# zakuro-ai/asr

Measured on AMD Instinct MI355X. Metric: utterances/sec (10 s, 161-bin) DS2 5x1024 BiGRU CTC train step, higher is better.
Workload: dtype bf16

## Files before the change

### asr_amd/_lib.py

```python
from __future__ import annotations

import ctypes as C
import os
from typing import Optional

_HERE = os.path.dirname(os.path.abspath(__file__))
LIB_PATH = os.environ.get("DS2_LIB_PATH") or os.path.join(_HERE, "lib", "libds2hip.so")

_lib: Optional[C.CDLL] = None

vp, i32, i64, f32, f64, sz = C.c_void_p, C.c_int, C.c_longlong, C.c_float, C.c_double, C.c_size_t

SIGNATURES = {
    "ds2_version": (C.c_char_p, []),
    "ds2_last_error": (C.c_char_p, []),
    "ds2_device_info": (i32, [C.POINTER(i32), C.POINTER(i32), C.c_char_p, i32]),
    "ds2_debug_flags": (i32, [vp, i32]),
    "ds2_rnn_ctx_init": (i32, [vp, vp, vp, vp]),
    "ds2_memset_async": (i32, [vp, i32, sz, vp]),
    "ds2_ablation_build": (i32, []),
    "ds2_rnn_persistent_status": (i32, [vp, vp]),
    "ds2_rnn_persistent_counters": (i32, [vp, vp]),
    "ds2_rnn_poison_if_starved": (i32, [vp, vp, sz, vp]),
    "ds2_rnn_poison_seen": (i32, [vp]),
    "ds2_rnn_step_gate": (i32, [vp, vp, vp, vp]),
    "ds2_rnn_persistent_enable": (i32, [vp, i32, i32]),
    "ds2_rnn_last_path": (i32, [vp]),
    "ds2_rnn_bwd_ksplit_footprint": (i32, [i32, i32, C.POINTER(i32)]),
    "ds2_gemm_f32_workspace_bytes": (sz, [i32, i32, i32, i32]),
    "ds2_gemm_f32": (i32, [i32, i32, i32, i32, i32, vp, i32, i64, vp, i32, i64, vp, i32, i64, vp, i32, i32, i32, vp, sz, vp]),
    "ds2_gemm_bf16_workspace_bytes": (sz, [i32, i32, i32, i32]),
    "ds2_conv1_fwd_bf16_stat_blocks": (i32, [i32, i32, i32]),
    "ds2_conv1_fwd_bf16_stats": (i32, [vp, vp, vp, vp, vp, i32, i32, i32, vp, vp]),
    "ds2_conv2_fwd_bf16_stat_blocks": (i32, [i32, i32, i32]),
    "ds2_conv2_fwd_bf16_stats": (i32, [vp, vp, vp, vp, vp, i32, i32, i32, vp, vp]),
    "ds2_chanstats_from_partials_workspace_bytes": (sz, []),
    "ds2_chanstats_from_partials": (i32, [vp, i32, i32, f64, vp, vp, vp, vp, f32, vp, sz, vp]),
    "ds2_gemm_bf16_tn": (i32, [i32, i32, i32, vp, i32, i64, vp, i32, i64, vp, i32, i64, i32, i32, i32, vp, sz, vp]),
    "ds2_gemm_bf16_tn_group": (i32, [i32, vp, i32, vp]),
    "ds2_gemm_bf16_tn_splitk_group_workspace_bytes": (sz, [i32, vp, i32]),
    "ds2_gemm_bf16_tn_splitk_group": (i32, [i32, vp, i32, vp, sz, vp]),
    "ds2_gemm_bf16_tn_splitk_group_ep": (i32, [i32, vp, i32, i32, vp, vp, vp, vp, sz, vp]),
    "ds2_gemm_bf16_nt": (i32, [i32, i32, i32, vp, i32, i64, vp, i32, i64, vp, i32, i64, vp, i32, i32, i32, vp, sz, vp]),
    "ds2_cast_bf16": (i32, [vp, i32, vp, i32, i32, i32, vp]),
    "ds2_gemm_bf16_nt_obf16": (i32, [i32, i32, i32, vp, i32, vp, i32, vp, i32, vp, vp]),
    "ds2_cast_f32_from_bf16": (i32, [vp, vp, i64, vp]),
    "ds2_rnn_fwd_x": (i32, [vp, i32, vp, vp, vp, vp, vp, vp, vp, i32, i32, i32, vp, vp, vp, vp, sz, vp]),
    "ds2_split_bf16": (i32, [vp, i32, vp, i32, i32, i32, i32, vp]),
    "ds2_cast_transpose_bf16": (i32, [vp, i32, vp, i32, i32, i32, vp]),
    "ds2_cast_bf16_both_workspace_bytes": (sz, [i32, i32]),
    "ds2_cast_bf16_both": (i32, [vp, i32, vp, i32, vp, i32, i32, i32, vp, vp, sz, vp]),
    "ds2_transpose_bf16": (i32, [vp, i32, vp, i32, i32, i32, vp, vp, sz, vp]),
    "ds2_colreduce_workspace_bytes": (sz, [i32, i32]),
    "ds2_colstats_f32": (i32, [vp, i32, i32, i32, vp, vp, vp, vp, f32, vp, sz, vp]),
    "ds2_add_colstats_f32": (i32, [vp, i32, vp, i32, vp, i32, i32, i32, vp, vp, vp, vp, f32, vp, sz, vp]),
    "ds2_colsum_f32": (i32, [vp, i32, i32, i32, vp, vp, vp, sz, vp]),
    "ds2_bn1d_apply_f32": (i32, [vp, i32, vp, i32, i32, i32, vp, vp, vp, vp, f32, vp]),
    "ds2_bn1d_apply_bf16": (i32, [vp, i32, vp, i32, i32, i32, vp, vp, vp, vp, f32, vp]),
    "ds2_bn1d_bwd_f32": (i32, [vp, i32, vp, i32, vp, i32, i32, i32, vp, vp, vp, f32, vp, vp, vp, sz, vp]),
    "ds2_bn1d_bwd_xbf16": (i32, [vp, i32, vp, i32, vp, i32, i32, i32, vp, vp, vp, f32, vp, vp, vp, sz, vp]),
    "ds2_center_colstats": (i32, [vp, i32, vp, i32, vp, i32, vp, i32, i32, i32, vp, vp, vp, vp, vp, f32, vp, sz, vp]),
    "ds2_wih_fold_bf16": (i32, [vp, i32, vp, i32, i32, vp, vp, vp, vp, f32, vp, i32, vp, vp, vp, vp]),
    "ds2_scale_rank1_f32": (i32, [vp, i32, i32, i32, vp, vp, vp, vp]),
    "ds2_chanreduce_workspace_bytes": (sz, [i32]),
    "ds2_bn2d_stats_f32": (i32, [vp, i32, i32, i32, i32, vp, vp, vp, vp, f32, vp, sz, vp]),
    "ds2_bn2d_act_fwd_f32": (i32, [vp, vp, i32, i32, i32, i32, vp, vp, vp, vp, vp, f32, vp]),
    "ds2_bn2d_act_bwd_f32": (i32, [vp, vp, vp, i32, i32, i32, i32, vp, vp, vp, vp, vp, f32, vp, vp, vp, sz, vp]),
    "ds2_bn2d_act_fwd_fused": (i32, [vp, i32, i32, i32, vp, vp, vp, vp, vp, f32, vp, vp, vp, vp]),
    "ds2_bn2d_act_collapse": (i32, [vp, i32, i32, i32, vp, vp, vp, vp, vp, f32, vp, vp, i32, vp]),
    "ds2_bn2d_act_bwd_fused_workspace_bytes": (sz, [i32, i32, i32]),
    "ds2_bn2d_act_bwd_fused": (i32, [vp, vp, i32, i32, i32, vp, vp, vp, vp, vp, f32, vp, vp, vp, vp, vp, vp, vp, sz, vp]),
    "ds2_transpose_bft_f32": (i32, [vp, vp, i32, i32, i32, i32, vp]),
    "ds2_transpose2d_f32": (i32, [vp, i32, i64, vp, i32, i64, i32, i32, i32, vp]),
    "ds2_conv_dims": (None, [i32, i32, C.POINTER(i32), C.POINTER(i32), C.POINTER(i32)]),
    "ds2_conv_packed_floats": (sz, [i32]),
    "ds2_conv_pack_f32": (i32, [vp, vp, vp, vp, vp, vp]),
    "ds2_conv1_fwd_f32": (i32, [vp, vp, vp, vp, vp, i32, i32, i32, vp]),
    "ds2_conv2_fwd_f32": (i32, [vp, vp, vp, vp, vp, i32, i32, i32, vp]),
    "ds2_conv2_dgrad_f32": (i32, [vp, vp, vp, i32, i32, i32, vp]),
    "ds2_conv_wgrad_workspace_bytes": (sz, [i32, i32, i32]),
    "ds2_conv1_wgrad_f32": (i32, [vp, vp, vp, vp, i32, i32, i32, i32, vp, sz, vp]),
    "ds2_conv2_wgrad_f32": (i32, [vp, vp, vp, vp, i32, i32, i32, i32, vp, sz, vp]),
    "ds2_conv2_bf16_packed_bytes": (sz, [i32]),
    "ds2_conv2_pack_bf16": (i32, [vp, vp, vp, vp, vp]),
    "ds2_nhwc_bf16_f32": (i32, [vp, vp, i32, i32, i32, vp]),
    "ds2_conv2_fwd_bf16": (i32, [vp, vp, vp, vp, vp, i32, i32, i32, vp]),
    "ds2_conv2_dgrad_bf16": (i32, [vp, vp, vp, vp, i32, i32, i32, vp]),
    "ds2_conv_padded_pitch": (i32, [i32]),
    "ds2_padcast_bf16": (i32, [vp, vp, i64, i32, vp]),
    "ds2_conv2_wgrad_bf16_workspace_bytes": (sz, [i32, i32]),
    "ds2_conv2_wgrad_bf16": (i32, [vp, vp, vp, vp, i32, i32, i32, vp, sz, vp]),
    "ds2_conv2_wgrad_nhwc_bf16": (i32, [vp, vp, vp, vp, i32, i32, i32, vp, sz, vp]),
    "ds2_rnn_packed_bytes": (sz, [i32, i32, i32, i32]),
    "ds2_rnn_pack_whh": (i32, [i32, vp, vp, vp, i32, i32, vp]),
    "ds2_weight_prep_bf16": (i32, [vp, i32, vp]),
    "ds2_rnn_fwd_workspace_bytes": (sz, [i32, i32, i32]),
    "ds2_rnn_fwd_ex": (i32, [vp, i32, vp, vp, vp, vp, vp, vp, i32, i32, i32, i32, vp, vp, vp, sz, vp]),
    "ds2_rnn_fwd": (i32, [vp, i32, vp, vp, vp, vp, vp, vp, i32, i32, i32, i32, vp, vp, sz, vp]),
    "ds2_rnn_bwd_workspace_bytes": (sz, [i32, i32, i32, i32]),
    "ds2_rnn_bwd_ex": (i32, [vp, i32, vp, i32, vp, vp, vp, vp, vp, i32, i32, i32, i32, vp, vp, vp, vp, vp, sz, vp]),
    "ds2_rnn_bwd_bn": (i32, [vp, i32, vp, i32, vp, i32, vp, vp, vp, vp, vp, f32, vp, vp, vp, vp, vp, vp, i32, i32, i32, i32, vp, vp, vp, vp, vp, sz, vp]),
    "ds2_rnn_bwd_bn_xbf16": (i32, [vp, i32, vp, i32, vp, i32, vp, vp, vp, vp, vp, f32, vp, vp, vp, vp, vp, vp, i32, i32, i32, i32, vp, vp, vp, vp, vp, sz, vp]),
    "ds2_rnn_bias_grads": (i32, [i32, vp, i32, i32, vp, vp, vp]),
    "ds2_rnn_bwd": (i32, [vp, i32, vp, i32, vp, vp, vp, vp, vp, i32, i32, i32, i32, vp, vp, vp, sz, vp]),
    "ds2_ctc_workspace_bytes": (sz, [i32, i32, i32]),
    "ds2_ctc_loss_f32": (i32, [vp, i32, i32, i32, i32, vp, vp, vp, vp, i32, vp, vp, i32, f32, vp, sz, vp]),
    "ds2_ctc_loss_ex_f32": (i32, [vp, i32, i32, i32, i32, vp, vp, vp, vp, i32, vp, vp, i32, f32, i32, vp, sz, vp]),
    "ds2_ctc_star_workspace_bytes": (sz, [i32, i32, i32]),
    "ds2_ctc_star_loss_f32": (i32, [vp, i32, i32, i32, i32, vp, vp, vp, vp, i32, f32, vp, vp, vp, i32, f32, i32, vp, sz, vp]),
    "ds2_ctc_mwer_workspace_bytes": (sz, [i32, i32, i32, i32]),
    "ds2_ctc_mwer_f32": (i32, [vp, i32, i32, i32, i32, i32, vp, vp, vp, vp, vp, i32, vp, vp, vp, vp, vp, i32, f32, i32, i32, vp, sz, vp]),
    "ds2_ctc_conf_max_unit_labels": (i32, []),
    "ds2_ctc_conf_workspace_bytes": (sz, [i32, i32, i32]),
    "ds2_ctc_conf_f32": (i32, [vp, i32, i32, i32, i32, vp, vp, vp, vp, i32, vp, vp, vp, vp, vp, i32, vp, vp, i32, vp, sz, vp]),
    "ds2_ctc_batch_mean_f32": (i32, [vp, i32, vp, vp]),
    "ds2_ctc_align_workspace_bytes": (sz, [i32, i32, i32]),
    "ds2_ctc_align_f32": (i32, [vp, i64, i64, i32, i32, i32, i32, vp, vp, vp, vp, i32, i32, vp, vp, vp, vp, vp, vp, sz, vp]),
    "ds2_ctc_align_tiled_workspace_bytes": (sz, [i32, i32, i32, i32, i32]),
    "ds2_ctc_align_tiled_f32": (i32, [vp, i64, i64, i32, i32, i32, i32, vp, vp, vp, vp, i32, i32, i32, vp, vp, vp, vp, vp, vp, sz, vp]),
    "ds2_ctc_align_star_row_f32": (i32, [vp, i64, i64, i32, i32, i32, i32, vp, f32, vp, vp]),
    "ds2_ctc_align_star_workspace_bytes": (sz, [i32, i32, i32]),
    "ds2_ctc_align_star_f32": (i32, [vp, i64, i64, i32, i32, i32, i32, vp, vp, vp, vp, i32, i32, f32, vp, vp, vp, vp, vp, vp, vp, sz, vp]),
    "ds2_ctc_align_star_tiled_workspace_bytes": (sz, [i32, i32, i32, i32, i32]),
    "ds2_ctc_align_star_tiled_f32": (i32, [vp, i64, i64, i32, i32, i32, i32, vp, vp, vp, vp, i32, i32, i32, f32, vp, vp, vp, vp, vp, vp, vp,
                                           sz, vp]),
    "ds2_ctc_kws_workspace_bytes": (sz, [i32, i32, i32, i32]),
    "ds2_ctc_kws_f32": (i32, [vp, i64, i64, i32, i32, i32, i32, vp, vp, vp, vp, i32, i32, vp, i32, vp, vp, vp, vp, vp, vp, vp, sz, vp]),
    "ds2_add_i64": (i32, [vp, i32, i64, vp]),
    "ds2_softmax_rows_f32": (i32, [vp, i32, vp, i32, i32, i32, vp]),
    "ds2_greedy_decode_workspace_bytes": (sz, [i32, i32]),
    "ds2_greedy_decode_f32": (i32, [vp, i64, i64, i32, i32, i32, vp, i32, vp, vp, vp, vp, sz, vp]),
    "ds2_ctc_segment_workspace_bytes": (sz, [i32, i32]),
    "ds2_ctc_segment_f32": (i32, [vp, i64, i64, i32, i32, i32, vp, i32, f32, i32, i32, i32, i32, vp, vp, vp, vp, vp, sz, vp]),
    "ds2_ctc_segment_gather_f32": (i32, [vp, i64, i64, i32, i32, i32, vp, vp, vp, i32, i32, vp, vp, vp]),
    "ds2_ctc_beam_max_width": (i32, []),
    "ds2_ctc_beam_workspace_bytes": (sz, [i32, i32, i32]),
    "ds2_ctc_beam_decode_f32": (i32, [vp, i64, i64, i32, i32, i32, vp, i32, i32, i32, f32, vp, vp, vp, vp, vp, sz, vp]),
    "ds2_ctc_beam_lm_max_candidates": (i32, []),
    "ds2_ctc_lm_packed_bytes": (sz, [i32, i32, i32, i32, i32]),
    "ds2_ctc_lm_pack": (i32, [i32, i32, vp, vp, vp, vp, i32, vp, vp, vp, i32, vp, i32, vp, i32, i32, vp, sz]),
    "ds2_ctc_lm_score": (i32, [vp, vp, i32, i32, C.POINTER(f32)]),
    "ds2_ctc_beam_decode_lm_f32": (i32, [vp, i64, i64, i32, i32, i32, vp, i32, i32, i32, f32, vp, sz, i32, i32, i32, f32, f32, vp, vp, vp, vp,
                                         vp, sz, vp]),
    "ds2_ctc_hot_packed_bytes": (sz, [i32, i32]),
    "ds2_ctc_hot_pack": (i32, [i32, i32, vp, vp, vp, vp, vp, vp, i32, vp, sz]),
    "ds2_ctc_hot_step": (i32, [vp, i32, i32, C.POINTER(i32), C.POINTER(f32)]),
    "ds2_ctc_beam_decode_hot_f32": (i32, [vp, i64, i64, i32, i32, i32, vp, i32, i32, i32, f32, vp, sz, i32, i32, i32, f32, f32, vp, vp, sz,
                                          vp, vp, vp, vp, vp, sz, vp]),
    "ds2_edit_distance_workspace_bytes": (sz, [i32, i64]),
    "ds2_edit_distance_i32": (i32, [vp, i64, vp, vp, vp, vp, i32, i64, vp, vp, sz, vp]),
    "ds2_edit_align_workspace_bytes": (sz, [i32, i64]),
    "ds2_edit_align_i32": (i32, [vp, i64, vp, vp, vp, vp, i32, i64, vp, vp, vp, vp, sz, vp]),
    "ds2_conv1_bf16_row_pitch": (i32, [i32]),
    "ds2_conv1_bf16_bytes": (sz, [i32, i32, i32, i32]),
    "ds2_conv1_pack_bf16": (i32, [vp, vp, vp]),
    "ds2_conv1_gather_bf16": (i32, [vp, vp, vp, i32, i32, i32, vp]),
    "ds2_conv1_fwd_bf16": (i32, [vp, vp, vp, vp, vp, i32, i32, i32, vp]),
    "ds2_conv1_wgrad_bf16_workspace_bytes": (sz, [i32, i32]),
    "ds2_conv1_wgrad_bf16": (i32, [vp, vp, vp, vp, i32, i32, i32, vp, sz, vp]),
    "ds2_spectrogram_frames": (i32, [i32, i32]),
    "ds2_spectrogram_workspace_bytes": (sz, [i32, i32, i32, i32]),
    "ds2_spectrogram_f32": (i32, [vp, i64, vp, i32, i32, i32, i32, vp, i32, i32, vp, vp, sz, vp]),
    "ds2_spectrogram_aug_workspace_bytes": (sz, [i32, i32, i32, i32]),
    "ds2_spectrogram_aug_f32": (i32, [vp, i64, vp, i32, i32, i32, i32, vp, i32, i32, vp, i64, vp, vp, vp, vp, vp, i32, vp, i32, vp, vp, sz,
                                      vp]),
    "ds2_tempo_sizes": (i32, [i32, f64, f64, f64, C.POINTER(i32), C.POINTER(i32), C.POINTER(i32)]),
    "ds2_tempo_out_samples": (i32, [i32, f64]),
    "ds2_tempo_workspace_bytes": (sz, [i32]),
    "ds2_tempo_gain_f32": (i32, [vp, i64, vp, vp, vp, i32, i32, f64, f64, f64, vp, i64, vp, vp, i32, vp, sz, vp]),
    "ds2_wave_unpack_f32": (i32, [vp, i64, i32, vp, vp, vp, i32, i32, vp, i64, vp]),
    "ds2_resample_out_samples": (i64, [i64, i32, i32]),
    "ds2_resample_tile_samples": (i32, []),
    "ds2_wave_resample_f32": (i32, [vp, i64, i32, vp, vp, vp, vp, vp, vp, vp, vp, i64, i32, i32, vp, i64, vp]),
    "ds2_reverb_max_taps": (i32, []),
    "ds2_reverb_tile_samples": (i32, []),
    "ds2_reverb_tap_chunk": (i32, []),
    "ds2_reverb_f32": (i32, [vp, i64, vp, vp, i64, vp, vp, i32, i32, vp, i64, vp]),
    "ds2_adamw_f32": (i32, [vp, vp, vp, vp, i64, f32, f32, f32, f32, f32, i32, f32, vp]),
    "ds2_adamw_gated_f32": (i32, [vp, vp, vp, vp, i64, f32, f32, f32, f32, f32, i32, f32, vp, vp]),
    "ds2_scale_f32": (i32, [vp, i64, f32, vp]),
    "ds2_bf16_residual_f32": (i32, [vp, vp, i64, vp]),
    "ds2_sum3_f32": (i32, [vp, vp, vp, vp, i64, vp]),
}


class TnProblem(C.Structure):
    _fields_ = [("A", vp), ("B", vp), ("C", vp), ("M", i32), ("N", i32), ("K", i32), ("lda", i32), ("ldb", i32), ("ldc", i32)]


class PrepLayer(C.Structure):
    _fields_ = [("whh", vp), ("wp_fwd", vp), ("wp_bwd", vp), ("wih", vp), ("wih_t", vp), ("wih_r", vp),
                ("gates", i32), ("H", i32), ("R", i32), ("Cc", i32), ("ld_wih", i32), ("ld_t", i32), ("ld_r", i32), ("reserved", i32)]


class DS2LibraryError(RuntimeError):
    pass


def load() -> C.CDLL:
    global _lib
    if _lib is not None:
        return _lib
    if not os.path.exists(LIB_PATH):
        raise DS2LibraryError(
            f"{LIB_PATH} not found: build the HIP extension first "
            "(python -c 'import __graft_entry__ as g; g.build()'  or  make -C asr_amd/csrc). "
            "asr_amd has no CPU fallback.")
    lib = C.CDLL(LIB_PATH)
    for name, (res, args) in SIGNATURES.items():
        fn = getattr(lib, name)
        fn.restype = res
        fn.argtypes = args
    _lib = lib
    return lib


def check(rc: int, what: str = ""):
    if rc != 0:
        msg = load().ds2_last_error().decode(errors="replace")
        raise DS2LibraryError(f"libds2hip call failed{(' in ' + what) if what else ''}: {msg}")


def version() -> str:
    return load().ds2_version().decode()


def conv_dims(F: int, Tin: int):
    d1, d2, t = i32(), i32(), i32()
    load().ds2_conv_dims(F, Tin, C.byref(d1), C.byref(d2), C.byref(t))
    return d1.value, d2.value, t.value
```

### asr_amd/csrc/conv_bf16.hip

```cpp
#include "common.h"
#include <stdlib.h>

namespace {

typedef __bf16 bf16x8 __attribute__((ext_vector_type(8)));

constexpr int TT = 128, KT = 11, PT = 5, CH = 32;
constexpr int NPIX = TT + KT - 1;
constexpr int IPITCH = 80;
constexpr int WROW = KT * 2 * 2 * 32 * 16;

__device__ __attribute__((aligned(16))) float g_zero_cb[4] = {0.f, 0.f, 0.f, 0.f};

struct CArgs {
  const __bf16* in;
  const __bf16* wpk;
  const float* bias;
  float* out;
  const int* lens;
  int B, Din, T, Dtot, KD, SD, PD, OS, OO;
  int gx, gy, gz;
};

constexpr int IN_CHUNKS = NPIX * 4;
constexpr int IN_IT = (IN_CHUNKS + 255) / 256;
constexpr int W_CHUNKS = WROW / 16;
constexpr int W_IT = (W_CHUNKS + 255) / 256;

template <int SD, int R>
__global__ __launch_bounds__(256) void conv2_bf16_rows_kernel(CArgs a, int n_out, float* __restrict__ stat_part) {
  constexpr int RING = (R - 1) * SD + 1;
  constexpr int SLOT = NPIX * IPITCH;
  __shared__ __attribute__((aligned(16))) char in_lds[RING * SLOT];
  __shared__ __attribute__((aligned(16))) char w_lds[WROW];
  const int tid = threadIdx.x, lane = tid & 63, wave = tid >> 6;
  const int half = lane >> 5, l31 = lane & 31;
  int bx, by, bz;
  {
    const int total = a.gx * a.gy * a.gz, id = blockIdx.x;
    const int lin = (total & 7) == 0 ? (id & 7) * (total >> 3) + (id >> 3) : id;
    by = lin % a.gy;
    const int pair = lin / a.gy;
    bx = pair % a.gx; bz = pair / a.gx;
  }
  const int t0 = bx * TT, o0 = R * by, b = bz;
  const int len = a.lens ? min(a.lens[b], a.T) : a.T;
  const int t = t0 + wave * 32 + l31;
  auto out_ptr = [&](int o, int co) { return a.out + (((long long)b * CH + co) * a.Dtot + (a.OS * o + a.OO)) * a.T + t; };
  if (t0 >= len) {
    if (t < a.T) {
#pragma unroll
      for (int q = 0; q < R; ++q)
        if (o0 + q < n_out) {
#pragma unroll
          for (int r = 0; r < 16; ++r) *out_ptr(o0 + q, (r & 3) + 8 * (r >> 2) + 4 * half) = 0.f;
        }
    }
    return;
  }
  f32x16 acc[R];
#pragma unroll
  for (int q = 0; q < R; ++q)
#pragma unroll
    for (int r = 0; r < 16; ++r) acc[q][r] = 0.f;

  const int f0 = SD * o0 - a.PD;
  f32x4 ri[IN_IT], rw[W_IT];
  auto load_in = [&](int f) {
    const bool rowok = f >= 0 && f < a.Din;
    const char* rowp = reinterpret_cast<const char*>(a.in + (((long long)b * a.Din + (rowok ? f : 0)) * a.T) * CH);
#pragma unroll
    for (int u = 0; u < IN_IT; ++u) {
      const int c = tid + 256 * u;
      const int pix = c >> 2, q = c & 3;
      const int tt = t0 - PT + pix;
      const bool ok = rowok && c < IN_CHUNKS && tt >= 0 && tt < a.T;
      const void* p = ok ? (const void*)(rowp + ((long long)tt * CH) * 2 + q * 16) : (const void*)g_zero_cb;
      ri[u] = *reinterpret_cast<const f32x4*>(p);
    }
  };
  auto store_in = [&](int slot) {
#pragma unroll
    for (int u = 0; u < IN_IT; ++u) {
      const int c = tid + 256 * u;
      if (c < IN_CHUNKS) *reinterpret_cast<f32x4*>(in_lds + slot * SLOT + (c >> 2) * IPITCH + (c & 3) * 16) = ri[u];
    }
  };
  auto load_w = [&](int kd) {
    const char* wp = reinterpret_cast<const char*>(a.wpk) + (long long)kd * WROW;
#pragma unroll
    for (int u = 0; u < W_IT; ++u) {
      const int c = tid + 256 * u;
      rw[u] = *reinterpret_cast<const f32x4*>(wp + (c < W_CHUNKS ? c : 0) * 16);
    }
  };
  auto store_w = [&]() {
#pragma unroll
    for (int u = 0; u < W_IT; ++u) {
      const int c = tid + 256 * u;
      if (c < W_CHUNKS) *reinterpret_cast<f32x4*>(w_lds + c * 16) = rw[u];
    }
  };
#pragma unroll
  for (int j = 0; j < RING - 1; ++j) {
    load_in(f0 + j);
    store_in(j);
  }
  load_in(f0 + RING - 1);
  load_w(0);
  const int pix_off = (wave * 32 + l31) * IPITCH + half * 16;
  const char* abase = w_lds + half * (32 * 16) + l31 * 16;
  int slot0 = 0;
  for (int kd = 0; kd < a.KD; ++kd) {
    __syncthreads();
    {
      int snew = slot0 + RING - 1;
      if (snew >= RING) snew -= RING;
      store_in(snew);
    }
    store_w();
    __syncthreads();
    if (kd + 1 < a.KD) {
      load_in(f0 + kd + RING);
      load_w(kd + 1);
    }
    const char* bq[R];
#pragma unroll
    for (int q = 0; q < R; ++q) {
      int sl = slot0 + q * SD;
      if (sl >= RING) sl -= RING;
      bq[q] = in_lds + sl * SLOT + pix_off;
    }
#pragma unroll
    for (int kt = 0; kt < KT; ++kt) {
#pragma unroll
      for (int kk = 0; kk < 2; ++kk) {
        const bf16x8 af = *reinterpret_cast<const bf16x8*>(abase + (kt * 2 + kk) * (2 * 32 * 16));
#pragma unroll
        for (int q = 0; q < R; ++q) {
          const bf16x8 x = *reinterpret_cast<const bf16x8*>(bq[q] + kt * IPITCH + kk * 32);
          acc[q] = __builtin_amdgcn_mfma_f32_32x32x16_bf16(af, x, acc[q], 0, 0, 0);
        }
      }
    }
    slot0 = slot0 + 1 == RING ? 0 : slot0 + 1;
  }
  float bv[16];
#pragma unroll
  for (int r = 0; r < 16; ++r) bv[r] = a.bias ? a.bias[(r & 3) + 8 * (r >> 2) + 4 * half] : 0.f;
  float s1[16], s2[16];
#pragma unroll
  for (int r = 0; r < 16; ++r) { s1[r] = 0.f; s2[r] = 0.f; }
#pragma unroll
  for (int q = 0; q < R; ++q)
    if (o0 + q < n_out) {
#pragma unroll
      for (int r = 0; r < 16; ++r) {
        const float v = (t >= len || t >= a.T) ? 0.f : acc[q][r] + bv[r];
        if (t < a.T) *out_ptr(o0 + q, (r & 3) + 8 * (r >> 2) + 4 * half) = v;
        s1[r] += v;
        s2[r] += v * v;
      }
    }
  if (stat_part) {
    __shared__ float red[4][32][2];
#pragma unroll
    for (int r = 0; r < 16; ++r) {
#pragma unroll
      for (int m = 1; m < 32; m <<= 1) { s1[r] += __shfl_xor(s1[r], m); s2[r] += __shfl_xor(s2[r], m); }
      if (l31 == 0) { const int co = (r & 3) + 8 * (r >> 2) + 4 * half; red[wave][co][0] = s1[r]; red[wave][co][1] = s2[r]; }
    }
    __syncthreads();
    if (tid < 64) {
      const int co = tid >> 1, w = tid & 1;
      const float sum = ((red[0][co][w] + red[1][co][w]) + red[2][co][w]) + red[3][co][w];
      const long long blk = ((long long)bz * a.gy + by) * a.gx + bx;
      stat_part[(blk * 32 + co) * 2 + w] = sum;
    }
  }
}

__global__ __launch_bounds__(256) void nhwc_cast_kernel(const float* __restrict__ src, __bf16* __restrict__ dst, int Bn, int D, int T) {
  __shared__ float tile[CH][65];
  const int t0 = blockIdx.x * 64, d = blockIdx.y, b = blockIdx.z;
  const int tx = threadIdx.x & 63, ty = threadIdx.x >> 6;
#pragma unroll
  for (int i = 0; i < 8; ++i) {
    const int c = ty + 4 * i, t = t0 + tx;
    tile[c][tx] = (t < T) ? src[(((long long)b * CH + c) * D + d) * T + t] : 0.f;
  }
  __syncthreads();
  const int c = threadIdx.x & 31, tq = threadIdx.x >> 5;
#pragma unroll
  for (int i = 0; i < 8; ++i) {
    const int tl = tq + 8 * i, t = t0 + tl;
    if (t < T) dst[(((long long)b * D + d) * T + t) * CH + c] = (__bf16)tile[c][tl];
  }
}

__global__ void pack_conv2_bf16_kernel(const float* __restrict__ W, __bf16* __restrict__ wf, __bf16* __restrict__ wd0, __bf16* __restrict__ wd1) {
  const int per_row = WROW / 2;
  const int nf = 21 * per_row, n0 = 11 * per_row, n1 = 10 * per_row;
  const int idx = blockIdx.x * blockDim.x + threadIdx.x;
  if (idx >= nf + n0 + n1) return;
  int which, i;
  if (idx < nf) { which = 0; i = idx; } else if (idx < nf + n0) { which = 1; i = idx - nf; } else { which = 2; i = idx - nf - n0; }
  const int j = i & 7, m = (i >> 3) & 31, kg = (i >> 8) & 1, kk = (i >> 9) & 1;
  const int rest = i >> 10;
  const int kt = rest % KT, kdr = rest / KT;
  const int kch = kk * 16 + kg * 8 + j;
  float v;
  if (which == 0) {
    v = W[((m * 32 + kch) * 21 + kdr) * 11 + kt];
    wf[i] = (__bf16)v;
  } else {
    const int p = which - 1, KDe = (21 - p + 1) / 2;
    v = W[((kch * 32 + m) * 21 + (2 * (KDe - 1 - kdr) + p)) * 11 + (10 - kt)];
    (which == 1 ? wd0 : wd1)[i] = (__bf16)v;
  }
}

}

extern "C" size_t ds2_conv2_bf16_packed_bytes(int which) { return (size_t)(which == 0 ? 21 : which == 1 ? 11 : 10) * WROW; }

extern "C" int ds2_conv2_pack_bf16(const float* w2, void* wf, void* wd0, void* wd1, void* stream) {
  DS2_REQUIRE(w2 && wf && wd0 && wd1, "ds2_conv2_pack_bf16: null pointer");
  const int total = (21 + 11 + 10) * (WROW / 2);
  hipLaunchKernelGGL(pack_conv2_bf16_kernel, dim3(ceil_div(total, 256)), dim3(256), 0, (hipStream_t)stream, w2, (__bf16*)wf, (__bf16*)wd0,
                     (__bf16*)wd1);
  DS2_LAUNCH_CHECK("pack_conv2_bf16_kernel");
  return 0;
}

extern "C" int ds2_nhwc_bf16_f32(const float* src, void* dst, int B, int D, int T, void* stream) {
  DS2_REQUIRE(src && dst && B > 0 && D > 0 && T > 0, "ds2_nhwc_bf16_f32: bad args");
  hipLaunchKernelGGL(nhwc_cast_kernel, dim3(ceil_div(T, 64), D, B), dim3(256), 0, (hipStream_t)stream, src, (__bf16*)dst, B, D, T);
  DS2_LAUNCH_CHECK("nhwc_cast_kernel");
  return 0;
}

extern "C" int ds2_conv2_fwd_bf16_stat_blocks(int B, int D1, int T) {
  const int D2 = (D1 + 2 * 10 - 21) / 2 + 1;
  return ceil_div(T, TT) * ceil_div(D2, 3) * B;
}

extern "C" int ds2_conv2_fwd_bf16_stats(const void* a1_nhwc, const void* wf, const float* bias, const int* lens_dev, float* y2, int B, int D1,
                                        int T, float* stat_part, void* stream) {
  DS2_REQUIRE(a1_nhwc && wf && y2, "ds2_conv2_fwd_bf16: null pointer");
  const int D2 = (D1 + 2 * 10 - 21) / 2 + 1;
  CArgs a{};
  a.in = (const __bf16*)a1_nhwc; a.wpk = (const __bf16*)wf; a.bias = bias; a.out = y2; a.lens = lens_dev;
  a.B = B; a.Din = D1; a.T = T; a.Dtot = D2; a.KD = 21; a.SD = 2; a.PD = 10; a.OS = 1; a.OO = 0;
  if (stat_part) DS2_HIP(hipMemsetAsync(stat_part, 0, (size_t)ds2_conv2_fwd_bf16_stat_blocks(B, D1, T) * 64 * sizeof(float), (hipStream_t)stream));
  a.gx = ceil_div(T, TT); a.gy = ceil_div(D2, 3); a.gz = B;
  hipLaunchKernelGGL((conv2_bf16_rows_kernel<2, 3>), dim3(a.gx * a.gy * a.gz), dim3(256), 0, (hipStream_t)stream, a, D2, stat_part);
  DS2_LAUNCH_CHECK("conv2_bf16_rows_kernel fwd");
  return 0;
}

extern "C" int ds2_conv2_fwd_bf16(const void* a1_nhwc, const void* wf, const float* bias, const int* lens_dev, float* y2, int B, int D1,
                                  int T, void* stream) {
  return ds2_conv2_fwd_bf16_stats(a1_nhwc, wf, bias, lens_dev, y2, B, D1, T, nullptr, stream);
}

extern "C" int ds2_conv2_dgrad_bf16(const void* dy2_nhwc, const void* wd0, const void* wd1, float* da1, int B, int D1, int T, void* stream) {
  DS2_REQUIRE(dy2_nhwc && wd0 && wd1 && da1, "ds2_conv2_dgrad_bf16: null pointer");
  const int D2 = (D1 + 2 * 10 - 21) / 2 + 1;
  for (int p = 0; p < 2; ++p) {
    const int KDe = (21 - p + 1) / 2;
    const int n_o = (D1 - p + 1) / 2;
    CArgs a{};
    a.in = (const __bf16*)dy2_nhwc; a.wpk = (const __bf16*)(p == 0 ? wd0 : wd1); a.bias = nullptr; a.out = da1; a.lens = nullptr;
    a.B = B; a.Din = D2; a.T = T; a.Dtot = D1; a.KD = KDe; a.SD = 1; a.PD = KDe - 6; a.OS = 2; a.OO = p;
    a.gx = ceil_div(T, TT); a.gy = ceil_div(n_o, 4); a.gz = B;
    hipLaunchKernelGGL((conv2_bf16_rows_kernel<1, 4>), dim3(a.gx * a.gy * a.gz), dim3(256), 0, (hipStream_t)stream, a, n_o, (float*)nullptr);
  }
  DS2_LAUNCH_CHECK("conv2_bf16_rows_kernel dgrad");
  return 0;
}

namespace {

constexpr int WT = 64;
constexpr int WK = WT + 16;
constexpr int WPITCH = 176;
constexpr int KDG = 3;
constexpr int TAPS = KDG * KT;
constexpr int TPW = (TAPS + 3) / 4;

struct WArgs {
  const __bf16* a1p;
  const __bf16* dyp;
  float* part;
  const int* lens;
  int B, D1, D2, T, Tp, pairs_per_chunk;
};

typedef unsigned int u32x4 __attribute__((ext_vector_type(4)));

__device__ __forceinline__ void store_shifted_copies(const u32x4 lo, const u32x4 hi, char* dst ) {
  const unsigned W[8] = {lo.x, lo.y, lo.z, lo.w, hi.x, hi.y, hi.z, hi.w};
#pragma unroll
  for (int r = 0; r < 8; ++r) {
    const int w0 = (8 - r) >> 1;
    u32x4 o;
    if ((r & 1) == 0) {
      o = u32x4{W[w0], W[w0 + 1], W[w0 + 2], W[w0 + 3]};
    } else {
      o = u32x4{__builtin_amdgcn_alignbit(W[w0 + 1], W[w0], 16), __builtin_amdgcn_alignbit(W[w0 + 2], W[w0 + 1], 16),
                __builtin_amdgcn_alignbit(W[w0 + 3], W[w0 + 2], 16), __builtin_amdgcn_alignbit(W[w0 + 4], W[w0 + 3], 16)};
    }
    *reinterpret_cast<u32x4*>(dst + r * 32 * WPITCH) = o;
  }
}

__global__ __launch_bounds__(256) __attribute__((amdgpu_waves_per_eu(2, 2))) void conv2_wgrad_bf16_kernel(WArgs a) {
  __shared__ __attribute__((aligned(16))) char dy_lds[8 * 32 * WPITCH];
  __shared__ __attribute__((aligned(16))) char a1_lds[KDG * 32 * WPITCH];
  const int tid = threadIdx.x, lane = tid & 63;
  const int wave = __builtin_amdgcn_readfirstlane(tid >> 6);
  const int l31 = lane & 31, half = lane >> 5;
  const int grp = blockIdx.x, chunk = blockIdx.y;
  const int kd0 = grp * KDG;

  f32x16 acc[TPW];
#pragma unroll
  for (int i = 0; i < TPW; ++i)
#pragma unroll
    for (int r = 0; r < 16; ++r) acc[i][r] = 0.f;

  constexpr int NDY = 2, NA1 = (KDG * 32 * 10 + 255) / 256;
  u32x4 dlo[NDY], dhi[NDY], av[NA1];

  const int npairs = a.B * a.D2;
  const int pend = min(npairs, (chunk + 1) * a.pairs_per_chunk);
  int p = chunk * a.pairs_per_chunk, t0 = 0, len = 0;
  auto settle = [&]() {
    while (p < pend) {
      len = a.lens ? min(a.lens[p / a.D2], a.T) : a.T;
      if (t0 < len) return true;
      ++p;
      t0 = 0;
    }
    return false;
  };
  auto load_tile = [&]() {
    const int b = p / a.D2, o = p % a.D2;
#pragma unroll
    for (int k = 0; k < NDY; ++k) {
      const int idx = tid + 256 * k;
      const int co = idx / 11, m = idx % 11;
      const __bf16* row = a.dyp + (((long long)b * 32 + min(co, 31)) * a.D2 + o) * a.Tp;
      const int xl = t0 - 8 + m * 8, xh = xl + 8;
      const bool okl = idx < 352 && m >= 2 && m < 2 + WT / 8 && xl + 8 <= a.Tp;
      const bool okh = idx < 352 && m + 1 >= 2 && m + 1 < 2 + WT / 8 && xh + 8 <= a.Tp;
      dlo[k] = *reinterpret_cast<const u32x4*>(okl ? (const void*)(row + xl) : (const void*)g_zero_cb);
      dhi[k] = *reinterpret_cast<const u32x4*>(okh ? (const void*)(row + xh) : (const void*)g_zero_cb);
    }
#pragma unroll
    for (int k = 0; k < NA1; ++k) {
      const int c = tid + 256 * k;
      const int ch = c % 10, ci = (c / 10) % 32, kdl = c / 320;
      const int f = 2 * o + (kd0 + kdl) - 10;
      const int x0 = t0 + ch * 8;
      const bool ok = c < KDG * 320 && (kd0 + kdl) < 21 && f >= 0 && f < a.D1 && x0 + 8 <= a.Tp;
      av[k] = *reinterpret_cast<const u32x4*>(ok ? (const void*)(a.a1p + (((long long)b * 32 + ci) * a.D1 + f) * a.Tp + x0)
                                                 : (const void*)g_zero_cb);
    }
  };

  bool have = settle();
  if (have) load_tile();
  while (have) {
    __syncthreads();
#pragma unroll
    for (int k = 0; k < NDY; ++k) {
      const int idx = tid + 256 * k;
      if (idx < 352) store_shifted_copies(dlo[k], dhi[k], dy_lds + (idx / 11) * WPITCH + (idx % 11) * 16);
    }
#pragma unroll
    for (int k = 0; k < NA1; ++k) {
      const int c = tid + 256 * k;
      if (c < KDG * 320) *reinterpret_cast<u32x4*>(a1_lds + ((c / 320) * 32 + (c / 10) % 32) * WPITCH + (c % 10) * 16) = av[k];
    }
    __syncthreads();
    t0 += WT;
    have = settle();
    if (have) load_tile();
    const char* ap[3];
#pragma unroll
    for (int q = 0; q < 3; ++q) {
      const int kt = min(wave + 4 * q, KT - 1);
      const int s = kt - PT;
      const int r = s & 7;
      const int joff = (s < 0) ? 8 : 0;
      ap[q] = dy_lds + (r * 32 + l31) * WPITCH + (8 * half + joff) * 2;
    }
    const char* bp = a1_lds + l31 * WPITCH + (8 * half) * 2;
#pragma unroll
    for (int ks = 0; ks < WK / 16; ++ks) {
      bf16x8 af[3], bfr[KDG];
#pragma unroll
      for (int q = 0; q < 3; ++q) af[q] = *reinterpret_cast<const bf16x8*>(ap[q] + ks * 32);
#pragma unroll
      for (int kdl = 0; kdl < KDG; ++kdl) bfr[kdl] = *reinterpret_cast<const bf16x8*>(bp + kdl * 32 * WPITCH + ks * 32);
#pragma unroll
      for (int q = 0; q < 3; ++q)
#pragma unroll
        for (int kdl = 0; kdl < KDG; ++kdl) acc[q * KDG + kdl] = __builtin_amdgcn_mfma_f32_32x32x16_bf16(af[q], bfr[kdl], acc[q * KDG + kdl], 0, 0, 0);
    }
  }
#pragma unroll
  for (int i = 0; i < TPW; ++i) {
    const int kt = wave + 4 * (i / KDG), kdl = i % KDG;
    if (kt < KT) {
      const int tap = kdl * KT + kt;
      float* out = a.part + ((((long long)chunk * gridDim.x + grp) * TAPS + tap) * 32) * 32;
#pragma unroll
      for (int r = 0; r < 16; ++r) {
        const int co = (r & 3) + 8 * (r >> 2) + 4 * half;
        out[co * 32 + l31] = acc[i][r];
      }
    }
  }
}

__global__ void conv2_wgrad_bf16_reduce_kernel(const float* __restrict__ part, float* __restrict__ dW, int chunks, int ngroups) {
  const int j = blockIdx.x * blockDim.x + threadIdx.x;
  const int per_chunk = ngroups * TAPS * 32 * 32;
  if (j >= per_chunk) return;
  const int ci = j & 31, co = (j >> 5) & 31, tap = (j >> 10) % TAPS, grp = (j >> 10) / TAPS;
// ... 259 lines not shown
```

### asr_amd/csrc/norm.hip

```cpp
#include "common.h"
#include <algorithm>

namespace {

typedef float f32x4_dw __attribute__((ext_vector_type(4), aligned(4)));
typedef __bf16 nbf16x4 __attribute__((ext_vector_type(4)));
constexpr int BN_ROWS_PER_BLOCK = 32;
__device__ __forceinline__ f32x4 ld4(const float* __restrict__ p, int valid, bool vec) {
  f32x4 v = {0.f, 0.f, 0.f, 0.f};
  if (valid >= 4 && vec) {
    v = *reinterpret_cast<const f32x4*>(p);
  } else if (valid >= 4) {
    const f32x4_dw q = *reinterpret_cast<const f32x4_dw*>(p);
    v.x = q.x; v.y = q.y; v.z = q.z; v.w = q.w;
  } else {
    if (valid > 0) v.x = p[0];
    if (valid > 1) v.y = p[1];
    if (valid > 2) v.z = p[2];
    if (valid > 3) v.w = p[3];
  }
  return v;
}
__device__ __forceinline__ void st4(float* __restrict__ p, f32x4 v, int valid, bool vec) {
  if (valid >= 4 && vec) {
// ... 347 lines not shown
#pragma unroll
        for (int j = 0; j < 4; ++j) if (tq0 + j < T) out_f32[row * T + tq0 + j] = r[j];
      }
    }
    if (out_pad) {
#pragma unroll
      for (int j = 0; j < 4; ++j) if (tq0 + j < T) out_pad[row * Tp + 8 + tq0 + j] = (nbf16)r[j];
      if (blockIdx.x == 0 && l16 < 8) out_pad[row * Tp + l16] = (nbf16)0.f;
      if (blockIdx.x == gridDim.x - 1) for (int q = l16; T + 8 + q < Tp; q += 16) out_pad[row * Tp + T + 8 + q] = (nbf16)0.f;
    }
    if (BWD && chan_part) {
      float sum = ((r[0] + r[1]) + r[2]) + r[3];
#pragma unroll
      for (int m = 1; m < 16; m <<= 1) sum += __shfl_xor(sum, m);
      const long long blk = ((long long)blockIdx.z * gridDim.y + blockIdx.y) * gridDim.x + blockIdx.x;
      if (l16 == 0) chan_part[blk * CH + c] = sum;
    }
  }
  if (out_nhwc) {
    __syncthreads();
    typedef nbf16 nbf16x8 __attribute__((ext_vector_type(8)));
    const int c8 = (threadIdx.x & 3) * 8, tl = threadIdx.x >> 2, tt = t0 + tl;
    if (tt < T) {
      nbf16x8 o;
#pragma unroll
      for (int j = 0; j < 8; ++j) o[j] = (nbf16)tile[c8 + j][tl];
      *reinterpret_cast<nbf16x8*>(out_nhwc + (((long long)b * D + d) * T + tt) * CH + c8) = o;
    }
  }
}

__global__ __launch_bounds__(256) void bn2d_act_collapse_kernel(const float* __restrict__ Yraw, int Bn, int D, int T, const int* __restrict__ lens,
                                                                const float* __restrict__ mean, const float* __restrict__ var,
                                                                const float* __restrict__ gamma, const float* __restrict__ beta, float eps,
                                                                float* __restrict__ out_f32, nbf16* __restrict__ out_bf, int ldb) {
  typedef float f32x4u __attribute__((ext_vector_type(4), aligned(4)));
  typedef nbf16 nbf16x8 __attribute__((ext_vector_type(8)));
  __shared__ float tile[64][33];
  const int F = 32 * D;
  const int b = blockIdx.z;
  const int f0 = blockIdx.y * 64, t0 = blockIdx.x * 32;
  const int len = min(lens[b], T);
  {
    const int q4 = (threadIdx.x & 7) * 4, t = t0 + q4;
#pragma unroll
    for (int i = 0; i < 2; ++i) {
      const int fl = (threadIdx.x >> 3) + 32 * i, f = f0 + fl;
      float a[4] = {0.f, 0.f, 0.f, 0.f};
      if (f < F && t < len) {
        const int c = f / D;
        const float sc = rsqrtf(var[c] + eps) * gamma[c], mu = mean[c], be = beta[c];
        const float* p = Yraw + ((long long)b * F + f) * T + t;
        float y[4] = {0.f, 0.f, 0.f, 0.f};
        if (t + 3 < T) { const f32x4u q = *reinterpret_cast<const f32x4u*>(p); y[0] = q.x; y[1] = q.y; y[2] = q.z; y[3] = q.w; }
        else for (int j = 0; j < 4; ++j) if (t + j < T) y[j] = p[j];
#pragma unroll
        for (int j = 0; j < 4; ++j) a[j] = (t + j < len) ? fminf(fmaxf((y[j] - mu) * sc + be, 0.f), 20.f) : 0.f;
      }
#pragma unroll
      for (int j = 0; j < 4; ++j) tile[fl][q4 + j] = a[j];
    }
  }
  __syncthreads();
  const int tl = threadIdx.x >> 3, t = t0 + tl, f8 = (threadIdx.x & 7) * 8, f = f0 + f8;
  if (t < T) {
    const long long row = (long long)t * Bn + b;
    if (out_f32) {
#pragma unroll
      for (int j = 0; j < 8; ++j) if (f + j < F) out_f32[row * F + f + j] = tile[f8 + j][tl];
    }
    if (out_bf && f < ldb) {
      nbf16x8 o;
#pragma unroll
      for (int j = 0; j < 8; ++j) o[j] = (f + j < F) ? (nbf16)tile[f8 + j][tl] : (nbf16)0.f;
      *reinterpret_cast<nbf16x8*>(out_bf + row * ldb + f) = o;
    }
  }
}

__global__ __launch_bounds__(256) void chan_part_finalize_kernel(const float* __restrict__ part, long long n, long long rpb, double* __restrict__ tmp,
                                                                 int nblk, float* __restrict__ out, int stage) {
  __shared__ double red[8][32];
  const int c = threadIdx.x & 31, r = threadIdx.x >> 5;
  double s = 0.0;
  if (stage == 0) {
    const long long k0 = (long long)blockIdx.x * rpb, k1 = k0 + rpb < n ? k0 + rpb : n;
    long long k = k0 + r;
    for (; k + 24 < k1; k += 32) {
      const float v0 = part[k * 32 + c], v1 = part[(k + 8) * 32 + c], v2 = part[(k + 16) * 32 + c], v3 = part[(k + 24) * 32 + c];
      s += (double)v0; s += (double)v1; s += (double)v2; s += (double)v3;
    }
    for (; k < k1; k += 8) s += (double)part[k * 32 + c];
  } else {
    for (int k = r; k < nblk; k += 8) s += tmp[(long long)k * 32 + c];
  }
  red[r][c] = s;
  __syncthreads();
  if (r == 0) {
    double t = 0.0;
#pragma unroll
    for (int i = 0; i < 8; ++i) t += red[i][c];
    if (stage == 0) tmp[(long long)blockIdx.x * 32 + c] = t;
    else out[c] = (float)t;
  }
}

__global__ __launch_bounds__(256) void transpose_bft_kernel(const float* __restrict__ src, float* __restrict__ dst, int Bn, int F, int T,
                                                            int dir) {
  typedef float f32x4u __attribute__((ext_vector_type(4), aligned(4)));
  __shared__ float tile[64][65];
  const int b = blockIdx.z;
  const int f0 = blockIdx.y * 64, t0 = blockIdx.x * 64;
  const int q4 = (threadIdx.x & 15) * 4, r16 = threadIdx.x >> 4;
  auto bft = [&](int f, int t) { return ((long long)b * F + f) * T + t; };
  auto tbf = [&](int t, int f) { return ((long long)t * Bn + b) * F + f; };
#pragma unroll
  for (int i = 0; i < 4; ++i) {
    const int r = r16 + 16 * i;
    float v[4] = {0.f, 0.f, 0.f, 0.f};
    if (dir == 0) {
      const int f = f0 + r, t = t0 + q4;
      if (f < F) {
        if (t + 3 < T) { const f32x4u q = *reinterpret_cast<const f32x4u*>(src + bft(f, t)); v[0] = q.x; v[1] = q.y; v[2] = q.z; v[3] = q.w; }
        else for (int j = 0; j < 4; ++j) if (t + j < T) v[j] = src[bft(f, t + j)];
      }
    } else {
      const int t = t0 + r, f = f0 + q4;
      if (t < T) {
        if (f + 3 < F) { const f32x4u q = *reinterpret_cast<const f32x4u*>(src + tbf(t, f)); v[0] = q.x; v[1] = q.y; v[2] = q.z; v[3] = q.w; }
        else for (int j = 0; j < 4; ++j) if (f + j < F) v[j] = src[tbf(t, f + j)];
      }
    }
#pragma unroll
    for (int j = 0; j < 4; ++j) tile[r][q4 + j] = v[j];
  }
  __syncthreads();
#pragma unroll
  for (int i = 0; i < 4; ++i) {
    const int r = r16 + 16 * i;
    const f32x4u o = {tile[q4][r], tile[q4 + 1][r], tile[q4 + 2][r], tile[q4 + 3][r]};
    if (dir == 0) {
      const int t = t0 + r, f = f0 + q4;
      if (t < T) {
        if (f + 3 < F) *reinterpret_cast<f32x4u*>(dst + tbf(t, f)) = o;
        else for (int j = 0; j < 4; ++j) if (f + j < F) dst[tbf(t, f + j)] = o[j];
      }
    } else {
      const int f = f0 + r, t = t0 + q4;
      if (f < F) {
        if (t + 3 < T) *reinterpret_cast<f32x4u*>(dst + bft(f, t)) = o;
        else for (int j = 0; j < 4; ++j) if (t + j < T) dst[bft(f, t + j)] = o[j];
      }
    }
  }
}

__global__ __launch_bounds__(256) void transpose2d_kernel(const float* __restrict__ src, int lds_, long long ss, float* __restrict__ dst,
                                                          int ldd, long long sd, int R, int Cc) {
  __shared__ float tile[32][33];
  src += (long long)blockIdx.z * ss;
  dst += (long long)blockIdx.z * sd;
  const int r0 = blockIdx.y * 32, c0 = blockIdx.x * 32;
  const int tx = threadIdx.x & 31, ty = threadIdx.x >> 5;
#pragma unroll
  for (int i = 0; i < 4; ++i) {
    const int r = r0 + ty + 8 * i, c = c0 + tx;
    tile[ty + 8 * i][tx] = (r < R && c < Cc) ? src[(long long)r * lds_ + c] : 0.f;
  }
  __syncthreads();
#pragma unroll
  for (int i = 0; i < 4; ++i) {
    const int c = c0 + ty + 8 * i, r = r0 + tx;
    if (r < R && c < Cc) dst[(long long)c * ldd + r] = tile[tx][ty + 8 * i];
  }
}


__global__ __launch_bounds__(256) void center_colstats_kernel(const float* __restrict__ Xa, int lda, const float* __restrict__ Xb, int ldb,
                                                              const float* __restrict__ hsum, int ntiles, __bf16* __restrict__ Yc, int ldy,
                                                              int M, int H, int rows_per_chunk, float inv_m, float* __restrict__ m0_out,
                                                              float* __restrict__ part, int vec) {
  __shared__ float red[16][64][2];
  const int cq = threadIdx.x & 15, rg = threadIdx.x >> 4;
  const int c0 = blockIdx.x * 64 + cq * 4;
  const int valid = H - c0;
  const int rbeg = blockIdx.y * rows_per_chunk;
  const int rend = min(M, rbeg + rows_per_chunk);
  f32x4 s0 = {0, 0, 0, 0}, s1 = {0, 0, 0, 0}, m0 = {0, 0, 0, 0};
  if (valid > 0) {
    for (int d = 0; d < 2; ++d)
      for (int t = 0; t < ntiles; ++t) m0 += ld4(hsum + ((long long)d * ntiles + t) * H + c0, valid, false);
    m0 *= inv_m;
    if (blockIdx.y == 0 && rg == 0) st4(m0_out + c0, m0, valid, false);
    for (int r = rbeg + rg; r < rend; r += 16) {
      const f32x4 x = ld4(Xa + (long long)r * lda + c0, valid, vec) + ld4(Xb + (long long)r * ldb + c0, valid, vec);
      const f32x4 xc = x - m0;
      s0 += xc;
      s1 += xc * xc;
      if (valid >= 4) {
        *reinterpret_cast<nbf16x4*>(Yc + (long long)r * ldy + c0) = nbf16x4{(__bf16)xc.x, (__bf16)xc.y, (__bf16)xc.z, (__bf16)xc.w};
      } else {
        const float v[4] = {xc.x, xc.y, xc.z, xc.w};
        for (int e = 0; e < 4; ++e) Yc[(long long)r * ldy + c0 + e] = (__bf16)(e < valid ? v[e] : 0.f);
      }
    }
  } else if (c0 < ldy) {
    for (int r = rbeg + rg; r < rend; r += 16)
      for (int e = 0; e < 4 && c0 + e < ldy; ++e) Yc[(long long)r * ldy + c0 + e] = (__bf16)0.f;
  }
  red[rg][cq * 4 + 0][0] = s0.x; red[rg][cq * 4 + 0][1] = s1.x;
  red[rg][cq * 4 + 1][0] = s0.y; red[rg][cq * 4 + 1][1] = s1.y;
  red[rg][cq * 4 + 2][0] = s0.z; red[rg][cq * 4 + 2][1] = s1.z;
  red[rg][cq * 4 + 3][0] = s0.w; red[rg][cq * 4 + 3][1] = s1.w;
  __syncthreads();
  if (threadIdx.x < 128) {
    const int c = threadIdx.x >> 1, w = threadIdx.x & 1;
    float sacc = 0.f;
#pragma unroll
    for (int g = 0; g < 16; ++g) sacc += red[g][c][w];
    const int col = blockIdx.x * 64 + c;
    if (col < H) part[((long long)blockIdx.y * H + col) * 2 + w] = sacc;
  }
}

__global__ __launch_bounds__(256) void center_finalize_kernel(const float* __restrict__ part, int chunks, int H, double count,
                                                              const float* __restrict__ m0, float* __restrict__ mean, float* __restrict__ var,
                                                              float* __restrict__ delta, float* __restrict__ run_mean,
                                                              float* __restrict__ run_var, float momentum) {
  __shared__ double red[8][32][2];
  const int cl = threadIdx.x & 31, grp = threadIdx.x >> 5;
  const int c = blockIdx.x * 32 + cl;
  double a = 0.0, b = 0.0;
  if (c < H)
    for (int k = grp; k < chunks; k += 8) {
      a += (double)part[((long long)k * H + c) * 2 + 0];
      b += (double)part[((long long)k * H + c) * 2 + 1];
    }
  red[grp][cl][0] = a;
  red[grp][cl][1] = b;
  __syncthreads();
  if (grp != 0 || c >= H) return;
  a = 0.0; b = 0.0;
#pragma unroll
  for (int g = 0; g < 8; ++g) { a += red[g][cl][0]; b += red[g][cl][1]; }
  const double d = a / count;
  double v = b / count - d * d;
  if (v < 0.0) v = 0.0;
  const double m = (double)m0[c] + d;
  delta[c] = (float)d;
  mean[c] = (float)m;
  var[c] = (float)v;
  if (run_mean) {
    const double unb = count > 1.0 ? v * count / (count - 1.0) : v;
    run_mean[c] = (float)((1.0 - momentum) * (double)run_mean[c] + momentum * m);
    run_var[c] = (float)((1.0 - momentum) * (double)run_var[c] + momentum * unb);
  }
}

__global__ __launch_bounds__(256) void col_reduce_bwd_xbf_kernel(const __bf16* __restrict__ X, int ldx, const float* __restrict__ dY, int lddy, int M, int H,
                                                                 int rows_per_chunk, const float* __restrict__ mean, const float* __restrict__ var,
                                                                 float eps, float* __restrict__ part, int vec) {
  __shared__ float red[16][64][2];
  const int cq = threadIdx.x & 15, rg = threadIdx.x >> 4;
  const int c0 = blockIdx.x * 64 + cq * 4;
  const int valid = H - c0;
  const int rbeg = blockIdx.y * rows_per_chunk;
  const int rend = min(M, rbeg + rows_per_chunk);
  f32x4 s0 = {0, 0, 0, 0}, s1 = {0, 0, 0, 0};
  if (valid > 0) {
    const f32x4 mu = ld4(mean + c0, valid, false), vv = ld4(var + c0, valid, false);
    f32x4 rs;
    rs.x = rsqrtf(vv.x + eps); rs.y = rsqrtf(vv.y + eps); rs.z = rsqrtf(vv.z + eps); rs.w = rsqrtf(vv.w + eps);
    for (int r = rbeg + rg; r < rend; r += 16) {
      f32x4 x = {0.f, 0.f, 0.f, 0.f};
      if (valid >= 4) {
        const nbf16x4 q = *reinterpret_cast<const nbf16x4*>(X + (long long)r * ldx + c0);
        x = f32x4{(float)q[0], (float)q[1], (float)q[2], (float)q[3]};
      } else {
        float v[4] = {0.f, 0.f, 0.f, 0.f};
        for (int e = 0; e < valid; ++e) v[e] = (float)X[(long long)r * ldx + c0 + e];
        x = f32x4{v[0], v[1], v[2], v[3]};
      }
      const f32x4 dy = ld4(dY + (long long)r * lddy + c0, valid, vec);
      s0 += dy;
      s1 += dy * ((x - mu) * rs);
    }
  }
  red[rg][cq * 4 + 0][0] = s0.x; red[rg][cq * 4 + 0][1] = s1.x;
  red[rg][cq * 4 + 1][0] = s0.y; red[rg][cq * 4 + 1][1] = s1.y;
  red[rg][cq * 4 + 2][0] = s0.z; red[rg][cq * 4 + 2][1] = s1.z;
  red[rg][cq * 4 + 3][0] = s0.w; red[rg][cq * 4 + 3][1] = s1.w;
  __syncthreads();
  if (threadIdx.x < 128) {
    const int c = threadIdx.x >> 1, w = threadIdx.x & 1;
    float sacc = 0.f;
#pragma unroll
    for (int g = 0; g < 16; ++g) sacc += red[g][c][w];
    const int col = blockIdx.x * 64 + c;
    if (col < H) part[((long long)blockIdx.y * H + col) * 2 + w] = sacc;
  }
}

__global__ __launch_bounds__(256) void bn1d_bwd_apply_xbf_kernel(const float* __restrict__ dY, int lddy, const __bf16* __restrict__ X, int ldx,
                                                                 float* __restrict__ dX, int lddx, int M, int H, const float* __restrict__ mean,
                                                                 const float* __restrict__ var, const float* __restrict__ gamma,
                                                                 const float* __restrict__ s0, const float* __restrict__ s1, float eps,
// ... 78 lines not shown
  return col_reduce_launch(0, X, ldx, nullptr, 0, nullptr, 0, M, H, nullptr, nullptr, 0.f, 0, mean, var, run_mean, run_var,
                           momentum, ws, ws_bytes, (hipStream_t)stream);
}

extern "C" int ds2_add_colstats_f32(const float* Xa, int lda, const float* Xb, int ldb, float* Y, int ldy, int M, int H,
                                    float* mean, float* var, float* run_mean, float* run_var, float momentum, void* ws,
                                    size_t ws_bytes, void* stream) {
  DS2_REQUIRE(Xa && Xb && Y && mean && var && M > 0 && H > 0, "ds2_add_colstats_f32: bad args");
  return col_reduce_launch(1, Xa, lda, Xb, ldb, Y, ldy, M, H, nullptr, nullptr, 0.f, 0, mean, var, run_mean, run_var, momentum,
                           ws, ws_bytes, (hipStream_t)stream);
}

extern "C" int ds2_colsum_f32(const float* X, int ldx, int M, int H, float* sum, float* sumsq, void* ws, size_t ws_bytes,
                              void* stream) {
  DS2_REQUIRE(X && sum && sumsq && M > 0 && H > 0, "ds2_colsum_f32: bad args");
  return col_reduce_launch(0, X, ldx, nullptr, 0, nullptr, 0, M, H, nullptr, nullptr, 0.f, 1, sum, sumsq, nullptr, nullptr, 0.f,
                           ws, ws_bytes, (hipStream_t)stream);
}

extern "C" int ds2_bn1d_apply_f32(const float* X, int ldx, float* Y, int ldy, int M, int H, const float* mean, const float* var,
                                  const float* gamma, const float* beta, float eps, void* stream) {
  DS2_REQUIRE(X && Y && mean && var && gamma && beta, "ds2_bn1d_apply_f32: null pointer");
  const int vec = (ldx % 4 == 0) && (ldy % 4 == 0) && ((uintptr_t)X % 16 == 0) && ((uintptr_t)Y % 16 == 0);
  dim3 grid(ceil_div(ceil_div(H, 4), 256), ceil_div(M, BN_ROWS_PER_BLOCK));
  hipLaunchKernelGGL((bn1d_apply_kernel<false>), grid, dim3(256), 0, (hipStream_t)stream, X, ldx, (void*)Y, ldy, M, H, mean, var, gamma, beta,
                     eps, vec);
  DS2_LAUNCH_CHECK("bn1d_apply_kernel");
  return 0;
}

extern "C" int ds2_bn1d_apply_bf16(const float* X, int ldx, void* Y, int ldy, int M, int H, const float* mean, const float* var,
                                   const float* gamma, const float* beta, float eps, void* stream) {
  DS2_REQUIRE(X && Y && mean && var && gamma && beta, "ds2_bn1d_apply_bf16: null pointer");
  DS2_REQUIRE(ldy >= H && (ldy % 8) == 0, "ds2_bn1d_apply_bf16: bad output pitch %d", ldy);
  const int vec = (ldx % 4 == 0) && ((uintptr_t)X % 16 == 0);
  dim3 grid(ceil_div(ldy / 4, 256), ceil_div(M, BN_ROWS_PER_BLOCK));
  hipLaunchKernelGGL((bn1d_apply_kernel<true>), grid, dim3(256), 0, (hipStream_t)stream, X, ldx, Y, ldy, M, H, mean, var, gamma, beta, eps, vec);
  DS2_LAUNCH_CHECK("bn1d_apply_kernel<bf16>");
  return 0;
}

int ds2i_bn1d_bwd_apply(const float* dY, int lddy, const float* X, int ldx, float* dX, int lddx, int M, int H, const float* mean, const float* var,
                        const float* gamma, const float* s0, const float* s1, float eps, hipStream_t stream) {
  const int vec = (ldx % 4 == 0) && (lddy % 4 == 0) && (lddx % 4 == 0) && ((uintptr_t)X % 16 == 0) &&
                  ((uintptr_t)dY % 16 == 0) && ((uintptr_t)dX % 16 == 0);
  dim3 grid(ceil_div(ceil_div(H, 4), 256), ceil_div(M, BN_ROWS_PER_BLOCK));
  hipLaunchKernelGGL(bn1d_bwd_apply_kernel, grid, dim3(256), 0, stream, dY, lddy, X, ldx, dX, lddx, M, H, mean, var, gamma, s0, s1, eps,
                     1.0f / (float)M, vec);
  DS2_LAUNCH_CHECK("bn1d_bwd_apply_kernel");
  return 0;
}

extern "C" int ds2_bn1d_bwd_f32(const float* dY, int lddy, const float* X, int ldx, float* dX, int lddx, int M, int H,
                                const float* mean, const float* var, const float* gamma, float eps, float* dgamma, float* dbeta,
                                void* ws, size_t ws_bytes, void* stream) {
  DS2_REQUIRE(dY && X && mean && var && gamma && dgamma && dbeta, "ds2_bn1d_bwd_f32: null pointer");
  int rc = col_reduce_launch(2, X, ldx, dY, lddy, nullptr, 0, M, H, mean, var, eps, 1, dbeta, dgamma, nullptr, nullptr, 0.f, ws,
                             ws_bytes, (hipStream_t)stream);
  if (rc || !dX) return rc;
  return ds2i_bn1d_bwd_apply(dY, lddy, X, ldx, dX, lddx, M, H, mean, var, gamma, dbeta, dgamma, eps, (hipStream_t)stream);
}


int ds2i_bn1d_bwd_apply_xbf(const float* dY, int lddy, const void* X, int ldx, float* dX, int lddx, int M, int H, const float* mean, const float* var,
                            const float* gamma, const float* s0, const float* s1, float eps, hipStream_t stream) {
  DS2_REQUIRE((H % 4) == 0 && (ldx % 4) == 0, "bn1d_bwd_apply (bf16 input): H and its pitch must be multiples of 4");
  const int vec = (lddy % 4 == 0) && (lddx % 4 == 0) && ((uintptr_t)dY % 16 == 0) && ((uintptr_t)dX % 16 == 0);
  dim3 grid(ceil_div(ceil_div(H, 4), 256), ceil_div(M, BN_ROWS_PER_BLOCK));
  hipLaunchKernelGGL(bn1d_bwd_apply_xbf_kernel, grid, dim3(256), 0, stream, dY, lddy, (const __bf16*)X, ldx, dX, lddx, M, H, mean, var, gamma, s0, s1, eps,
                     1.0f / (float)M, vec);
  DS2_LAUNCH_CHECK("bn1d_bwd_apply_xbf_kernel");
  return 0;
}

extern "C" int ds2_center_colstats(const float* Xa, int lda, const float* Xb, int ldb, const float* hsum, int ntiles, void* Yc_bf16, int ldyc, int M,
                                   int H, float* mean, float* var, float* delta, float* run_mean, float* run_var, float momentum, void* ws,
                                   size_t ws_bytes, void* stream) {
  DS2_REQUIRE(Xa && Xb && hsum && Yc_bf16 && mean && var && delta && M > 0 && H > 0 && ntiles > 0, "ds2_center_colstats: bad args");
  DS2_REQUIRE(ldyc >= H && (ldyc % 8) == 0 && ((uintptr_t)Yc_bf16 % 16) == 0, "ds2_center_colstats: bad operand pitch %d", ldyc);
  const int colblocks = ceil_div(ldyc, 64);
  const int chunks = pick_chunks(M, colblocks, 64);
  const int rpc = ceil_div(M, chunks);
  const int nch = ceil_div(M, rpc);
  DS2_REQUIRE(ws && ws_bytes >= ((size_t)nch * H * 2 + H) * sizeof(float), "ds2_center_colstats: workspace too small");
  const int vec = (lda % 4 == 0) && (ldb % 4 == 0) && ((uintptr_t)Xa % 16 == 0) && ((uintptr_t)Xb % 16 == 0);
  float* part = (float*)ws;
  float* m0 = part + (size_t)nch * H * 2;
  hipStream_t s = (hipStream_t)stream;
  hipLaunchKernelGGL(center_colstats_kernel, dim3(colblocks, nch), dim3(256), 0, s, Xa, lda, Xb, ldb, hsum, ntiles, (__bf16*)Yc_bf16, ldyc, M, H, rpc,
                     1.0f / (float)M, m0, part, vec);
  DS2_LAUNCH_CHECK("center_colstats_kernel");
  hipLaunchKernelGGL(center_finalize_kernel, dim3(ceil_div(H, 32)), dim3(256), 0, s, (const float*)part, nch, H, (double)M, (const float*)m0, mean, var,
                     delta, run_mean, run_var, momentum);
  DS2_LAUNCH_CHECK("center_finalize_kernel");
  return 0;
}

extern "C" int ds2_bn1d_bwd_xbf16(const float* dY, int lddy, const void* X_bf16, int ldx, float* dX, int lddx, int M, int H, const float* mean,
                                  const float* var, const float* gamma, float eps, float* dgamma, float* dbeta, void* ws, size_t ws_bytes, void* stream) {
  DS2_REQUIRE(dY && X_bf16 && mean && var && gamma && dgamma && dbeta && M > 0 && H > 0 && (ldx % 4) == 0, "ds2_bn1d_bwd_xbf16: bad args");
  const int colblocks = ceil_div(H, 64);
  const int chunks = pick_chunks(M, colblocks, 64);
  const int rpc = ceil_div(M, chunks);
  const int nch = ceil_div(M, rpc);
  DS2_REQUIRE(ws && ws_bytes >= (size_t)nch * H * 2 * sizeof(float), "ds2_bn1d_bwd_xbf16: workspace too small");
  const int vec = (lddy % 4 == 0) && ((uintptr_t)dY % 16 == 0);
  hipStream_t s = (hipStream_t)stream;
  hipLaunchKernelGGL(col_reduce_bwd_xbf_kernel, dim3(colblocks, nch), dim3(256), 0, s, (const __bf16*)X_bf16, ldx, dY, lddy, M, H, rpc, mean, var, eps,
                     (float*)ws, vec);
  DS2_LAUNCH_CHECK("col_reduce_bwd_xbf_kernel");
  hipLaunchKernelGGL(col_finalize_kernel, dim3(ceil_div(H, 32)), dim3(256), 0, s, (const float*)ws, nch, H, (double)M, 1, dbeta, dgamma, (float*)nullptr,
                     (float*)nullptr, 0.f);
  DS2_LAUNCH_CHECK("col_finalize_kernel");
  if (!dX) return 0;
  return ds2i_bn1d_bwd_apply_xbf(dY, lddy, X_bf16, ldx, dX, lddx, M, H, mean, var, gamma, dbeta, dgamma, eps, s);
}

extern "C" int ds2_scale_rank1_f32(float* C, int ldc, int R, int N, const float* scale, const float* rowv, const float* shift, void* stream) {
  DS2_REQUIRE(C && scale && rowv && shift && R > 0 && N > 0 && (N % 4) == 0 && (ldc % 4) == 0 && ((uintptr_t)C % 16) == 0 &&
              ((uintptr_t)scale % 16) == 0 && ((uintptr_t)shift % 16) == 0, "ds2_scale_rank1_f32: bad args");
  const long long total = (long long)R * (N / 4);
  const int blocks = (int)std::min<long long>((total + 255) / 256, 8192);
  hipLaunchKernelGGL(scale_rank1_kernel, dim3(blocks), dim3(256), 0, (hipStream_t)stream, C, ldc, R, N, scale, rowv, shift);
  DS2_LAUNCH_CHECK("scale_rank1_kernel");
  return 0;
}

extern "C" size_t ds2_chanreduce_workspace_bytes(int C) { return (size_t)2048 * 2 * sizeof(float) * (size_t)(C > 1 ? C : 1); }

static int chan_reduce_launch(int mode, const float* Y, const float* dA, int Bn, int C, int D, int T, const int* lens,
                              const float* mean, const float* var, const float* gamma, const float* beta, float eps, int kind,
                              float* out0, float* out1, float* run_mean, float* run_var, float momentum, void* ws,
                              size_t ws_bytes, hipStream_t s) {
  const int nrows = Bn * D;
  int chunks = 2048 / C;
  if (chunks < 1) chunks = 1;
  if (chunks > nrows) chunks = nrows;
  const int rpc = ceil_div(nrows, chunks);
  const int nch = ceil_div(nrows, rpc);
  DS2_REQUIRE(ws && ws_bytes >= (size_t)nch * C * 2 * sizeof(float), "chan_reduce: workspace too small");
  float* part = (float*)ws;
  dim3 grid(C, nch), block(256);
  if (mode == 0) hipLaunchKernelGGL((chan_reduce_kernel<0>), grid, block, 0, s, Y, dA, Bn, C, D, T, rpc, lens, mean, var, gamma, beta, eps, part);
  else hipLaunchKernelGGL((chan_reduce_kernel<1>), grid, block, 0, s, Y, dA, Bn, C, D, T, rpc, lens, mean, var, gamma, beta, eps, part);
  DS2_LAUNCH_CHECK("chan_reduce_kernel");
  hipLaunchKernelGGL(col_finalize_kernel, dim3(ceil_div(C, 32)), dim3(256), 0, s, (const float*)part, nch, C,
                     (double)Bn * D * T, kind, out0, out1, run_mean, run_var, momentum);
  DS2_LAUNCH_CHECK("col_finalize_kernel");
  return 0;
}

__global__ __launch_bounds__(256) void chanstats_partials_kernel(const float* __restrict__ part, int n, int rpb, double* __restrict__ tmp, int nblk,
                                                                 double count, float* __restrict__ mean, float* __restrict__ var,
                                                                 float* __restrict__ run_mean, float* __restrict__ run_var, float momentum, int stage) {
  __shared__ double red[4][64];
  const int c = threadIdx.x & 63, r = threadIdx.x >> 6;
  double s = 0.0;
  if (stage == 0) {
    const int k0 = blockIdx.x * rpb, k1 = min(n, k0 + rpb);
    int k = k0 + r;
    for (; k + 12 < k1; k += 16) {
      const float v0 = part[(long long)k * 64 + c], v1 = part[(long long)(k + 4) * 64 + c], v2 = part[(long long)(k + 8) * 64 + c],
                  v3 = part[(long long)(k + 12) * 64 + c];
      s += (double)v0; s += (double)v1; s += (double)v2; s += (double)v3;
    }
    for (; k < k1; k += 4) s += (double)part[(long long)k * 64 + c];
  } else {
    for (int k = r; k < nblk; k += 4) s += tmp[(long long)k * 64 + c];
  }
  red[r][c] = s;
  __syncthreads();
  if (r != 0) return;
  const double t = ((red[0][c] + red[1][c]) + red[2][c]) + red[3][c];
  if (stage == 0) {
    tmp[(long long)blockIdx.x * 64 + c] = t;
    return;
  }
  red[0][c] = t;
  __syncthreads();
  if (c < 32) {
    const double m = red[0][2 * c] / count;
    double v = red[0][2 * c + 1] / count - m * m;
    if (v < 0.0) v = 0.0;
    mean[c] = (float)m;
    var[c] = (float)v;
    if (run_mean) {
      const double unb = count > 1.0 ? v * count / (count - 1.0) : v;
      run_mean[c] = (float)((1.0 - momentum) * (double)run_mean[c] + momentum * m);
      run_var[c] = (float)((1.0 - momentum) * (double)run_var[c] + momentum * unb);
    }
  }
}

extern "C" size_t ds2_chanstats_from_partials_workspace_bytes(void) { return (size_t)128 * 64 * sizeof(double); }

extern "C" int ds2_chanstats_from_partials(const float* part, int nblk, int C, double count, float* mean, float* var, float* run_mean,
                                           float* run_var, float momentum, void* ws, size_t ws_bytes, void* stream) {
  DS2_REQUIRE(part && mean && var && nblk > 0 && C > 0 && count > 0, "ds2_chanstats_from_partials: bad args");
  if (C == 32 && nblk >= 512 && ws && ws_bytes >= ds2_chanstats_from_partials_workspace_bytes()) {
    constexpr int SB = 128;
    const int rpb = ceil_div(nblk, SB), nb = ceil_div(nblk, rpb);
    hipLaunchKernelGGL(chanstats_partials_kernel, dim3(nb), dim3(256), 0, (hipStream_t)stream, part, nblk, rpb, (double*)ws, nb, count, mean, var,
                       run_mean, run_var, momentum, 0);
    hipLaunchKernelGGL(chanstats_partials_kernel, dim3(1), dim3(256), 0, (hipStream_t)stream, part, nblk, rpb, (double*)ws, nb, count, mean, var,
                       run_mean, run_var, momentum, 1);
    DS2_LAUNCH_CHECK("chanstats_partials_kernel");
    return 0;
  }
  hipLaunchKernelGGL(col_finalize_kernel, dim3(ceil_div(C, 32)), dim3(256), 0, (hipStream_t)stream, part, nblk, C, count, 0, mean, var, run_mean,
                     run_var, momentum);
  DS2_LAUNCH_CHECK("col_finalize_kernel");
  return 0;
}

extern "C" int ds2_bn2d_stats_f32(const float* Y, int B, int C, int D, int T, float* mean, float* var, float* run_mean,
                                  float* run_var, float momentum, void* ws, size_t ws_bytes, void* stream) {
  DS2_REQUIRE(Y && mean && var, "ds2_bn2d_stats_f32: null pointer");
  return chan_reduce_launch(0, Y, nullptr, B, C, D, T, nullptr, nullptr, nullptr, nullptr, nullptr, 0.f, 0, mean, var, run_mean,
                            run_var, momentum, ws, ws_bytes, (hipStream_t)stream);
}

extern "C" int ds2_bn2d_act_fwd_f32(const float* Y, float* A, int B, int C, int D, int T, const int* lens_dev, const float* mean,
                                    const float* var, const float* gamma, const float* beta, float eps, void* stream) {
  DS2_REQUIRE(Y && A && lens_dev && mean && var && gamma && beta, "ds2_bn2d_act_fwd_f32: null pointer");
  const long long total = (long long)B * C * D * ((T + 3) / 4);
  int blocks = (int)((total + 255) / 256);
  if (blocks > 8192) blocks = 8192;
  hipLaunchKernelGGL(bn2d_act_fwd_kernel, dim3(blocks), dim3(256), 0, (hipStream_t)stream, Y, A, B, C, D, T, lens_dev, mean, var,
                     gamma, beta, eps);
  DS2_LAUNCH_CHECK("bn2d_act_fwd_kernel");
  return 0;
}

extern "C" int ds2_bn2d_act_bwd_f32(const float* Y, const float* dA, float* dY, int B, int C, int D, int T, const int* lens_dev,
                                    const float* mean, const float* var, const float* gamma, const float* beta, float eps,
                                    float* dgamma, float* dbeta, void* ws, size_t ws_bytes, void* stream) {
  DS2_REQUIRE(Y && dA && dY && lens_dev && mean && var && gamma && beta && dgamma && dbeta, "ds2_bn2d_act_bwd_f32: null pointer");
  int rc = chan_reduce_launch(1, Y, dA, B, C, D, T, lens_dev, mean, var, gamma, beta, eps, 1, dbeta, dgamma, nullptr, nullptr,
                              0.f, ws, ws_bytes, (hipStream_t)stream);
  if (rc) return rc;
  const long long total = (long long)B * C * D * ((T + 3) / 4);
  int blocks = (int)((total + 255) / 256);
  if (blocks > 8192) blocks = 8192;
  hipLaunchKernelGGL(bn2d_act_bwd_apply_kernel, dim3(blocks), dim3(256), 0, (hipStream_t)stream, Y, dA, dY, B, C, D, T, lens_dev,
                     mean, var, gamma, beta, (const float*)dbeta, (const float*)dgamma, eps, 1.0f / ((float)B * D * T));
  DS2_LAUNCH_CHECK("bn2d_act_bwd_apply_kernel");
  return 0;
}

extern "C" int ds2_bn2d_act_fwd_fused(const float* Y, int B, int D, int T, const int* lens_dev, const float* mean, const float* var,
                                      const float* gamma, const float* beta, float eps, float* a_f32, void* a_pad, void* a_nhwc, void* stream) {
  DS2_REQUIRE(Y && lens_dev && mean && var && gamma && beta && (a_f32 || a_pad || a_nhwc), "ds2_bn2d_act_fwd_fused: null pointer");
  const int Tp = (T + 16 + 7) / 8 * 8;
  hipLaunchKernelGGL((bn2d_tile_kernel<false>), dim3(ceil_div(T, 64), D, B), dim3(256), 0, (hipStream_t)stream, Y, (const float*)nullptr, B, D, T, Tp,
                     lens_dev, mean, var, gamma, beta, (const float*)nullptr, (const float*)nullptr, eps, 0.f, a_f32, (nbf16*)a_pad, (nbf16*)a_nhwc,
                     (float*)nullptr);
  DS2_LAUNCH_CHECK("bn2d_tile_kernel<fwd>");
  return 0;
}

extern "C" int ds2_bn2d_act_collapse(const float* Y, int B, int D, int T, const int* lens_dev, const float* mean, const float* var,
                                     const float* gamma, const float* beta, float eps, float* x_f32, void* x_bf16, int ld_bf, void* stream) {
  DS2_REQUIRE(Y && lens_dev && mean && var && gamma && beta && (x_f32 || x_bf16), "ds2_bn2d_act_collapse: null pointer");
  DS2_REQUIRE(!x_bf16 || (ld_bf >= 32 * D && (ld_bf % 8) == 0), "ds2_bn2d_act_collapse: bad bf16 pitch %d", ld_bf);
  hipLaunchKernelGGL(bn2d_act_collapse_kernel, dim3(ceil_div(T, 32), ceil_div(ld_bf > 32 * D ? ld_bf : 32 * D, 64), B), dim3(256), 0, (hipStream_t)stream, Y, B, D, T, lens_dev, mean, var,
                     gamma, beta, eps, x_f32, (nbf16*)x_bf16, ld_bf);
  DS2_LAUNCH_CHECK("bn2d_act_collapse_kernel");
  return 0;
}

constexpr int CPF_BLOCKS = 128;
extern "C" size_t ds2_bn2d_act_bwd_fused_workspace_bytes(int B, int D, int T) {
  return ds2_chanreduce_workspace_bytes(32) + align_up((size_t)B * D * ceil_div(T, 64) * 32 * sizeof(float), 16) + (size_t)CPF_BLOCKS * 32 * sizeof(double);
}

extern "C" int ds2_bn2d_act_bwd_fused(const float* Y, const float* dA, int B, int D, int T, const int* lens_dev, const float* mean,
                                      const float* var, const float* gamma, const float* beta, float eps, float* dgamma, float* dbeta,
                                      float* dbias, float* dy_f32, void* dy_pad, void* dy_nhwc, void* ws, size_t ws_bytes, void* stream) {
  DS2_REQUIRE(Y && dA && lens_dev && mean && var && gamma && beta && dgamma && dbeta && dbias, "ds2_bn2d_act_bwd_fused: null pointer");
  DS2_REQUIRE(ws && ws_bytes >= ds2_bn2d_act_bwd_fused_workspace_bytes(B, D, T), "ds2_bn2d_act_bwd_fused: workspace too small");
  const size_t red_bytes = ds2_chanreduce_workspace_bytes(32);
  int rc = chan_reduce_launch(1, Y, dA, B, 32, D, T, lens_dev, mean, var, gamma, beta, eps, 1, dbeta, dgamma, nullptr, nullptr, 0.f, ws,
                              red_bytes, (hipStream_t)stream);
  if (rc) return rc;
  float* part = reinterpret_cast<float*>(static_cast<char*>(ws) + red_bytes);
  const int Tp = (T + 16 + 7) / 8 * 8;
  const dim3 grid(ceil_div(T, 64), D, B);
  hipLaunchKernelGGL((bn2d_tile_kernel<true>), grid, dim3(256), 0, (hipStream_t)stream, Y, dA, B, D, T, Tp, lens_dev, mean, var, gamma, beta,
                     (const float*)dbeta, (const float*)dgamma, eps, 1.0f / ((float)B * D * T), dy_f32, (nbf16*)dy_pad, (nbf16*)dy_nhwc, part);
  DS2_LAUNCH_CHECK("bn2d_tile_kernel<bwd>");
  const long long nparts = (long long)grid.x * grid.y * grid.z;
  double* tmp = reinterpret_cast<double*>(reinterpret_cast<char*>(part) + align_up((size_t)nparts * 32 * sizeof(float), 16));
  const long long rpb = (nparts + CPF_BLOCKS - 1) / CPF_BLOCKS;
  const int nblk = (int)((nparts + rpb - 1) / rpb);
  hipLaunchKernelGGL(chan_part_finalize_kernel, dim3(nblk), dim3(256), 0, (hipStream_t)stream, (const float*)part, nparts, rpb, tmp, nblk, dbias, 0);
  hipLaunchKernelGGL(chan_part_finalize_kernel, dim3(1), dim3(256), 0, (hipStream_t)stream, (const float*)part, nparts, rpb, tmp, nblk, dbias, 1);
  DS2_LAUNCH_CHECK("chan_part_finalize_kernel");
  return 0;
}

extern "C" int ds2_transpose_bft_f32(const float* src, float* dst, int B, int F, int T, int dir, void* stream) {
  DS2_REQUIRE(src && dst && B > 0 && F > 0 && T > 0, "ds2_transpose_bft_f32: bad args");
  dim3 grid(ceil_div(T, 64), ceil_div(F, 64), B);
  hipLaunchKernelGGL(transpose_bft_kernel, grid, dim3(256), 0, (hipStream_t)stream, src, dst, B, F, T, dir);
  DS2_LAUNCH_CHECK("transpose_bft_kernel");
  return 0;
}

extern "C" int ds2_transpose2d_f32(const float* src, int ld_src, long long stride_src, float* dst, int ld_dst, long long stride_dst,
                                   int R, int Cc, int batch, void* stream) {
  DS2_REQUIRE(src && dst && R > 0 && Cc > 0 && batch > 0, "ds2_transpose2d_f32: bad args");
  dim3 grid(ceil_div(Cc, 32), ceil_div(R, 32), batch);
  hipLaunchKernelGGL(transpose2d_kernel, grid, dim3(256), 0, (hipStream_t)stream, src, ld_src, stride_src, dst, ld_dst, stride_dst, R, Cc);
  DS2_LAUNCH_CHECK("transpose2d_kernel");
  return 0;
}
```

### asr_amd/engine.py

```python
from __future__ import annotations

from dataclasses import dataclass, field
from typing import Dict, List, Optional

import torch

from . import _lib, ops

Tensor = torch.Tensor
import os as _os
def _tune(name: str, default: str) -> str:
    return _os.environ.get(name, default) if _os.environ.get("DS2_EXPERIMENTAL") == "1" else default


OVERLAP_MODE = _tune("DS2_OVERLAP", "2")
OVERLAP_WGRAD = OVERLAP_MODE == "1"
WGRAD_TN = _tune("DS2_WGRAD_TN", "1") != "0"
CONV_STATS = _tune("DS2_CONV_STATS", "1") != "0"
FUSE_BN_BWD = _tune("DS2_FUSE_BN_BWD", "1") != "0"
WGRAD_SIDE = _tune("DS2_WGRAD_SIDE", "sk")
WGRAD_IDLE = _tune("DS2_WGRAD_IDLE", "1") != "0"
WGRAD_IDLE_MIN_CUS = int(_tune("DS2_WGRAD_IDLE_MIN_CUS", "64"))
F32_GEMM = _os.environ.get("DS2_F32_GEMM", "split")

# ... 522 lines not shown
    done("fc")
    if deferred:
        serial = getattr(getattr(on_bucket, "__self__", None), "mode", None) == "serial"
        dy = _backward_rnn_deferred(W, Gr, cfg, ctx, dy, done, on_bucket is not None, serial)
        first_layer = -1
    else:
        first_layer = L - 1
    defer = idle_f32 and not OVERLAP_WGRAD
    pending_off = None
    for l in range(first_layer, -1, -1):
        lc = ctx.layers[l]
        bf = cfg.precision == "bf16"
        split = (not bf) and lc.xs is not None
        bfd = bf and B % 8 == 0
        gshape = lc.gx.shape if lc.gx is not None else lc.gshape
        dgx_bf = torch.empty(gshape, dtype=torch.bfloat16, device=dy.device) if bfd else None
        rmode = 1 if bf else (2 if (F32_RNN == "split" and H % 32 == 0) else 0)
        ops.rnn_bwd(G, dy, lc.gx, lc.aux, lc.hbuf, lc.wpb, lens_dev, T, B, H, bf16=rmode, dgx_bf16=dgx_bf, gates_bf16=lc.rec)
        if not bf:
            _BWD_PERSISTENT[f32_key] = bool(ops.rnn_last_path(dy.device) & 2)
        if pending_off is not None:
            fn, ev, pl = pending_off
            pending_off = None
            fn(after=ev)
            with torch.cuda.stream(side):
                done(f"rnns.{pl}")
        lc.rec = None
        dgx = dgx_bf if bfd else lc.gx
        dgxT = dgs = dbih_sum = None
        if bfd:
            dxn = ops.gemm_bf16_nt(dgx_bf, (lc.wihT if lc.wihT is not None else ops.cast_transpose_bf16(W[f"rnns.{l}.wih_cat"])))
            dgxT, dbih_sum = ops.transpose_bf16(dgx_bf, colsum=Gr[f"rnns.{l}.bih_cat"].view(-1))
        elif bf:
            dgx_r, dgxT, dbih_sum = ops.cast_bf16_both(dgx, colsum=True)
            dxn = ops.gemm_bf16_nt(dgx_r, (lc.wihT if lc.wihT is not None else ops.cast_transpose_bf16(W[f"rnns.{l}.wih_cat"])))
            del dgx_r
        elif split:
            dgs = ops.split_bf16(dgx, 0, pad_rows=64)
            wT = ops.transpose_batched(W[f"rnns.{l}.wih_cat"].unsqueeze(0))[0]
            dxn = ops.gemm_bf16_nt(dgs[:M], ops.split_bf16(wT, 1))
            del wT
        else:
            dxn = ops.gemm(dgx, W[f"rnns.{l}.wih_cat"])
        def off_path(l=l, lc=lc, dgx=dgx, dgs=dgs, dgxT=dgxT, dbih_sum=dbih_sum, bf=bf, bfd=bfd, split=split, after=None):
            if after is not None:
                side.wait_event(after)
            else:
                side.wait_stream(main)
            keep.append((dgx, lc.aux, lc.hbuf, lc.xn))
            with torch.cuda.stream(side):
                dbih = Gr[f"rnns.{l}.bih_cat"]
                if not bfd:
                    dbih.copy_(dbih_sum if bf else ops.colsum(dgx))
                dbhh = Gr[f"rnns.{l}.bhh_cat"]
                dbhh.copy_(dbih.view(2, G * H))
                auxT = None
                if G == 3 and T > 1 and bfd:
                    dbn = torch.empty(2 * H, dtype=torch.float32, device=dgx.device)
                    auxT = ops.cast_transpose_bf16(lc.aux, colsum=dbn)
                    dbhh[:, 2 * H:] = dbn.view(2, H)
                elif G == 3:
                    dbhh[:, 2 * H:] = ops.colsum(lc.aux).view(2, H)
                dwhh = Gr[f"rnns.{l}.whh_cat"]
                if T > 1 and bfd:
                    hT = ops.cast_transpose_bf16(lc.hbuf)
                    rows = 2 * H if G == 3 else G * H
                    ka = (slice(B, M), slice(0, M - B))
                    kb = (slice(0, M - B), slice(B, M))
                    ops.gemm_bf16_nt_pair(dgxT[0:rows, ka[0]], dgxT[G * H:G * H + rows, ka[1]], hT[0:H, kb[0]], hT[H:2 * H, kb[1]], dwhh[:, :rows])
                    if G == 3:
                        ops.gemm_bf16_nt_pair(auxT[0:H, ka[0]], auxT[H:2 * H, ka[1]], hT[0:H, kb[0]], hT[H:2 * H, kb[1]], dwhh[:, 2 * H:])
                    keep.append((dgxT, hT, auxT))
                elif T > 1 and split:
                    C2, Iw = 2 * G * H, W[f"rnns.{l}.wih_cat"].shape[1]
                    Ip = lc.xs.shape[1] // 3
                    hs = ops.split_bf16(lc.hbuf, 2)
                    d_hi, d_lo, h_hi, h_lo = dgs[:, :C2], dgs[:, 2 * C2:], hs[:, :2 * H], hs[:, 2 * H:]
                    rows = 2 * H if G == 3 else G * H
                    ra, rb = (slice(B, M), slice(0, M - B)), (slice(0, M - B), slice(B, M))
                    probs = []
                    for d in (0, 1):
                        for a, b in ((d_hi, h_hi), (d_hi, h_lo), (d_lo, h_hi)):
                            probs.append((a[ra[d], d * G * H:d * G * H + rows], b[rb[d], d * H:(d + 1) * H], dwhh[d, :rows]))
                    if G == 3:
                        axs = ops.split_bf16(lc.aux, 2)
                        a_hi, a_lo = axs[:, :2 * H], axs[:, 2 * H:]
                        for d in (0, 1):
                            for a, b in ((a_hi, h_hi), (a_hi, h_lo), (a_lo, h_hi)):
                                probs.append((a[ra[d], d * H:(d + 1) * H], b[rb[d], d * H:(d + 1) * H], dwhh[d, 2 * H:]))
                        keep.append((axs,))
                    x_hi, x_lo = lc.xs[:, :Iw], lc.xs[:, 2 * Ip:2 * Ip + Iw]
                    for a, b in ((d_hi, x_hi), (d_hi, x_lo), (d_lo, x_hi)):
                        probs.append((a, b, Gr[f"rnns.{l}.wih_cat"]))
                    if len(probs) <= 16 and Iw % 8 == 0:
                        ops.gemm_bf16_tn_splitk_group(probs)
                    else:
                        seen = set()
                        for a, b, o in probs:
                            ops.gemm_bf16_tn(a, b, out=o, accumulate=o.data_ptr() in seen)
                            seen.add(o.data_ptr())
                    keep.append((hs, dgs, lc.xs))
                elif T > 1:
                    K = (T - 1) * B
                    ldg, ldh = 2 * G * H, 2 * H
                    a0 = dgx.data_ptr() + 4 * (B * ldg)
                    b0 = lc.hbuf.data_ptr()
                    a1 = dgx.data_ptr() + 4 * (G * H)
                    b1 = lc.hbuf.data_ptr() + 4 * (H + B * ldh)
                    sA, sB = (a1 - a0) // 4, (b1 - b0) // 4
                    rows = 2 * H if G == 3 else G * H
                    ops.gemm_raw(True, False, rows, H, K, a0, ldg, sA, b0, ldh, sB, dwhh.data_ptr(), H, G * H * H, dgx.device, batch=2)
                    if G == 3:
                        x0 = lc.aux.data_ptr() + 4 * (B * ldh)
                        x1 = lc.aux.data_ptr() + 4 * H
                        ops.gemm_raw(True, False, H, H, K, x0, ldh, (x1 - x0) // 4, b0, ldh, sB, dwhh.data_ptr() + 4 * (2 * H * H), H,
                                     G * H * H, dgx.device, batch=2)
                else:
                    dwhh.zero_()
                if bf:
                    xnT = ops.transpose_bf16(lc.xn[:, :W[f"rnns.{l}.wih_cat"].shape[1]])
                    ops.gemm_bf16_nt(dgxT, xnT, out=Gr[f"rnns.{l}.wih_cat"])
                    keep.append((dgxT, xnT))
                elif split and T > 1:
                    pass
                elif split:
                    C2, I = 2 * G * H, W[f"rnns.{l}.wih_cat"].shape[1]
                    Ip = lc.xs.shape[1] // 3
                    for k, (a, b) in enumerate(((dgs[:, :C2], lc.xs[:, :I]), (dgs[:, :C2], lc.xs[:, 2 * Ip:2 * Ip + I]), (dgs[:, 2 * C2:], lc.xs[:, :I]))):
                        ops.gemm_bf16_tn(a, b, out=Gr[f"rnns.{l}.wih_cat"], accumulate=k > 0)
                    keep.append((dgs, lc.xs))
                else:
                    ops.gemm(dgx, lc.xn, transA=True, out=Gr[f"rnns.{l}.wih_cat"])
            lc.gx = lc.aux = lc.hbuf = lc.xn = lc.wpb = lc.xs = lc.wihT = None
        if not defer:
            off_path()
        if l > 0:
            bp = f"rnns.{l}.batch_norm.module."
            dy = ops.bn1d_bwd(dxn, lc.xin, lc.mean, lc.var, W[bp + "weight"], Gr[bp + "weight"], Gr[bp + "bias"])
        else:
            dy = dxn
        del dxn
        if defer and l > 0:
            ev = torch.cuda.Event()
            ev.record(main)
            pending_off = (off_path, ev, l)
            continue
        if defer:
            off_path()
        if side is not main:
            side.wait_stream(main)
        with torch.cuda.stream(side):
            done(f"rnns.{l}")
    cp = "conv.seq_module."
    da2 = ops.transpose_bft(dy, B, 32 * D2, T, to_tbf=False).view(B, 32, D2, T)
    m2, v2 = ctx.st2
    bf = cfg.precision == "bf16"
    if bf:
        _, dy2p, dy2n = ops.bn2d_act_bwd_fused(ctx.y2, da2, lens_dev, m2, v2, W[cp + "4.weight"], W[cp + "4.bias"], Gr[cp + "4.weight"],
                                               Gr[cp + "4.bias"], Gr[cp + "3.bias"], want_pad=CONV2_WGRAD != "nhwc", want_nhwc=True)
        del da2
        if CONV2_WGRAD == "nhwc":
            ops.conv2_wgrad_nhwc_bf16(ctx.a1p, dy2n, lens_dev, Gr[cp + "3.weight"])
        else:
            ops.conv2_wgrad_bf16(ctx.a1p, dy2p, lens_dev, Gr[cp + "3.weight"], T)
        da1 = ops.conv2_dgrad_bf16(dy2n, ctx.packs[1], ctx.packs[2], D1)
        del dy2p, dy2n
        m1, v1 = ctx.st1
        dy1, _, _ = ops.bn2d_act_bwd_fused(ctx.y1, da1, lens_dev, m1, v1, W[cp + "1.weight"], W[cp + "1.bias"], Gr[cp + "1.weight"],
                                           Gr[cp + "1.bias"], Gr[cp + "0.bias"], want_f32=True)
        del da1
        ops.conv1_wgrad_bf16(ctx.x16t, dy1, lens_dev, Gr[cp + "0.weight"], ctx.x.shape[3])
        ctx.x16t = None
    elif F32_CONV == "split":
        dy2, dy2p, dy2n = ops.bn2d_act_bwd_fused(ctx.y2, da2, lens_dev, m2, v2, W[cp + "4.weight"], W[cp + "4.bias"], Gr[cp + "4.weight"],
                                                 Gr[cp + "4.bias"], Gr[cp + "3.bias"], want_f32=True, want_pad=True, want_nhwc=True)
        del da2
        r2 = ops.bf16_residual(dy2)
        del dy2
        dy2p_lo, dy2n_lo = ops.padcast_bf16(r2), ops.nhwc_bf16(r2)
        r2 = ops.bf16_residual(ctx.a1)
        a1p = (ops.padcast_bf16(ctx.a1), ops.padcast_bf16(r2))
        del r2
        ph = ops.conv2_pack_bf16(W[cp + "3.weight"])
        pl = ops.conv2_pack_bf16(ops.bf16_residual(W[cp + "3.weight"]))
        g2 = Gr[cp + "3.weight"]
        gb, gc = torch.empty_like(g2), torch.empty_like(g2)
        ops.conv2_wgrad_bf16(a1p[0], dy2p, lens_dev, g2, T)
        ops.conv2_wgrad_bf16(a1p[1], dy2p, lens_dev, gb, T)
        ops.conv2_wgrad_bf16(a1p[0], dy2p_lo, lens_dev, gc, T)
        ops.sum3_(g2, gb, gc)
        del a1p
        wd0, wd1, wl0, wl1 = ph[1], ph[2], pl[1], pl[2]
        da1 = ops.conv2_dgrad_bf16(dy2n, wd0, wd1, D1)
        ops.sum3_(da1, ops.conv2_dgrad_bf16(dy2n_lo, wd0, wd1, D1), ops.conv2_dgrad_bf16(dy2n, wl0, wl1, D1))
        del dy2p, dy2n, dy2p_lo, dy2n_lo
        m1, v1 = ctx.st1
        dy1 = ops.bn2d_act_bwd(ctx.y1, da1, lens_dev, m1, v1, W[cp + "1.weight"], W[cp + "1.bias"], Gr[cp + "1.weight"], Gr[cp + "1.bias"])
        del da1
        Gr[cp + "0.bias"].copy_(ops.chan_sum(dy1))
        ops.conv1_wgrad(ctx.x, dy1, lens_dev, Gr[cp + "0.weight"])
    else:
        dy2 = ops.bn2d_act_bwd(ctx.y2, da2, lens_dev, m2, v2, W[cp + "4.weight"], W[cp + "4.bias"], Gr[cp + "4.weight"], Gr[cp + "4.bias"])
        del da2
        Gr[cp + "3.bias"].copy_(ops.chan_sum(dy2))
        ops.conv2_wgrad(ctx.a1, dy2, lens_dev, Gr[cp + "3.weight"])
        da1 = ops.conv2_dgrad(dy2, ctx.packs[0], D1)
        del dy2
        m1, v1 = ctx.st1
        dy1 = ops.bn2d_act_bwd(ctx.y1, da1, lens_dev, m1, v1, W[cp + "1.weight"], W[cp + "1.bias"], Gr[cp + "1.weight"], Gr[cp + "1.bias"])
        del da1
        Gr[cp + "0.bias"].copy_(ops.chan_sum(dy1))
        ops.conv1_wgrad(ctx.x, dy1, lens_dev, Gr[cp + "0.weight"])
    done("conv")
    if side is not main:
        main.wait_stream(side)
    if getattr(ctx, "side_used", False):
        main.wait_stream(_side_stream(dlogits.device))
    keep.clear()
```

### asr_amd/ops.py

```python
from __future__ import annotations

import ctypes as C
import math
import threading
from typing import Optional, Tuple

import numpy as np
import torch

from . import _lib

Tensor = torch.Tensor
BN_EPS = 1e-5
BN_MOMENTUM = 0.1


def _ptr(t: Optional[Tensor]):
    return None if t is None else t.data_ptr()


def _stream():
    return torch.cuda.current_stream().cuda_stream


# ... 467 lines not shown
    if out is None:
        both = torch.empty(2, H, dtype=torch.float32, device=dY.device)
        out = (both[0], both[1])
    s0, s1 = out
    _chk_f32(s0, s1)
    assert s0.is_contiguous() and s1.is_contiguous() and s0.numel() == H == s1.numel()
    wsb = lib.ds2_colreduce_workspace_bytes(M, H)
    ws = _ws(wsb, dY.device)
    _lib.check(lib.ds2_bn1d_bwd_xbf16(dY.data_ptr(), _row_pitch(dY), X.data_ptr(), X.stride(0), None, 0, M, H, mean.data_ptr(), var.data_ptr(),
                                      gamma.data_ptr(), BN_EPS, s1.data_ptr(), s0.data_ptr(), ws.data_ptr(), wsb, _stream()), "ds2_bn1d_bwd_xbf16")
    return s0, s1


def bn1d_bwd_xbf(dY: Tensor, X: Tensor, mean: Tensor, var: Tensor, gamma: Tensor, dgamma: Tensor, dbeta: Tensor) -> Tensor:
    _chk_f32(dY, mean, var, gamma, dgamma, dbeta)
    assert X.dtype == torch.bfloat16 and X.is_cuda and X.stride(1) == 1
    lib = _lib.load()
    M, H = dY.shape
    dX = torch.empty(M, H, dtype=torch.float32, device=dY.device)
    wsb = lib.ds2_colreduce_workspace_bytes(M, H)
    ws = _ws(wsb, dY.device)
    _lib.check(lib.ds2_bn1d_bwd_xbf16(dY.data_ptr(), _row_pitch(dY), X.data_ptr(), X.stride(0), dX.data_ptr(), H, M, H, mean.data_ptr(), var.data_ptr(),
                                      gamma.data_ptr(), BN_EPS, dgamma.data_ptr(), dbeta.data_ptr(), ws.data_ptr(), wsb, _stream()), "ds2_bn1d_bwd_xbf16")
    return dX


def colsum(X: Tensor) -> Tensor:
    _chk_f32(X)
    lib = _lib.load()
    M, H = X.shape
    s = torch.empty(H, dtype=torch.float32, device=X.device)
    s2 = torch.empty_like(s)
    wsb = lib.ds2_colreduce_workspace_bytes(M, H)
    ws = _ws(wsb, X.device)
    _lib.check(lib.ds2_colsum_f32(X.data_ptr(), _row_pitch(X), M, H, s.data_ptr(), s2.data_ptr(), ws.data_ptr(), wsb, _stream()),
               "ds2_colsum_f32")
    return s


def bn1d_apply(X: Tensor, mean: Tensor, var: Tensor, gamma: Tensor, beta: Tensor) -> Tensor:
    _chk_f32(X, mean, var, gamma, beta)
    M, H = X.shape
    Y = torch.empty(M, H, dtype=torch.float32, device=X.device)
    _lib.check(_lib.load().ds2_bn1d_apply_f32(X.data_ptr(), _row_pitch(X), Y.data_ptr(), H, M, H, mean.data_ptr(), var.data_ptr(),
                                              gamma.data_ptr(), beta.data_ptr(), BN_EPS, _stream()), "ds2_bn1d_apply_f32")
    return Y


def bn1d_apply_bf16(X: Tensor, mean: Tensor, var: Tensor, gamma: Tensor, beta: Tensor) -> Tensor:
    _chk_f32(X, mean, var, gamma, beta)
    M, H = X.shape
    Y = torch.empty(M, _pad8(H), dtype=torch.bfloat16, device=X.device)
    _lib.check(_lib.load().ds2_bn1d_apply_bf16(X.data_ptr(), _row_pitch(X), Y.data_ptr(), Y.size(1), M, H, mean.data_ptr(), var.data_ptr(),
                                               gamma.data_ptr(), beta.data_ptr(), BN_EPS, _stream()), "ds2_bn1d_apply_bf16")
    return Y


def bn1d_bwd(dY: Tensor, X: Tensor, mean: Tensor, var: Tensor, gamma: Tensor, dgamma: Tensor, dbeta: Tensor,
             dX: Optional[Tensor] = None) -> Tensor:
    _chk_f32(dY, X, mean, var, gamma, dgamma, dbeta, dX)
    lib = _lib.load()
    M, H = X.shape
    if dX is None:
        dX = torch.empty(M, H, dtype=torch.float32, device=X.device)
    wsb = lib.ds2_colreduce_workspace_bytes(M, H)
    ws = _ws(wsb, X.device)
    _lib.check(lib.ds2_bn1d_bwd_f32(dY.data_ptr(), _row_pitch(dY), X.data_ptr(), _row_pitch(X), dX.data_ptr(), _row_pitch(dX), M, H,
                                    mean.data_ptr(), var.data_ptr(), gamma.data_ptr(), BN_EPS, dgamma.data_ptr(), dbeta.data_ptr(),
                                    ws.data_ptr(), wsb, _stream()), "ds2_bn1d_bwd_f32")
    return dX


def bn2d_stats(Y: Tensor, run_mean: Optional[Tensor] = None, run_var: Optional[Tensor] = None):
    _chk_f32(Y, run_mean, run_var)
    lib = _lib.load()
    B, Cc, D, T = Y.shape
    mean = torch.empty(Cc, dtype=torch.float32, device=Y.device)
    var = torch.empty_like(mean)
    wsb = lib.ds2_chanreduce_workspace_bytes(Cc)
    ws = _ws(wsb, Y.device)
    _lib.check(lib.ds2_bn2d_stats_f32(Y.data_ptr(), B, Cc, D, T, mean.data_ptr(), var.data_ptr(), _ptr(run_mean), _ptr(run_var),
                                      BN_MOMENTUM, ws.data_ptr(), wsb, _stream()), "ds2_bn2d_stats_f32")
    return mean, var


def bn2d_act_fwd(Y: Tensor, lens_dev: Tensor, mean, var, gamma, beta) -> Tensor:
    _chk_f32(Y, mean, var, gamma, beta)
    B, Cc, D, T = Y.shape
    A = torch.empty_like(Y)
    _lib.check(_lib.load().ds2_bn2d_act_fwd_f32(Y.data_ptr(), A.data_ptr(), B, Cc, D, T, lens_dev.data_ptr(), mean.data_ptr(),
                                                var.data_ptr(), gamma.data_ptr(), beta.data_ptr(), BN_EPS, _stream()),
               "ds2_bn2d_act_fwd_f32")
    return A


def bn2d_act_bwd(Y: Tensor, dA: Tensor, lens_dev: Tensor, mean, var, gamma, beta, dgamma: Tensor, dbeta: Tensor) -> Tensor:
    _chk_f32(Y, dA, mean, var, gamma, beta, dgamma, dbeta)
    lib = _lib.load()
    B, Cc, D, T = Y.shape
    dY = torch.empty_like(Y)
    wsb = lib.ds2_chanreduce_workspace_bytes(Cc)
    ws = _ws(wsb, Y.device)
    _lib.check(lib.ds2_bn2d_act_bwd_f32(Y.data_ptr(), dA.data_ptr(), dY.data_ptr(), B, Cc, D, T, lens_dev.data_ptr(), mean.data_ptr(),
                                        var.data_ptr(), gamma.data_ptr(), beta.data_ptr(), BN_EPS, dgamma.data_ptr(), dbeta.data_ptr(),
                                        ws.data_ptr(), wsb, _stream()), "ds2_bn2d_act_bwd_f32")
    return dY


def bn2d_act_fwd_fused(Y: Tensor, lens_dev: Tensor, mean, var, gamma, beta, want_f32=False, want_pad=False, want_nhwc=False):
    _chk_f32(Y, mean, var, gamma, beta)
    lib = _lib.load()
    B, Cc, D, T = Y.shape
    assert Cc == 32 and Y.is_contiguous() and (want_f32 or want_pad or want_nhwc)
    a32 = torch.empty_like(Y) if want_f32 else None
    apad = torch.empty(B, 32, D, lib.ds2_conv_padded_pitch(T), dtype=torch.bfloat16, device=Y.device) if want_pad else None
    anh = torch.empty(B, D, T, 32, dtype=torch.bfloat16, device=Y.device) if want_nhwc else None
    _lib.check(lib.ds2_bn2d_act_fwd_fused(Y.data_ptr(), B, D, T, lens_dev.data_ptr(), mean.data_ptr(), var.data_ptr(), gamma.data_ptr(),
                                          beta.data_ptr(), BN_EPS, _ptr(a32), _ptr(apad), _ptr(anh), _stream()), "ds2_bn2d_act_fwd_fused")
    return a32, apad, anh


def bn2d_act_collapse(Y: Tensor, lens_dev: Tensor, mean, var, gamma, beta, want_f32=False, want_bf16=True, pad_to: int = 8):
    _chk_f32(Y, mean, var, gamma, beta)
    B, Cc, D, T = Y.shape
    assert Cc == 32 and Y.is_contiguous() and (want_f32 or want_bf16)
    F = 32 * D
    x32 = torch.empty(T * B, F, dtype=torch.float32, device=Y.device) if want_f32 else None
    xbf = None
    if want_bf16:
        xbf = torch.empty(T * B, -(-F // pad_to) * pad_to, dtype=torch.bfloat16, device=Y.device)
    _lib.check(_lib.load().ds2_bn2d_act_collapse(Y.data_ptr(), B, D, T, lens_dev.data_ptr(), mean.data_ptr(), var.data_ptr(), gamma.data_ptr(),
                                                 beta.data_ptr(), BN_EPS, _ptr(x32), _ptr(xbf), xbf.size(1) if xbf is not None else 0, _stream()),
               "ds2_bn2d_act_collapse")
    return x32, xbf


def bn2d_act_bwd_fused(Y: Tensor, dA: Tensor, lens_dev: Tensor, mean, var, gamma, beta, dgamma: Tensor, dbeta: Tensor, dbias: Tensor,
                       want_f32=False, want_pad=False, want_nhwc=False):
    _chk_f32(Y, dA, mean, var, gamma, beta, dgamma, dbeta, dbias)
    lib = _lib.load()
    B, Cc, D, T = Y.shape
    assert Cc == 32 and Y.is_contiguous() and dA.is_contiguous() and dA.shape == Y.shape
    d32 = torch.empty_like(Y) if want_f32 else None
    dpad = torch.empty(B, 32, D, lib.ds2_conv_padded_pitch(T), dtype=torch.bfloat16, device=Y.device) if want_pad else None
    dnh = torch.empty(B, D, T, 32, dtype=torch.bfloat16, device=Y.device) if want_nhwc else None
    wsb = lib.ds2_bn2d_act_bwd_fused_workspace_bytes(B, D, T)
    ws = _ws(wsb, Y.device)
    _lib.check(lib.ds2_bn2d_act_bwd_fused(Y.data_ptr(), dA.data_ptr(), B, D, T, lens_dev.data_ptr(), mean.data_ptr(), var.data_ptr(),
                                          gamma.data_ptr(), beta.data_ptr(), BN_EPS, dgamma.data_ptr(), dbeta.data_ptr(), dbias.data_ptr(),
                                          _ptr(d32), _ptr(dpad), _ptr(dnh), ws.data_ptr(), wsb, _stream()), "ds2_bn2d_act_bwd_fused")
    return d32, dpad, dnh


def chan_sum(Y: Tensor) -> Tensor:
    mean, _ = bn2d_stats(Y)
    B, Cc, D, T = Y.shape
    return mean * float(B * D * T)


def transpose_bft(src: Tensor, B: int, F: int, T: int, to_tbf: bool) -> Tensor:
    _chk_f32(src)
    dst = torch.empty((T, B, F) if to_tbf else (B, F, T), dtype=torch.float32, device=src.device)
    _lib.check(_lib.load().ds2_transpose_bft_f32(src.data_ptr(), dst.data_ptr(), B, F, T, 0 if to_tbf else 1, _stream()),
               "ds2_transpose_bft_f32")
    return dst


def transpose_batched(src: Tensor) -> Tensor:
    _chk_f32(src)
    nb, R, Cc = src.shape
    dst = torch.empty(nb, Cc, R, dtype=torch.float32, device=src.device)
    _lib.check(_lib.load().ds2_transpose2d_f32(src.data_ptr(), Cc, R * Cc, dst.data_ptr(), R, R * Cc, R, Cc, nb, _stream()),
               "ds2_transpose2d_f32")
    return dst


def conv_pack(w1: Tensor, w2: Tensor):
    _chk_f32(w1, w2)
    lib = _lib.load()
    dev = w1.device
    wpk1 = torch.empty(lib.ds2_conv_packed_floats(0), dtype=torch.float32, device=dev)
    wpk2 = torch.empty(lib.ds2_conv_packed_floats(1), dtype=torch.float32, device=dev)
    wpk2d = torch.empty(lib.ds2_conv_packed_floats(2), dtype=torch.float32, device=dev)
    _lib.check(lib.ds2_conv_pack_f32(w1.data_ptr(), w2.data_ptr(), wpk1.data_ptr(), wpk2.data_ptr(), wpk2d.data_ptr(), _stream()),
               "ds2_conv_pack_f32")
    return wpk1, wpk2, wpk2d


def conv1_fwd(x: Tensor, wpk1: Tensor, bias: Tensor, lens_dev: Tensor) -> Tensor:
    _chk_f32(x, wpk1, bias)
    B, _, F, Tin = x.shape
    D1, D2, T = _lib.conv_dims(F, Tin)
    y1 = torch.empty(B, 32, D1, T, dtype=torch.float32, device=x.device)
    _lib.check(_lib.load().ds2_conv1_fwd_f32(x.data_ptr(), wpk1.data_ptr(), bias.data_ptr(), lens_dev.data_ptr(), y1.data_ptr(), B, F,
                                             Tin, _stream()), "ds2_conv1_fwd_f32")
    return y1


def conv2_fwd(a1: Tensor, wpk2: Tensor, bias: Tensor, lens_dev: Tensor) -> Tensor:
    _chk_f32(a1, wpk2, bias)
    B, _, D1, T = a1.shape
    D2 = (D1 + 20 - 21) // 2 + 1
    y2 = torch.empty(B, 32, D2, T, dtype=torch.float32, device=a1.device)
    _lib.check(_lib.load().ds2_conv2_fwd_f32(a1.data_ptr(), wpk2.data_ptr(), bias.data_ptr(), lens_dev.data_ptr(), y2.data_ptr(), B, D1,
                                             T, _stream()), "ds2_conv2_fwd_f32")
    return y2


def conv2_dgrad(dy2: Tensor, wpk2d: Tensor, D1: int) -> Tensor:
    _chk_f32(dy2, wpk2d)
    B, _, D2, T = dy2.shape
    da1 = torch.empty(B, 32, D1, T, dtype=torch.float32, device=dy2.device)
    _lib.check(_lib.load().ds2_conv2_dgrad_f32(dy2.data_ptr(), wpk2d.data_ptr(), da1.data_ptr(), B, D1, T, _stream()),
               "ds2_conv2_dgrad_f32")
    return da1


def conv1_wgrad(x: Tensor, dy1: Tensor, lens_dev: Tensor, dW1: Tensor):
    _chk_f32(x, dy1, dW1)
    lib = _lib.load()
    B, _, F, Tin = x.shape
    wsb = lib.ds2_conv_wgrad_workspace_bytes(0, B, F)
    ws = _ws(wsb, x.device)
    _lib.check(lib.ds2_conv1_wgrad_f32(x.data_ptr(), dy1.data_ptr(), lens_dev.data_ptr(), dW1.data_ptr(), B, F, Tin, 0, ws.data_ptr(),
                                       wsb, _stream()), "ds2_conv1_wgrad_f32")


def conv2_wgrad(a1: Tensor, dy2: Tensor, lens_dev: Tensor, dW2: Tensor):
    _chk_f32(a1, dy2, dW2)
    lib = _lib.load()
    B, _, D1, T = a1.shape
    wsb = lib.ds2_conv_wgrad_workspace_bytes(1, B, 161)
    ws = _ws(wsb, a1.device)
    _lib.check(lib.ds2_conv2_wgrad_f32(a1.data_ptr(), dy2.data_ptr(), lens_dev.data_ptr(), dW2.data_ptr(), B, D1, T, 0, ws.data_ptr(),
                                       wsb, _stream()), "ds2_conv2_wgrad_f32")


def conv1_pack_bf16(w1: Tensor) -> Tensor:
    _chk_f32(w1)
    lib = _lib.load()
    wp = torch.empty(lib.ds2_conv1_bf16_bytes(0, 0, 0, 0), dtype=torch.uint8, device=w1.device)
    _lib.check(lib.ds2_conv1_pack_bf16(w1.data_ptr(), wp.data_ptr(), _stream()), "ds2_conv1_pack_bf16")
    return wp


def conv1_gather_bf16(x: Tensor, want_fwd: bool = True, want_wgrad: bool = True):
    _chk_f32(x)
    assert x.is_contiguous()
    lib = _lib.load()
    B, _, F, Tin = x.shape
    _, _, T = _lib.conv_dims(F, Tin)
    XB = torch.empty(lib.ds2_conv1_bf16_bytes(1, B, F, T) // 2, dtype=torch.bfloat16, device=x.device).view(B, F, lib.ds2_conv1_bf16_row_pitch(T)) if want_fwd else None
    X16T = torch.empty(lib.ds2_conv1_bf16_bytes(2, B, F, T) // 2, dtype=torch.bfloat16, device=x.device).view(B, F, 16, -1) if want_wgrad else None
    _lib.check(lib.ds2_conv1_gather_bf16(x.data_ptr(), _ptr(XB), _ptr(X16T), B, F, Tin, _stream()), "ds2_conv1_gather_bf16")
    return XB, X16T


def conv1_fwd_bf16(XB: Tensor, wp: Tensor, bias: Tensor, lens_dev: Tensor, Tin: int, stats: bool = False):
    B, F, P = XB.shape
    D1, _, T = _lib.conv_dims(F, Tin)
    lib = _lib.load()
    assert P == lib.ds2_conv1_bf16_row_pitch(T) and XB.is_contiguous()
    y1 = torch.empty(B, 32, D1, T, dtype=torch.float32, device=XB.device)
    part = torch.empty(lib.ds2_conv1_fwd_bf16_stat_blocks(B, F, Tin), 32, 2, dtype=torch.float32, device=XB.device) if stats else None
    _lib.check(lib.ds2_conv1_fwd_bf16_stats(XB.data_ptr(), wp.data_ptr(), bias.data_ptr(), lens_dev.data_ptr(), y1.data_ptr(), B, F, Tin,
                                            _ptr(part), _stream()), "ds2_conv1_fwd_bf16")
    return (y1, part) if stats else y1


def chanstats_from_partials(part: Tensor, count: int, run_mean: Optional[Tensor] = None, run_var: Optional[Tensor] = None):
    _chk_f32(part, run_mean, run_var)
    nblk, Cc, _ = part.shape
    mean = torch.empty(Cc, dtype=torch.float32, device=part.device)
    var = torch.empty_like(mean)
    lib = _lib.load()
    wsb = lib.ds2_chanstats_from_partials_workspace_bytes()
    ws = _ws(wsb, part.device)
    _lib.check(lib.ds2_chanstats_from_partials(part.data_ptr(), nblk, Cc, float(count), mean.data_ptr(), var.data_ptr(), _ptr(run_mean),
                                               _ptr(run_var), BN_MOMENTUM, ws.data_ptr(), wsb, _stream()), "ds2_chanstats_from_partials")
    return mean, var


def conv1_wgrad_bf16(X16T: Tensor, dy1: Tensor, lens_dev: Tensor, dW1: Tensor, Tin: int):
    _chk_f32(dy1, dW1)
    lib = _lib.load()
    B, F = X16T.shape[0], X16T.shape[1]
    wsb = lib.ds2_conv1_wgrad_bf16_workspace_bytes(B, Tin)
    ws = _ws(wsb, dy1.device)
    _lib.check(lib.ds2_conv1_wgrad_bf16(X16T.data_ptr(), dy1.data_ptr(), lens_dev.data_ptr(), dW1.data_ptr(), B, F, Tin, ws.data_ptr(), wsb,
                                        _stream()), "ds2_conv1_wgrad_bf16")


def conv2_pack_bf16(w2: Tensor):
    _chk_f32(w2)
    lib = _lib.load()
    bufs = [torch.empty(lib.ds2_conv2_bf16_packed_bytes(i), dtype=torch.uint8, device=w2.device) for i in range(3)]
    _lib.check(lib.ds2_conv2_pack_bf16(w2.data_ptr(), bufs[0].data_ptr(), bufs[1].data_ptr(), bufs[2].data_ptr(), _stream()),
               "ds2_conv2_pack_bf16")
    return tuple(bufs)


def nhwc_bf16(x: Tensor) -> Tensor:
    _chk_f32(x)
    B, Cc, D, T = x.shape
    assert Cc == 32 and x.is_contiguous()
    out = torch.empty(B, D, T, 32, dtype=torch.bfloat16, device=x.device)
    _lib.check(_lib.load().ds2_nhwc_bf16_f32(x.data_ptr(), out.data_ptr(), B, D, T, _stream()), "ds2_nhwc_bf16_f32")
    return out


def bf16_residual(x: Tensor) -> Tensor:
    _chk_f32(x)
    assert x.is_contiguous()
    r = torch.empty_like(x)
    _lib.check(_lib.load().ds2_bf16_residual_f32(x.data_ptr(), r.data_ptr(), x.numel(), _stream()), "ds2_bf16_residual_f32")
    return r


def sum3_(a: Tensor, b: Tensor, c: Optional[Tensor] = None) -> Tensor:
    _chk_f32(a, b) if c is None else _chk_f32(a, b, c)
    assert a.is_contiguous() and b.is_contiguous() and a.shape == b.shape and (c is None or (c.is_contiguous() and c.shape == a.shape))
    _lib.check(_lib.load().ds2_sum3_f32(a.data_ptr(), b.data_ptr(), _ptr(c), a.data_ptr(), a.numel(), _stream()), "ds2_sum3_f32")
    return a


def conv2_fwd_bf16(a1_nhwc: Tensor, wf: Tensor, bias: Tensor, lens_dev: Tensor, stats: bool = False):
    B, D1, T, _ = a1_nhwc.shape
    D2 = (D1 + 20 - 21) // 2 + 1
    lib = _lib.load()
    y2 = torch.empty(B, 32, D2, T, dtype=torch.float32, device=a1_nhwc.device)
    part = torch.empty(lib.ds2_conv2_fwd_bf16_stat_blocks(B, D1, T), 32, 2, dtype=torch.float32, device=a1_nhwc.device) if stats else None
    _lib.check(lib.ds2_conv2_fwd_bf16_stats(a1_nhwc.data_ptr(), wf.data_ptr(), bias.data_ptr(), lens_dev.data_ptr(), y2.data_ptr(), B, D1, T,
                                            _ptr(part), _stream()), "ds2_conv2_fwd_bf16")
    return (y2, part) if stats else y2


def conv2_dgrad_bf16(dy2_nhwc: Tensor, wd0: Tensor, wd1: Tensor, D1: int) -> Tensor:
    B, D2, T, _ = dy2_nhwc.shape
    da1 = torch.empty(B, 32, D1, T, dtype=torch.float32, device=dy2_nhwc.device)
    _lib.check(_lib.load().ds2_conv2_dgrad_bf16(dy2_nhwc.data_ptr(), wd0.data_ptr(), wd1.data_ptr(), da1.data_ptr(), B, D1, T, _stream()),
               "ds2_conv2_dgrad_bf16")
    return da1


def padcast_bf16(x: Tensor) -> Tensor:
    _chk_f32(x)
    assert x.is_contiguous()
    lib = _lib.load()
    B, Cc, D, T = x.shape
    Tp = lib.ds2_conv_padded_pitch(T)
    out = torch.empty(B, Cc, D, Tp, dtype=torch.bfloat16, device=x.device)
    _lib.check(lib.ds2_padcast_bf16(x.data_ptr(), out.data_ptr(), B * Cc * D, T, _stream()), "ds2_padcast_bf16")
    return out


def conv2_wgrad_bf16(a1p: Tensor, dy2p: Tensor, lens_dev: Tensor, dW2: Tensor, T: int):
    lib = _lib.load()
    B, _, D1, _ = a1p.shape
    wsb = lib.ds2_conv2_wgrad_bf16_workspace_bytes(B, D1)
    ws = _ws(wsb, a1p.device)
    _lib.check(lib.ds2_conv2_wgrad_bf16(a1p.data_ptr(), dy2p.data_ptr(), lens_dev.data_ptr(), dW2.data_ptr(), B, D1, T, ws.data_ptr(), wsb,
                                        _stream()), "ds2_conv2_wgrad_bf16")


def conv2_wgrad_nhwc_bf16(a1n: Tensor, dy2n: Tensor, lens_dev: Tensor, dW2: Tensor):
    lib = _lib.load()
    B, D1, T, _ = a1n.shape
    assert a1n.dtype == torch.bfloat16 and dy2n.dtype == torch.bfloat16 and a1n.is_contiguous() and dy2n.is_contiguous() and dy2n.shape[2] == T
    wsb = lib.ds2_conv2_wgrad_bf16_workspace_bytes(B, D1)
    ws = _ws(wsb, a1n.device)
    _lib.check(lib.ds2_conv2_wgrad_nhwc_bf16(a1n.data_ptr(), dy2n.data_ptr(), lens_dev.data_ptr(), dW2.data_ptr(), B, D1, T, ws.data_ptr(), wsb,
                                             _stream()), "ds2_conv2_wgrad_nhwc_bf16")


def rnn_pack(gates: int, whh: Tensor, bf16=False):
    _chk_f32(whh)
    assert whh.is_contiguous() and whh.dim() == 3
    lib = _lib.load()
    H = whh.size(2)
    wpf = torch.empty(lib.ds2_rnn_packed_bytes(gates, H, 0, int(bf16)), dtype=torch.uint8, device=whh.device)
    wpb = torch.empty(lib.ds2_rnn_packed_bytes(gates, H, 1, int(bf16)), dtype=torch.uint8, device=whh.device)
    _lib.check(lib.ds2_rnn_pack_whh(gates, whh.data_ptr(), wpf.data_ptr(), wpb.data_ptr(), H, int(bf16), _stream()), "ds2_rnn_pack_whh")
    return wpf, wpb


def weight_prep_bf16(layers):
    lib = _lib.load()
    tab = (_lib.PrepLayer * len(layers))()
    out = []
    for e, (gates, whh, wih, ld_r) in zip(tab, layers):
        wpf = wpb = wt = wr = None
        if whh is not None:
            _chk_f32(whh)
            assert whh.is_contiguous() and whh.dim() == 3
            dev, H = whh.device, whh.size(2)
            wpf = torch.empty(lib.ds2_rnn_packed_bytes(gates, H, 0, 1), dtype=torch.uint8, device=dev)
            wpb = torch.empty(lib.ds2_rnn_packed_bytes(gates, H, 1, 1), dtype=torch.uint8, device=dev)
            e.whh, e.wp_fwd, e.wp_bwd, e.gates, e.H = whh.data_ptr(), wpf.data_ptr(), wpb.data_ptr(), gates, H
        if wih is not None:
            _chk_f32(wih)
            R, Cc = wih.shape
            wt = torch.empty(Cc, _pad8(R), dtype=torch.bfloat16, device=wih.device)
            e.wih, e.wih_t, e.R, e.Cc, e.ld_wih, e.ld_t = wih.data_ptr(), wt.data_ptr(), R, Cc, _row_pitch(wih), wt.size(1)
            if ld_r is not None:
                assert ld_r >= Cc and ld_r % 8 == 0
                wr = torch.empty(R, ld_r, dtype=torch.bfloat16, device=wih.device)
                e.wih_r, e.ld_r = wr.data_ptr(), ld_r
        out.append((wpf, wpb, wt, wr))
    _lib.check(lib.ds2_weight_prep_bf16(tab, len(layers), _stream()), "ds2_weight_prep_bf16")
    return out


def rnn_ws(kind: str, gates: int, B: int, H: int, bf16, device) -> Tensor:
    lib = _lib.load()
    n = lib.ds2_rnn_fwd_workspace_bytes(B, H, int(bf16)) if kind == "fwd" else lib.ds2_rnn_bwd_workspace_bytes(gates, B, H, int(bf16))
    ws = _ws(n, device)
    _lib.check(lib.ds2_memset_async(ws.data_ptr(), 0xff, ws.numel(), _stream()), "ds2_memset_async")
    return ws


def _take_ws(ws: Optional[Tensor], need: int, device):
    if ws is None:
        return _ws(need, device), False
    assert ws.numel() >= need and ws.device == torch.device(device)
    return ws, True


def _rnn_call(device, armed: bool, thunk):
    ctx = rnn_ctx(device)
    ctx.ws_prearmed = 1 if armed else 0
    try:
        return thunk()
    finally:
        ctx.ws_prearmed = 0


def rnn_persistent_enable(forward: bool = True, backward: bool = True, device=None) -> None:
    _lib.check(_lib.load().ds2_rnn_persistent_enable(_ctxp(device), int(bool(forward)), int(bool(backward))), "ds2_rnn_persistent_enable")


def rnn_persistent_check(device=None) -> None:
    rec = (C.c_int * 8)()
    _lib.check(_lib.load().ds2_rnn_persistent_status(_ctxp(device), C.cast(rec, C.c_void_p)), "ds2_rnn_persistent_status")
    if rec[0]:
        starved, left = rnn_persistent_counters(device)
        what = {1: "forward", 2: "backward", 3: "census (launch never resident)"}.get(rec[0], str(rec[0]))
        raise _lib.DS2LibraryError(
            f"persistent recurrence starved ({what}): ids ({rec[1]}, {rec[2]}, {rec[3]}) step {rec[4]} wave {rec[5]} pending chunks {rec[6] & 0xffffffff:08x} "
            f"(L2-local exchange: {rec[7]}); the results of that step are invalid.  The next {left if left >= 0 else 'ALL'} recurrence calls run on the "
            f"one-launch-per-step kernels, then the persistent kernels are armed again (DS2_RNN_REARM_CALLS; DS2_RNN_PERSISTENT=0 selects the step "
            f"kernels from the start).  Starved launches since load: {starved}.")


def rnn_poison_if_starved(buf: Tensor) -> None:
    _chk_f32(buf)
    assert buf.is_contiguous()
    _lib.check(_lib.load().ds2_rnn_poison_if_starved(_ctxp(buf.device), buf.data_ptr(), buf.numel(), _stream()), "ds2_rnn_poison_if_starved")


def rnn_poison_seen(device=None) -> bool:
    return bool(_lib.load().ds2_rnn_poison_seen(_ctxp(device)))


def rnn_persistent_counters(device=None):
    out = (C.c_int * 2)()
    _lib.check(_lib.load().ds2_rnn_persistent_counters(_ctxp(device), C.cast(out, C.c_void_p)), "ds2_rnn_persistent_counters")
    return int(out[0]), int(out[1])


def rnn_fwd(gates: int, gx: Tensor, wp_fwd: Tensor, bhh: Tensor, lens_dev: Tensor, T: int, B: int, H: int, bf16=False,
            packed_gates: bool = False, h_bf16: Optional[Tensor] = None, hsum: Optional[Tensor] = None, ws: Optional[Tensor] = None):
    _chk_f32(bhh, hsum)
    assert gx.is_contiguous() and bhh.is_contiguous()
    if h_bf16 is not None:
        assert h_bf16.dtype == torch.bfloat16 and h_bf16.is_contiguous() and h_bf16.numel() == T * B * 2 * H
    lib = _lib.load()
    hbuf = torch.empty(T * B, 2 * H, dtype=torch.float32, device=gx.device)
    aux = torch.empty_like(hbuf) if gates != 1 else None
    rec = torch.empty(T * B, 2 * H, 4, dtype=torch.bfloat16, device=gx.device) if (packed_gates and gates != 1) else None
    wsb = lib.ds2_rnn_fwd_workspace_bytes(B, H, int(bf16))
    ws, armed = _take_ws(ws, wsb, gx.device)
    if gx.dtype == torch.bfloat16 or hsum is not None:
        assert int(bf16) == 1 and packed_gates, "rnn_fwd: bf16 x-projections / hsum belong to the bf16 training mode with packed gate records"
        gxb = gx if gx.dtype == torch.bfloat16 else None
        gxf = None if gxb is not None else gx
        for _attempt in (0, 1):
            rc = _rnn_call(gx.device, armed and _attempt == 0, lambda: lib.ds2_rnn_fwd_x(
                _ctxp(gx.device), gates, _ptr(gxf), _ptr(gxb), wp_fwd.data_ptr(), bhh.data_ptr(), hbuf.data_ptr(), _ptr(aux),
                lens_dev.data_ptr(), T, B, H, _ptr(rec), _ptr(h_bf16), _ptr(hsum), ws.data_ptr(), wsb, _stream()))
            if rc != 1:
                break
            gxf, gxb = widen_bf16(gxb), None
        _lib.check(rc, "ds2_rnn_fwd_x")
        return hbuf, aux, rec
# ... 847 lines not shown
```

### include/ds2hip.h

```cpp
#ifndef DS2HIP_H
#define DS2HIP_H

#include <stddef.h>
#include <stdint.h>

#ifdef __cplusplus
extern "C" {
#endif

const char* ds2_version(void);
const char* ds2_last_error(void);
int ds2_device_info(int* cu_count, int* wave_size, char* arch, int arch_len);
int ds2_ablation_build(void);

typedef struct ds2_rnn_ctx {
  int size;
  int persist_fwd, persist_bwd;
  int cooldown;
  int rearm_calls;
  int starved_total;
  int last_path;
  int last_bwd_kind;
  int debug_flags;
  int ws_prearmed;
  int reserved[6];
  int* status_dev;
  int* poison_host;
  int* poison_dev;
} ds2_rnn_ctx;
int ds2_rnn_ctx_init(ds2_rnn_ctx* ctx, int* status_dev, int* poison_host, int* poison_dev);
int ds2_memset_async(void* dst, int value, size_t bytes, void* stream);
int ds2_debug_flags(ds2_rnn_ctx* ctx, int flags);

size_t ds2_gemm_f32_workspace_bytes(int M, int N, int batch, int splitk);
int ds2_gemm_f32(int transA, int transB, int M, int N, int K, const float* A, int lda, long long strideA, const float* B, int ldb,
                 long long strideB, float* C, int ldc, long long strideC, const float* bias, int accumulate, int batch, int splitk,
                 void* workspace, size_t workspace_bytes, void* stream);

size_t ds2_gemm_bf16_workspace_bytes(int M, int N, int batch, int splitk);
int ds2_gemm_bf16_nt(int M, int N, int K, const void* A, int lda, long long strideA, const void* B, int ldb, long long strideB, float* C,
                     int ldc, long long strideC, const float* bias, int accumulate, int batch, int splitk, void* workspace,
                     size_t workspace_bytes, void* stream);
int ds2_gemm_bf16_nt_obf16(int M, int N, int K, const void* A, int lda, const void* B, int ldb, void* C, int ldc, const float* bias, void* stream);
int ds2_cast_f32_from_bf16(const void* src, float* dst, long long n, void* stream);
int ds2_gemm_bf16_tn(int M, int N, int K, const void* A, int lda, long long strideA, const void* B, int ldb, long long strideB, float* C,
                     int ldc, long long strideC, int accumulate, int batch, int splitk, void* workspace, size_t workspace_bytes,
                     void* stream);
typedef struct ds2_tn_problem {
  const void* A; const void* B; float* C;
  int M, N, K, lda, ldb, ldc;
} ds2_tn_problem;
int ds2_gemm_bf16_tn_group(int nprob, const ds2_tn_problem* problems, int max_workgroups, void* stream);
size_t ds2_gemm_bf16_tn_splitk_group_workspace_bytes(int nprob, const ds2_tn_problem* problems, int splitk);
int ds2_gemm_bf16_tn_splitk_group(int nprob, const ds2_tn_problem* problems, int splitk, void* workspace, size_t workspace_bytes, void* stream);
int ds2_gemm_bf16_tn_splitk_group_ep(int nprob, const ds2_tn_problem* probs, int splitk, int ep_index, const float* ep_scale, const float* ep_rowv,
                                     const float* ep_shift, void* workspace, size_t workspace_bytes, void* stream);
int ds2_cast_bf16(const float* src, int ld_src, void* dst, int ld_dst, int R, int Cc, void* stream);
int ds2_split_bf16(const float* src, int ld_src, void* dst, int ld_dst, int R, int Cc, int order, void* stream);
int ds2_cast_transpose_bf16(const float* src, int ld_src, void* dst, int ld_dst, int R, int Cc, void* stream);
size_t ds2_cast_bf16_both_workspace_bytes(int R, int Cc);
int ds2_cast_bf16_both(const float* src, int ld_src, void* dst_r, int ld_r, void* dst_t, int ld_t, int R, int Cc, float* colsum, void* ws,
                       size_t ws_bytes, void* stream);
int ds2_transpose_bf16(const void* src, int ld_src, void* dst_t, int ld_t, int R, int Cc, float* colsum, void* ws, size_t ws_bytes,
                       void* stream);

size_t ds2_colreduce_workspace_bytes(int M, int H);
int ds2_colstats_f32(const float* X, int ldx, int M, int H, float* mean, float* var, float* run_mean, float* run_var, float momentum,
                     void* ws, size_t ws_bytes, void* stream);
int ds2_add_colstats_f32(const float* Xa, int lda, const float* Xb, int ldb, float* Y, int ldy, int M, int H, float* mean, float* var,
                         float* run_mean, float* run_var, float momentum, void* ws, size_t ws_bytes, void* stream);
int ds2_colsum_f32(const float* X, int ldx, int M, int H, float* sum, float* sumsq, void* ws, size_t ws_bytes, void* stream);
int ds2_bn1d_apply_f32(const float* X, int ldx, float* Y, int ldy, int M, int H, const float* mean, const float* var,
                       const float* gamma, const float* beta, float eps, void* stream);
int ds2_bn1d_apply_bf16(const float* X, int ldx, void* Y, int ldy, int M, int H, const float* mean, const float* var, const float* gamma,
                        const float* beta, float eps, void* stream);
int ds2_bn1d_bwd_f32(const float* dY, int lddy, const float* X, int ldx, float* dX, int lddx, int M, int H, const float* mean,
                     const float* var, const float* gamma, float eps, float* dgamma, float* dbeta, void* ws, size_t ws_bytes,
                     void* stream);

int ds2_center_colstats(const float* Xa, int lda, const float* Xb, int ldb, const float* hsum, int ntiles, void* Yc_bf16, int ldyc, int M, int H,
                        float* mean, float* var, float* delta, float* run_mean, float* run_var, float momentum, void* ws, size_t ws_bytes,
                        void* stream);
int ds2_wih_fold_bf16(const float* W, int ldw, const float* bias, int R, int I, const float* var, const float* gamma, const float* beta,
                      const float* delta, float eps, void* W2_bf16, int ldw2, float* bias2, float* colscale, float* colshift, void* stream);
int ds2_scale_rank1_f32(float* C, int ldc, int R, int N, const float* scale, const float* rowv, const float* shift, void* stream);
int ds2_bn1d_bwd_xbf16(const float* dY, int lddy, const void* X_bf16, int ldx, float* dX, int lddx, int M, int H, const float* mean, const float* var,
                       const float* gamma, float eps, float* dgamma, float* dbeta, void* ws, size_t ws_bytes, void* stream);

size_t ds2_chanreduce_workspace_bytes(int C);
int ds2_bn2d_stats_f32(const float* Y, int B, int C, int D, int T, float* mean, float* var, float* run_mean, float* run_var,
                       float momentum, void* ws, size_t ws_bytes, void* stream);
int ds2_bn2d_act_fwd_f32(const float* Y, float* A, int B, int C, int D, int T, const int* lens_dev, const float* mean,
                         const float* var, const float* gamma, const float* beta, float eps, void* stream);
int ds2_bn2d_act_bwd_f32(const float* Y, const float* dA, float* dY, int B, int C, int D, int T, const int* lens_dev, const float* mean,
                         const float* var, const float* gamma, const float* beta, float eps, float* dgamma, float* dbeta, void* ws,
                         size_t ws_bytes, void* stream);

int ds2_bn2d_act_fwd_fused(const float* Y, int B, int D, int T, const int* lens_dev, const float* mean, const float* var,
                           const float* gamma, const float* beta, float eps, float* a_f32, void* a_pad, void* a_nhwc, void* stream);
int ds2_bn2d_act_collapse(const float* Y, int B, int D, int T, const int* lens_dev, const float* mean, const float* var,
                          const float* gamma, const float* beta, float eps, float* x_f32, void* x_bf16, int ld_bf, void* stream);
size_t ds2_bn2d_act_bwd_fused_workspace_bytes(int B, int D, int T);
int ds2_bn2d_act_bwd_fused(const float* Y, const float* dA, int B, int D, int T, const int* lens_dev, const float* mean,
                           const float* var, const float* gamma, const float* beta, float eps, float* dgamma, float* dbeta,
                           float* dbias, float* dy_f32, void* dy_pad, void* dy_nhwc, void* ws, size_t ws_bytes, void* stream);
int ds2_transpose_bft_f32(const float* src, float* dst, int B, int F, int T, int dir, void* stream);
int ds2_transpose2d_f32(const float* src, int ld_src, long long stride_src, float* dst, int ld_dst, long long stride_dst, int R, int Cc,
                        int batch, void* stream);

void ds2_conv_dims(int F, int Tin, int* D1, int* D2, int* T);
size_t ds2_conv_packed_floats(int which );
int ds2_conv_pack_f32(const float* w1, const float* w2, float* wpk1, float* wpk2, float* wpk2d, void* stream);
int ds2_conv1_fwd_f32(const float* x, const float* wpk1, const float* bias, const int* lens_dev, float* y1, int B, int F, int Tin,
                      void* stream);
int ds2_conv2_fwd_f32(const float* a1, const float* wpk2, const float* bias, const int* lens_dev, float* y2, int B, int D1, int T,
                      void* stream);
int ds2_conv2_dgrad_f32(const float* dy2, const float* wpk2d, float* da1, int B, int D1, int T, void* stream);
size_t ds2_conv_wgrad_workspace_bytes(int which , int B, int F);
int ds2_conv1_wgrad_f32(const float* x, const float* dy1, const int* lens_dev, float* dW1, int B, int F, int Tin, int accumulate, void* ws,
                        size_t ws_bytes, void* stream);
int ds2_conv2_wgrad_f32(const float* a1, const float* dy2, const int* lens_dev, float* dW2, int B, int D1, int T, int accumulate, void* ws,
                        size_t ws_bytes, void* stream);

size_t ds2_conv2_bf16_packed_bytes(int which );
int ds2_conv2_pack_bf16(const float* w2, void* wf, void* wd0, void* wd1, void* stream);
int ds2_nhwc_bf16_f32(const float* src, void* dst, int B, int D, int T, void* stream);
int ds2_conv2_fwd_bf16(const void* a1_nhwc, const void* wf, const float* bias, const int* lens_dev, float* y2, int B, int D1, int T,
                       void* stream);
int ds2_conv2_fwd_bf16_stat_blocks(int B, int D1, int T);
int ds2_conv2_fwd_bf16_stats(const void* a1_nhwc, const void* wf, const float* bias, const int* lens_dev, float* y2, int B, int D1, int T,
                             float* stat_part, void* stream);
size_t ds2_chanstats_from_partials_workspace_bytes(void);
int ds2_chanstats_from_partials(const float* part, int nblk, int C, double count, float* mean, float* var, float* run_mean, float* run_var,
                                float momentum, void* ws, size_t ws_bytes, void* stream);
int ds2_conv2_dgrad_bf16(const void* dy2_nhwc, const void* wd0, const void* wd1, float* da1, int B, int D1, int T, void* stream);

int ds2_conv_padded_pitch(int T);
int ds2_padcast_bf16(const float* src, void* dst, long long R, int T, void* stream);
size_t ds2_conv2_wgrad_bf16_workspace_bytes(int B, int D1);
int ds2_conv2_wgrad_bf16(const void* a1p, const void* dy2p, const int* lens_dev, float* dW2, int B, int D1, int T, void* ws, size_t ws_bytes,
                         void* stream);
int ds2_conv2_wgrad_nhwc_bf16(const void* a1_nhwc, const void* dy2_nhwc, const int* lens_dev, float* dW2, int B, int D1, int T, void* ws,
                              size_t ws_bytes, void* stream);

size_t ds2_rnn_packed_bytes(int gates, int H, int which , int bf16);
int ds2_rnn_pack_whh(int gates, const float* whh, void* wp_fwd, void* wp_bwd, int H, int bf16, void* stream);
typedef struct ds2_prep_layer {
  const float* whh; void* wp_fwd; void* wp_bwd;
  const float* wih; void* wih_t; void* wih_r;
  int gates, H, R, Cc, ld_wih, ld_t, ld_r, reserved;
} ds2_prep_layer;
int ds2_weight_prep_bf16(const ds2_prep_layer* layers, int n, void* stream);
int ds2_rnn_persistent_status(ds2_rnn_ctx* ctx, int* out8);
int ds2_rnn_persistent_counters(const ds2_rnn_ctx* ctx, int* out2);
int ds2_rnn_poison_if_starved(ds2_rnn_ctx* ctx, float* buf, size_t n, void* stream);
int ds2_rnn_poison_seen(const ds2_rnn_ctx* ctx);
int ds2_rnn_step_gate(const ds2_rnn_ctx* ctx, const float* loss_dev, int* flag_dev, void* stream);
int ds2_rnn_persistent_enable(ds2_rnn_ctx* ctx, int forward, int backward);
int ds2_rnn_bwd_ksplit_footprint(int gates, int H, int* out3);
int ds2_rnn_last_path(const ds2_rnn_ctx* ctx);
size_t ds2_rnn_fwd_workspace_bytes(int B, int H, int bf16);
int ds2_rnn_fwd(ds2_rnn_ctx* ctx, int gates, float* gx, const void* wp_fwd, const float* bhh, float* hbuf, float* aux, const int* lens_dev, int T, int B,
                int H, int bf16, void* gates_bf16, void* ws, size_t ws_bytes, void* stream);
int ds2_rnn_fwd_ex(ds2_rnn_ctx* ctx, int gates, float* gx, const void* wp_fwd, const float* bhh, float* hbuf, float* aux, const int* lens_dev, int T, int B,
                   int H, int bf16, void* gates_bf16, void* h_bf16, void* ws, size_t ws_bytes, void* stream);
int ds2_rnn_fwd_x(ds2_rnn_ctx* ctx, int gates, float* gx, const void* gx_bf16, const void* wp_fwd, const float* bhh, float* hbuf, float* aux,
                  const int* lens_dev, int T, int B, int H, void* gates_bf16, void* h_bf16, float* hsum, void* ws, size_t ws_bytes, void* stream);
size_t ds2_rnn_bwd_workspace_bytes(int gates, int B, int H, int bf16);
int ds2_rnn_bwd(ds2_rnn_ctx* ctx, int gates, const float* dy, int lddy, float* gx, float* aux, const float* hbuf, const void* wp_bwd, const int* lens_dev,
                int T, int B, int H, int bf16, void* dgx_bf16, const void* gates_bf16, void* ws, size_t ws_bytes, void* stream);

int ds2_rnn_bwd_ex(ds2_rnn_ctx* ctx, int gates, const float* dy, int lddy, float* gx, float* aux, const float* hbuf, const void* wp_bwd, const int* lens_dev,
                   int T, int B, int H, int bf16, void* dgx_bf16, const void* gates_bf16, void* dhn_bf16, float* bias_part, void* ws,
                   size_t ws_bytes, void* stream);

int ds2_rnn_bwd_bn(ds2_rnn_ctx* ctx, int gates, const float* dyn, int lddyn, const float* bn_x, int ldx, const float* bn_mean, const float* bn_var,
                   const float* bn_gamma, const float* bn_s0, const float* bn_s1, float bn_eps, float* dy_scratch, float* gx, float* aux,
                   const float* hbuf, const void* wp_bwd, const int* lens_dev, int T, int B, int H, int bf16, void* dgx_bf16,
                   const void* gates_bf16, void* dhn_bf16, float* bias_part, void* ws, size_t ws_bytes, void* stream);

int ds2_rnn_bwd_bn_xbf16(ds2_rnn_ctx* ctx, int gates, const float* dyn, int lddyn, const void* bn_x_bf16, int ldx, const float* bn_mean,
                         const float* bn_var, const float* bn_gamma, const float* bn_s0, const float* bn_s1, float bn_eps, float* dy_scratch, float* gx,
                         float* aux, const float* hbuf, const void* wp_bwd, const int* lens_dev, int T, int B, int H, int bf16, void* dgx_bf16,
                         const void* gates_bf16, void* dhn_bf16, float* bias_part, void* ws, size_t ws_bytes, void* stream);

int ds2_rnn_bias_grads(int gates, const float* bias_part, int B, int H, float* dbih, float* dbhh, void* stream);

size_t ds2_ctc_workspace_bytes(int T, int B, int max_target_len);
int ds2_ctc_loss_f32(const float* logits, int ld, int T, int B, int C, const int* targets_dev, const int* tgt_off_dev,
                     const int* in_lens_dev, const int* tgt_lens_dev, int max_target_len, float* nll_dev, float* grad, int ldg,
                     float grad_scale, void* ws, size_t ws_bytes, void* stream);
int ds2_ctc_loss_ex_f32(const float* logits, int ld, int T, int B, int C, const int* targets_dev, const int* tgt_off_dev,
                        const int* in_lens_dev, const int* tgt_lens_dev, int max_target_len, float* nll_dev, float* grad, int ldg,
                        float grad_scale, int lattice, void* ws, size_t ws_bytes, void* stream);

size_t ds2_ctc_star_workspace_bytes(int T, int B, int max_target_len);
int ds2_ctc_star_loss_f32(const float* logits, int ld, int T, int B, int C, const int* targets_dev, const int* tgt_off_dev,
                          const int* in_lens_dev, const int* tgt_lens_dev, int max_target_len, float star_penalty, const int* flags_dev,
                          float* nll_dev, float* grad, int ldg, float grad_scale, int lattice, void* ws, size_t ws_bytes, void* stream);

size_t ds2_ctc_mwer_workspace_bytes(int T, int B, int K, int max_hyp_len);
int ds2_ctc_mwer_f32(const float* logits, int ld, int T, int B, int C, int K, const int* hyps_dev, const long long* hyp_off_dev,
                     const int* hyp_lens_dev, const int* hyp_valid_dev, const int* in_lens_dev, int max_hyp_len, const float* risk_dev,
                     float* loss_dev, float* nll_hyp_dev, float* post_dev, float* grad, int ldg, float grad_scale, int accumulate,
                     int lattice, void* ws, size_t ws_bytes, void* stream);

int ds2_ctc_conf_max_unit_labels(void);
size_t ds2_ctc_conf_workspace_bytes(int T, int B, int max_hyp_len);
int ds2_ctc_conf_f32(const float* logits, int ld, int T, int B, int C, const int* hyps_dev, const long long* hyp_off_dev,
                     const int* hyp_lens_dev, const int* in_lens_dev, int max_hyp_len, const int* n_units_dev, const int* unit_lo_dev,
                     const int* unit_hi_dev, const int* win_start_dev, const int* win_end_dev, int W_max, float* nll_dev,
                     float* logconf_dev, int lattice, void* ws, size_t ws_bytes, void* stream);

int ds2_ctc_batch_mean_f32(const float* nll_dev, int B, float* out_dev, void* stream);

size_t ds2_ctc_align_workspace_bytes(int B, int T, int max_target_len);
int ds2_ctc_align_f32(const float* x, long long ld_b, long long ld_t, int B, int T, int C, int is_log,
                      const int* targets_dev, const int* tgt_off_dev, const int* in_lens_dev, const int* tgt_lens_dev,
                      int max_target_len, int variant,
                      float* score, int* states, int* tok_start, int* tok_end, float* tok_logp,
                      void* ws, size_t ws_bytes, void* stream);

size_t ds2_ctc_align_tiled_workspace_bytes(int B, int T, int max_target_len, int tile_frames, int tile_pairs);
int ds2_ctc_align_tiled_f32(const float* x, long long ld_b, long long ld_t, int B, int T, int C, int is_log,
                            const int* targets_dev, const int* tgt_off_dev, const int* in_lens_dev, const int* tgt_lens_dev,
                            int max_target_len, int tile_frames, int tile_pairs,
                            float* score, int* states, int* tok_start, int* tok_end, float* tok_logp,
                            void* ws, size_t ws_bytes, void* stream);

int ds2_ctc_align_star_row_f32(const float* x, long long ld_b, long long ld_t, int B, int T, int C, int is_log,
                               const int* in_lens_dev, float star_penalty, float* g, void* stream);
size_t ds2_ctc_align_star_workspace_bytes(int B, int T, int max_target_len);
int ds2_ctc_align_star_f32(const float* x, long long ld_b, long long ld_t, int B, int T, int C, int is_log,
                           const int* targets_dev, const int* tgt_off_dev, const int* in_lens_dev, const int* tgt_lens_dev,
                           int max_target_len, int variant, float star_penalty, const int* flags_dev,
                           float* score, int* states, int* tok_start, int* tok_end, float* tok_logp,
                           void* ws, size_t ws_bytes, void* stream);

size_t ds2_ctc_align_star_tiled_workspace_bytes(int B, int T, int max_target_len, int tile_frames, int tile_pairs);
int ds2_ctc_align_star_tiled_f32(const float* x, long long ld_b, long long ld_t, int B, int T, int C, int is_log,
                                 const int* targets_dev, const int* tgt_off_dev, const int* in_lens_dev, const int* tgt_lens_dev,
                                 int max_target_len, int tile_frames, int tile_pairs, float star_penalty, const int* flags_dev,
                                 float* score, int* states, int* tok_start, int* tok_end, float* tok_logp,
                                 void* ws, size_t ws_bytes, void* stream);

size_t ds2_ctc_kws_workspace_bytes(int B, int T, int K, int max_hits);
int ds2_ctc_kws_f32(const float* x, long long ld_b, long long ld_t, int B, int T, int C, int is_log, const int* in_lens_dev,
                    const int* kw_labels_dev, const int* kw_off_dev, const int* kw_lens_dev, int K, int max_kw_len,
                    const float* thr_dev, int max_hits,
                    float* frame_score, int* frame_start, int* hit_start, int* hit_end, float* hit_score, int* n_hits,
                    void* ws, size_t ws_bytes, void* stream);

int ds2_softmax_rows_f32(const float* x, int ldx, float* y, int ldy, int rows, int C, void* stream);

size_t ds2_greedy_decode_workspace_bytes(int B, int T);
int ds2_greedy_decode_f32(const float* probs, long long ld_b, long long ld_t, int B, int T, int C, const int* sizes_dev, int blank,
                          int* ids, int* offs, int* out_len, void* ws, size_t ws_bytes, void* stream);

int ds2_ctc_beam_max_width(void);
size_t ds2_ctc_beam_workspace_bytes(int B, int T, int beam_width);
int ds2_ctc_beam_decode_f32(const float* probs, long long ld_b, long long ld_t, int B, int T, int C, const int* sizes_dev, int blank,
                            int beam_width, int cutoff_top_n, float cutoff_prob, int* labels, int* offsets, int* lens, float* scores,
                            void* ws, size_t ws_bytes, void* stream);

int ds2_ctc_beam_lm_max_candidates(void);
size_t ds2_ctc_lm_packed_bytes(int order, int n_ngrams, int n_edges, int n_nodes, int C);
int ds2_ctc_lm_pack(int order, int n_ngrams, const int* ngram_tok, const int* ngram_n, const float* prob, const float* bow, int n_edges,
                    const int* edge_node, const int* edge_label, const int* edge_child, int n_nodes, const int* node_word, int C,
                    const int* label_tok, int bos, int mode, void* out, size_t out_bytes);
int ds2_ctc_lm_score(const void* packed, const int* hist, int n_hist, int w, float* out);
int ds2_ctc_beam_decode_lm_f32(const float* probs, long long ld_b, long long ld_t, int B, int T, int C, const int* sizes_dev, int blank,
                               int beam_width, int cutoff_top_n, float cutoff_prob, const void* lm_dev, size_t lm_bytes, int lm_order,
                               int lm_mode, int space, float alpha, float beta, int* labels, int* offsets, int* lens, float* scores,
                               void* ws, size_t ws_bytes, void* stream);

size_t ds2_ctc_hot_packed_bytes(int n_nodes, int n_edges);
int ds2_ctc_hot_pack(int n_nodes, int n_edges, const int* edge_node, const int* edge_label, const int* edge_child, const int* fail,
                     const float* phi, const int* terminal, int C, void* out, size_t out_bytes);
int ds2_ctc_hot_step(const void* packed, int node, int label, int* next, float* term);
int ds2_ctc_beam_decode_hot_f32(const float* probs, long long ld_b, long long ld_t, int B, int T, int C, const int* sizes_dev, int blank,
                                int beam_width, int cutoff_top_n, float cutoff_prob, const void* lm_dev, size_t lm_bytes, int lm_order,
                                int lm_mode, int space, float alpha, float beta, const void* hot_dev, const void* hot_host,
                                size_t hot_bytes, int* labels, int* offsets, int* lens, float* scores, void* ws, size_t ws_bytes,
                                void* stream);

size_t ds2_edit_distance_workspace_bytes(int P, long long max_len);
int ds2_edit_distance_i32(const int* seq, long long n_seq, const long long* a_off, const int* a_len, const long long* b_off,
                          const int* b_len, int P, long long max_len, int* dist, void* ws, size_t ws_bytes, void* stream);

// ... 74 lines not shown
```

Measured before the change: 2857.

## Fuse BN2d backward reductions into transpose and conv2 dgrad epilogues

Computes the BatchNorm2d backward channel sums (dbeta, dgamma) inside the producers of the gradient: the bft transpose kernel for the conv2 BN and the bf16 conv2 dgrad kernel epilogue for the conv1 BN. Per-block partials are then finalized with the existing chanstats partials kernel in a new sum-only mode. The downstream elementwise BN backward then uses the precomputed sums instead of doing its own reduction pass over Y and dA. The goal is to remove an extra full read of the large conv activations and gradients, at the cost of extra registers and a Y read in the dgrad epilogue, plus some additional small launches.

```diff
diff --git a/asr_amd/_lib.py b/asr_amd/_lib.py
--- a/asr_amd/_lib.py
+++ b/asr_amd/_lib.py
@@ -86,6 +86,14 @@
     "ds2_nhwc_bf16_f32": (i32, [vp, vp, i32, i32, i32, vp]),
     "ds2_conv2_fwd_bf16": (i32, [vp, vp, vp, vp, vp, i32, i32, i32, vp]),
     "ds2_conv2_dgrad_bf16": (i32, [vp, vp, vp, vp, i32, i32, i32, vp]),
+    "ds2_bn2d_bwd_sums_from_partials_workspace_bytes": (sz, []),
+    "ds2_bn2d_bwd_sums_from_partials": (i32, [vp, i32, vp, vp, vp, sz, vp]),
+    "ds2_conv2_dgrad_bf16_sums_workspace_bytes": (sz, [i32, i32, i32]),
+    "ds2_conv2_dgrad_bf16_sums": (i32, [vp, vp, vp, vp, i32, i32, i32, vp, vp, vp, vp, vp, vp, f32, vp, vp, vp, sz, vp]),
+    "ds2_transpose_bft_sums_workspace_bytes": (sz, [i32, i32, i32]),
+    "ds2_transpose_bft_sums": (i32, [vp, vp, i32, i32, i32, vp, vp, vp, vp, vp, vp, f32, vp, vp, vp, sz, vp]),
+    "ds2_bn2d_act_bwd_from_sums_workspace_bytes": (sz, [i32, i32, i32]),
+    "ds2_bn2d_act_bwd_from_sums": (i32, [vp, vp, i32, i32, i32, vp, vp, vp, vp, vp, f32, vp, vp, vp, vp, vp, vp, vp, sz, vp]),
     "ds2_conv_padded_pitch": (i32, [i32]),
     "ds2_padcast_bf16": (i32, [vp, vp, i64, i32, vp]),
     "ds2_conv2_wgrad_bf16_workspace_bytes": (sz, [i32, i32]),
diff --git a/asr_amd/csrc/conv_bf16.hip b/asr_amd/csrc/conv_bf16.hip
--- a/asr_amd/csrc/conv_bf16.hip
+++ b/asr_amd/csrc/conv_bf16.hip
@@ -22,13 +22,21 @@
   int gx, gy, gz;
 };
 
+struct BArgs {
+  const float* y;
+  const int* lens;
+  const float *mean, *var, *gamma, *beta;
+  float eps;
+  float* part;
+};
+
 constexpr int IN_CHUNKS = NPIX * 4;
 constexpr int IN_IT = (IN_CHUNKS + 255) / 256;
 constexpr int W_CHUNKS = WROW / 16;
 constexpr int W_IT = (W_CHUNKS + 255) / 256;
 
-template <int SD, int R>
-__global__ __launch_bounds__(256) void conv2_bf16_rows_kernel(CArgs a, int n_out, float* __restrict__ stat_part) {
+template <int SD, int R, bool BSUMS = false>
+__global__ __launch_bounds__(256) void conv2_bf16_rows_kernel(CArgs a, int n_out, float* __restrict__ stat_part, BArgs s) {
   constexpr int RING = (R - 1) * SD + 1;
   constexpr int SLOT = NPIX * IPITCH;
   __shared__ __attribute__((aligned(16))) char in_lds[RING * SLOT];
@@ -64,6 +72,26 @@
 #pragma unroll
     for (int r = 0; r < 16; ++r) acc[q][r] = 0.f;
 
+  __shared__ float bnc[BSUMS ? 4 : 1][32];
+  float yv[BSUMS ? R : 1][16];
+  int slen = 0;
+  if constexpr (BSUMS) {
+    if (tid < 128) {
+      const int c = tid & 31, k = tid >> 5;
+      bnc[k][c] = k == 0 ? s.mean[c] : k == 1 ? rsqrtf(s.var[c] + s.eps) : k == 2 ? s.gamma[c] : s.beta[c];
+    }
+    slen = min(s.lens[b], a.T);
+  }
+  auto load_y = [&]() {
+#pragma unroll
+    for (int q = 0; q < (BSUMS ? R : 0); ++q)
+#pragma unroll
+      for (int r = 0; r < 16; ++r) {
+        const int co = (r & 3) + 8 * (r >> 2) + 4 * half;
+        yv[q][r] = (t < slen && o0 + q < n_out) ? s.y[out_ptr(o0 + q, co) - a.out] : 0.f;
+      }
+  };
+
   const int f0 = SD * o0 - a.PD;
   f32x4 ri[IN_IT], rw[W_IT];
   auto load_in = [&](int f) {
@@ -111,7 +139,7 @@
   const int pix_off = (wave * 32 + l31) * IPITCH + half * 16;
   const char* abase = w_lds + half * (32 * 16) + l31 * 16;
   int slot0 = 0;
-  for (int kd = 0; kd < a.KD; ++kd) {
+  auto kernel_row = [&](int kd, bool last) {
     __syncthreads();
     {
       int snew = slot0 + RING - 1;
@@ -120,9 +148,11 @@
     }
     store_w();
     __syncthreads();
-    if (kd + 1 < a.KD) {
+    if (!last) {
       load_in(f0 + kd + RING);
       load_w(kd + 1);
+    } else if constexpr (BSUMS) {
+      load_y();
     }
     const char* bq[R];
 #pragma unroll
@@ -144,6 +174,56 @@
       }
     }
     slot0 = slot0 + 1 == RING ? 0 : slot0 + 1;
+  };
+  if constexpr (BSUMS) {
+    for (int kd = 0; kd + 1 < a.KD; ++kd) kernel_row(kd, false);
+    kernel_row(a.KD - 1, true);
+  } else {
+    for (int kd = 0; kd < a.KD; ++kd) kernel_row(kd, kd + 1 == a.KD);
+  }
+  if constexpr (BSUMS) {
+    const bool live = t < slen;
+    float sv[32];
+#pragma unroll
+    for (int r = 0; r < 16; ++r) {
+      const int co = (r & 3) + 8 * (r >> 2) + 4 * half;
+      const float mu = bnc[0][co], rs = bnc[1][co], ga = bnc[2][co], be = bnc[3][co];
+      sv[r] = 0.f; sv[16 + r] = 0.f;
+#pragma unroll
+      for (int q = 0; q < R; ++q)
+        if (o0 + q < n_out) {
+          const float v = acc[q][r];
+          if (t < a.T) *out_ptr(o0 + q, co) = v;
+          const float xh = (yv[q][r] - mu) * rs;
+          const float z = xh * ga + be;
+          const float dz = (live && z > 0.f && z < 20.f) ? v : 0.f;
+          sv[r] += dz;
+          sv[16 + r] += dz * xh;
+        }
+    }
+    __shared__ float bred[4][32][2];
+#define DS2_HALVE(N)                                                                               \
+    {                                                                                              \
+      const bool up = (l31 & N) != 0;      \
+      _Pragma("unroll") for (int i = 0; i < N; ++i) {                                              \
+        const float give = up ? sv[i] : sv[i + N], keep = up ? sv[i + N] : sv[i];                  \
+        sv[i] = keep + __shfl_xor(give, N);                                                        \
+      }                                                                                            \
+    }
+    DS2_HALVE(16) DS2_HALVE(8) DS2_HALVE(4) DS2_HALVE(2) DS2_HALVE(1)
+#undef DS2_HALVE
+    {
+      const int r = l31 & 15;
+      bred[wave][(r & 3) + 8 * (r >> 2) + 4 * half][l31 >> 4] = sv[0];
+    }
+    __syncthreads();
+    if (tid < 64) {
+      const int co = tid >> 1, w = tid & 1;
+      const float sum = ((bred[0][co][w] + bred[1][co][w]) + bred[2][co][w]) + bred[3][co][w];
+      const long long blk = ((long long)bz * a.gy + by) * a.gx + bx;
+      s.part[(blk * 32 + co) * 2 + w] = sum;
+    }
+    return;
   }
   float bv[16];
 #pragma unroll
@@ -254,7 +334,7 @@
   a.B = B; a.Din = D1; a.T = T; a.Dtot = D2; a.KD = 21; a.SD = 2; a.PD = 10; a.OS = 1; a.OO = 0;
   if (stat_part) DS2_HIP(hipMemsetAsync(stat_part, 0, (size_t)ds2_conv2_fwd_bf16_stat_blocks(B, D1, T) * 64 * sizeof(float), (hipStream_t)stream));
   a.gx = ceil_div(T, TT); a.gy = ceil_div(D2, 3); a.gz = B;
-  hipLaunchKernelGGL((conv2_bf16_rows_kernel<2, 3>), dim3(a.gx * a.gy * a.gz), dim3(256), 0, (hipStream_t)stream, a, D2, stat_part);
+  hipLaunchKernelGGL((conv2_bf16_rows_kernel<2, 3>), dim3(a.gx * a.gy * a.gz), dim3(256), 0, (hipStream_t)stream, a, D2, stat_part, BArgs{});
   DS2_LAUNCH_CHECK("conv2_bf16_rows_kernel fwd");
   return 0;
 }
@@ -264,8 +344,7 @@
   return ds2_conv2_fwd_bf16_stats(a1_nhwc, wf, bias, lens_dev, y2, B, D1, T, nullptr, stream);
 }
 
-extern "C" int ds2_conv2_dgrad_bf16(const void* dy2_nhwc, const void* wd0, const void* wd1, float* da1, int B, int D1, int T, void* stream) {
-  DS2_REQUIRE(dy2_nhwc && wd0 && wd1 && da1, "ds2_conv2_dgrad_bf16: null pointer");
+static int conv2_dgrad_launch(const void* dy2_nhwc, const void* wd0, const void* wd1, float* da1, int B, int D1, int T, BArgs sums, void* stream) {
   const int D2 = (D1 + 2 * 10 - 21) / 2 + 1;
   for (int p = 0; p < 2; ++p) {
     const int KDe = (21 - p + 1) / 2;
@@ -274,10 +353,42 @@
     a.in = (const __bf16*)dy2_nhwc; a.wpk = (const __bf16*)(p == 0 ? wd0 : wd1); a.bias = nullptr; a.out = da1; a.lens = nullptr;
     a.B = B; a.Din = D2; a.T = T; a.Dtot = D1; a.KD = KDe; a.SD = 1; a.PD = KDe - 6; a.OS = 2; a.OO = p;
     a.gx = ceil_div(T, TT); a.gy = ceil_div(n_o, 4); a.gz = B;
-    hipLaunchKernelGGL((conv2_bf16_rows_kernel<1, 4>), dim3(a.gx * a.gy * a.gz), dim3(256), 0, (hipStream_t)stream, a, n_o, (float*)nullptr);
+    if (a.gy == 0) continue;
+    if (sums.part) {
+      hipLaunchKernelGGL((conv2_bf16_rows_kernel<1, 4, true>), dim3(a.gx * a.gy * a.gz), dim3(256), 0, (hipStream_t)stream, a, n_o, (float*)nullptr, sums);
+      sums.part += (size_t)a.gx * a.gy * a.gz * 64;
+    } else {
+      hipLaunchKernelGGL((conv2_bf16_rows_kernel<1, 4>), dim3(a.gx * a.gy * a.gz), dim3(256), 0, (hipStream_t)stream, a, n_o, (float*)nullptr, BArgs{});
+    }
   }
   DS2_LAUNCH_CHECK("conv2_bf16_rows_kernel dgrad");
   return 0;
+}
+
+extern "C" int ds2_conv2_dgrad_bf16(const void* dy2_nhwc, const void* wd0, const void* wd1, float* da1, int B, int D1, int T, void* stream) {
+  DS2_REQUIRE(dy2_nhwc && wd0 && wd1 && da1, "ds2_conv2_dgrad_bf16: null pointer");
+  return conv2_dgrad_launch(dy2_nhwc, wd0, wd1, da1, B, D1, T, BArgs{}, stream);
+}
+
+static int conv2_dgrad_sum_slots(int B, int D1, int T) { return ceil_div(T, TT) * (ceil_div((D1 + 1) / 2, 4) + ceil_div(D1 / 2, 4)) * B; }
+
+extern "C" size_t ds2_conv2_dgrad_bf16_sums_workspace_bytes(int B, int D1, int T) {
+  return (size_t)conv2_dgrad_sum_slots(B, D1, T) * 64 * sizeof(float) + ds2_bn2d_bwd_sums_from_partials_workspace_bytes();
+}
+
+extern "C" int ds2_conv2_dgrad_bf16_sums(const void* dy2_nhwc, const void* wd0, const void* wd1, float* da1, int B, int D1, int T, const float* y1,
+                                         const int* lens_dev, const float* mean, const float* var, const float* gamma, const float* beta, float eps,
+                                         float* dgamma, float* dbeta, void* ws, size_t ws_bytes, void* stream) {
+  DS2_REQUIRE(dy2_nhwc && wd0 && wd1 && da1 && y1 && lens_dev && mean && var && gamma && beta && dgamma && dbeta,
+              "ds2_conv2_dgrad_bf16_sums: null pointer");
+  DS2_REQUIRE(B > 0 && D1 > 0 && T > 0, "ds2_conv2_dgrad_bf16_sums: bad shape B %d D1 %d T %d", B, D1, T);
+  DS2_REQUIRE(ws && ws_bytes >= ds2_conv2_dgrad_bf16_sums_workspace_bytes(B, D1, T), "ds2_conv2_dgrad_bf16_sums: workspace too small");
+  const int nslots = conv2_dgrad_sum_slots(B, D1, T);
+  BArgs sums{y1, lens_dev, mean, var, gamma, beta, eps, (float*)ws};
+  const int rc = conv2_dgrad_launch(dy2_nhwc, wd0, wd1, da1, B, D1, T, sums, stream);
+  if (rc) return rc;
+  char* fin = static_cast<char*>(ws) + (size_t)nslots * 64 * sizeof(float);
+  return ds2_bn2d_bwd_sums_from_partials((const float*)ws, nslots, dgamma, dbeta, fin, ws_bytes - (size_t)(fin - static_cast<char*>(ws)), stream);
 }
 
 namespace {
diff --git a/asr_amd/csrc/norm.hip b/asr_amd/csrc/norm.hip
--- a/asr_amd/csrc/norm.hip
+++ b/asr_amd/csrc/norm.hip
@@ -523,6 +523,74 @@
         else for (int j = 0; j < 4; ++j) if (t + j < T) dst[bft(f, t + j)] = o[j];
       }
     }
+  }
+}
+
+__global__ __launch_bounds__(256) void transpose_bft_sums_kernel(const float* __restrict__ src, float* __restrict__ dst, int Bn, int D, int T,
+                                                                 const float* __restrict__ Yraw, const int* __restrict__ lens,
+                                                                 const float* __restrict__ mean, const float* __restrict__ var,
+                                                                 const float* __restrict__ gamma, const float* __restrict__ beta, float eps,
+                                                                 float* __restrict__ part) {
+  typedef float f32x4u __attribute__((ext_vector_type(4), aligned(4)));
+  __shared__ float tile[64][65];
+  __shared__ float rowsum[64][2];
+  const int F = 32 * D;
+  const int b = blockIdx.z;
+  const int f0 = blockIdx.y * 64, t0 = blockIdx.x * 64;
+  const int q4 = (threadIdx.x & 15) * 4, r16 = threadIdx.x >> 4;
+  const int len = min(lens[b], T);
+#pragma unroll
+  for (int i = 0; i < 4; ++i) {
+    const int r = r16 + 16 * i;
+    float v[4] = {0.f, 0.f, 0.f, 0.f};
+    const int t = t0 + r, f = f0 + q4;
+    if (t < T) {
+      const float* p = src + ((long long)t * Bn + b) * F + f;
+      if (f + 3 < F) { const f32x4u q = *reinterpret_cast<const f32x4u*>(p); v[0] = q.x; v[1] = q.y; v[2] = q.z; v[3] = q.w; }
+      else for (int j = 0; j < 4; ++j) if (f + j < F) v[j] = p[j];
+    }
+#pragma unroll
+    for (int j = 0; j < 4; ++j) tile[r][q4 + j] = v[j];
+  }
+  __syncthreads();
+#pragma unroll
+  for (int i = 0; i < 4; ++i) {
+    const int r = r16 + 16 * i;
+    const f32x4u o = {tile[q4][r], tile[q4 + 1][r], tile[q4 + 2][r], tile[q4 + 3][r]};
+    const int f = f0 + r, t = t0 + q4;
+    float a0 = 0.f, a1 = 0.f;
+    if (f < F) {
+      const long long at = ((long long)b * F + f) * T + t;
+      if (t + 3 < T) *reinterpret_cast<f32x4u*>(dst + at) = o;
+      else for (int j = 0; j < 4; ++j) if (t + j < T) dst[at + j] = o[j];
+      if (t < len) {
+        const int c = f / D;
+        const float mu = mean[c], rs = rsqrtf(var[c] + eps), ga = gamma[c], be = beta[c];
+        float y[4] = {0.f, 0.f, 0.f, 0.f};
+        if (t + 3 < T) { const f32x4u q = *reinterpret_cast<const f32x4u*>(Yraw + at); y[0] = q.x; y[1] = q.y; y[2] = q.z; y[3] = q.w; }
+        else for (int j = 0; j < 4; ++j) if (t + j < T) y[j] = Yraw[at + j];
+#pragma unroll
+        for (int j = 0; j < 4; ++j) {
+          const float xh = (y[j] - mu) * rs;
+          const float z = xh * ga + be;
+          const float dz = (t + j < len && z > 0.f && z < 20.f) ? o[j] : 0.f;
+          a0 += dz;
+          a1 += dz * xh;
+        }
+      }
+    }
+#pragma unroll
+    for (int m = 1; m < 16; m <<= 1) { a0 += __shfl_xor(a0, m); a1 += __shfl_xor(a1, m); }
+    if ((threadIdx.x & 15) == 0) { rowsum[r][0] = a0; rowsum[r][1] = a1; }
+  }
+  __syncthreads();
+  if (threadIdx.x < 64) {
+    const int c = threadIdx.x >> 1, w = threadIdx.x & 1;
+    const int lo = max(c * D, f0) - f0, hi = min(min((c + 1) * D, F), f0 + 64) - f0;
+    double s = 0.0;
+    for (int k = lo; k < hi; ++k) s += (double)rowsum[k][w];
+    const long long blk = ((long long)blockIdx.z * gridDim.y + blockIdx.y) * gridDim.x + blockIdx.x;
+    part[blk * 64 + threadIdx.x] = (float)s;
   }
 }
 
@@ -907,7 +975,8 @@
 
 __global__ __launch_bounds__(256) void chanstats_partials_kernel(const float* __restrict__ part, int n, int rpb, double* __restrict__ tmp, int nblk,
                                                                  double count, float* __restrict__ mean, float* __restrict__ var,
-                                                                 float* __restrict__ run_mean, float* __restrict__ run_var, float momentum, int stage) {
+                                                                 float* __restrict__ run_mean, float* __restrict__ run_var, float momentum, int stage,
+                                                                 int kind) {
   __shared__ double red[4][64];
   const int c = threadIdx.x & 63, r = threadIdx.x >> 6;
   double s = 0.0;
@@ -933,7 +1002,10 @@
   }
   red[0][c] = t;
   __syncthreads();
-  if (c < 32) {
+  if (c < 32 && kind == 1) {
+    mean[c] = (float)red[0][2 * c];
+    var[c] = (float)red[0][2 * c + 1];
+  } else if (c < 32) {
     const double m = red[0][2 * c] / count;
     double v = red[0][2 * c + 1] / count - m * m;
     if (v < 0.0) v = 0.0;
@@ -956,15 +1028,31 @@
     constexpr int SB = 128;
     const int rpb = ceil_div(nblk, SB), nb = ceil_div(nblk, rpb);
     hipLaunchKernelGGL(chanstats_partials_kernel, dim3(nb), dim3(256), 0, (hipStream_t)stream, part, nblk, rpb, (double*)ws, nb, count, mean, var,
-                       run_mean, run_var, momentum, 0);
+                       run_mean, run_var, momentum, 0, 0);
     hipLaunchKernelGGL(chanstats_partials_kernel, dim3(1), dim3(256), 0, (hipStream_t)stream, part, nblk, rpb, (double*)ws, nb, count, mean, var,
-                       run_mean, run_var, momentum, 1);
+                       run_mean, run_var, momentum, 1, 0);
     DS2_LAUNCH_CHECK("chanstats_partials_kernel");
     return 0;
   }
   hipLaunchKernelGGL(col_finalize_kernel, dim3(ceil_div(C, 32)), dim3(256), 0, (hipStream_t)stream, part, nblk, C, count, 0, mean, var, run_mean,
                      run_var, momentum);
   DS2_LAUNCH_CHECK("col_finalize_kernel");
+  return 0;
+}
+
+extern "C" size_t ds2_bn2d_bwd_sums_from_partials_workspace_bytes(void) { return ds2_chanstats_from_partials_workspace_bytes(); }
+
+extern "C" int ds2_bn2d_bwd_sums_from_partials(const float* part, int nslots, float* dgamma, float* dbeta, void* ws, size_t ws_bytes, void* stream) {
+  DS2_REQUIRE(part && dgamma && dbeta, "ds2_bn2d_bwd_sums_from_partials: null pointer");
+  DS2_REQUIRE(nslots > 0, "ds2_bn2d_bwd_sums_from_partials: bad slot count %d", nslots);
+  DS2_REQUIRE(ws && ws_bytes >= ds2_bn2d_bwd_sums_from_partials_workspace_bytes(), "ds2_bn2d_bwd_sums_from_partials: workspace too small");
+  constexpr int SB = 128;
+  const int rpb = ceil_div(nslots, SB), nb = ceil_div(nslots, rpb);
+  hipLaunchKernelGGL(chanstats_partials_kernel, dim3(nb), dim3(256), 0, (hipStream_t)stream, part, nslots, rpb, (double*)ws, nb, 1.0, dbeta, dgamma,
+                     (float*)nullptr, (float*)nullptr, 0.f, 0, 1);
+  hipLaunchKernelGGL(chanstats_partials_kernel, dim3(1), dim3(256), 0, (hipStream_t)stream, part, nslots, rpb, (double*)ws, nb, 1.0, dbeta, dgamma,
+                     (float*)nullptr, (float*)nullptr, 0.f, 1, 1);
+  DS2_LAUNCH_CHECK("chanstats_partials_kernel");
   return 0;
 }
 
@@ -1025,6 +1113,9 @@
 }
 
 constexpr int CPF_BLOCKS = 128;
+static int bn2d_bwd_tile_launch(const float* Y, const float* dA, int B, int D, int T, const int* lens_dev, const float* mean, const float* var,
+                                const float* gamma, const float* beta, float eps, const float* dgamma, const float* dbeta, float* dbias,
+                                float* dy_f32, void* dy_pad, void* dy_nhwc, void* ws, void* stream);
 extern "C" size_t ds2_bn2d_act_bwd_fused_workspace_bytes(int B, int D, int T) {
   return ds2_chanreduce_workspace_bytes(32) + align_up((size_t)B * D * ceil_div(T, 64) * 32 * sizeof(float), 16) + (size_t)CPF_BLOCKS * 32 * sizeof(double);
 }
@@ -1038,7 +1129,28 @@
   int rc = chan_reduce_launch(1, Y, dA, B, 32, D, T, lens_dev, mean, var, gamma, beta, eps, 1, dbeta, dgamma, nullptr, nullptr, 0.f, ws,
                               red_bytes, (hipStream_t)stream);
   if (rc) return rc;
-  float* part = reinterpret_cast<float*>(static_cast<char*>(ws) + red_bytes);
+  return bn2d_bwd_tile_launch(Y, dA, B, D, T, lens_dev, mean, var, gamma, beta, eps, dgamma, dbeta, dbias, dy_f32, dy_pad, dy_nhwc,
+                              static_cast<char*>(ws) + red_bytes, stream);
+}
+
+extern "C" size_t ds2_bn2d_act_bwd_from_sums_workspace_bytes(int B, int D, int T) {
+  return align_up((size_t)B * D * ceil_div(T, 64) * 32 * sizeof(float), 16) + (size_t)CPF_BLOCKS * 32 * sizeof(double);
+}
+
+extern "C" int ds2_bn2d_act_bwd_from_sums(const float* Y, const float* dA, int B, int D, int T, const int* lens_dev, const float* mean,
+                                          const float* var, const float* gamma, const float* beta, float eps, const float* dgamma,
+                                          const float* dbeta, float* dbias, float* dy_f32, void* dy_pad, void* dy_nhwc, void* ws, size_t ws_bytes,
+                                          void* stream) {
+  DS2_REQUIRE(Y && dA && lens_dev && mean && var && gamma && beta && dgamma && dbeta && dbias, "ds2_bn2d_act_bwd_from_sums: null pointer");
+  DS2_REQUIRE(B > 0 && D > 0 && T > 0, "ds2_bn2d_act_bwd_from_sums: bad shape B %d D %d T %d", B, D, T);
+  DS2_REQUIRE(ws && ws_bytes >= ds2_bn2d_act_bwd_from_sums_workspace_bytes(B, D, T), "ds2_bn2d_act_bwd_from_sums: workspace too small");
+  return bn2d_bwd_tile_launch(Y, dA, B, D, T, lens_dev, mean, var, gamma, beta, eps, dgamma, dbeta, dbias, dy_f32, dy_pad, dy_nhwc, ws, stream);
+}
+
+static int bn2d_bwd_tile_launch(const float* Y, const float* dA, int B, int D, int T, const int* lens_dev, const float* mean, const float* var,
+                                const float* gamma, const float* beta, float eps, const float* dgamma, const float* dbeta, float* dbias,
+                                float* dy_f32, void* dy_pad, void* dy_nhwc, void* ws, void* stream) {
+  float* part = static_cast<float*>(ws);
   const int Tp = (T + 16 + 7) / 8 * 8;
   const dim3 grid(ceil_div(T, 64), D, B);
   hipLaunchKernelGGL((bn2d_tile_kernel<true>), grid, dim3(256), 0, (hipStream_t)stream, Y, dA, B, D, T, Tp, lens_dev, mean, var, gamma, beta,
@@ -1062,6 +1174,26 @@
   return 0;
 }
 
+extern "C" size_t ds2_transpose_bft_sums_workspace_bytes(int B, int D, int T) {
+  return (size_t)B * ceil_div(32 * D, 64) * ceil_div(T, 64) * 64 * sizeof(float) + ds2_bn2d_bwd_sums_from_partials_workspace_bytes();
+}
+
+extern "C" int ds2_transpose_bft_sums(const float* src, float* dst, int B, int D, int T, const float* Y, const int* lens_dev, const float* mean,
+                                      const float* var, const float* gamma, const float* beta, float eps, float* dgamma, float* dbeta, void* ws,
+                                      size_t ws_bytes, void* stream) {
+  DS2_REQUIRE(src && dst && Y && lens_dev && mean && var && gamma && beta && dgamma && dbeta, "ds2_transpose_bft_sums: null pointer");
+  DS2_REQUIRE(B > 0 && D > 0 && T > 0, "ds2_transpose_bft_sums: bad shape B %d D %d T %d", B, D, T);
+  DS2_REQUIRE(ws && ws_bytes >= ds2_transpose_bft_sums_workspace_bytes(B, D, T), "ds2_transpose_bft_sums: workspace too small");
+  const dim3 grid(ceil_div(T, 64), ceil_div(32 * D, 64), B);
+  float* part = static_cast<float*>(ws);
+  hipLaunchKernelGGL(transpose_bft_sums_kernel, grid, dim3(256), 0, (hipStream_t)stream, src, dst, B, D, T, Y, lens_dev, mean, var, gamma, beta, eps,
+                     part);
+  DS2_LAUNCH_CHECK("transpose_bft_sums_kernel");
+  const int nslots = (int)(grid.x * grid.y * grid.z);
+  const size_t part_bytes = (size_t)nslots * 64 * sizeof(float);
+  return ds2_bn2d_bwd_sums_from_partials(part, nslots, dgamma, dbeta, static_cast<char*>(ws) + part_bytes, ws_bytes - part_bytes, stream);
+}
+
 extern "C" int ds2_transpose2d_f32(const float* src, int ld_src, long long stride_src, float* dst, int ld_dst, long long stride_dst,
                                    int R, int Cc, int batch, void* stream) {
   DS2_REQUIRE(src && dst && R > 0 && Cc > 0 && batch > 0, "ds2_transpose2d_f32: bad args");
diff --git a/asr_amd/engine.py b/asr_amd/engine.py
--- a/asr_amd/engine.py
+++ b/asr_amd/engine.py
@@ -698,26 +698,28 @@
         with torch.cuda.stream(side):
             done(f"rnns.{l}")
     cp = "conv.seq_module."
-    da2 = ops.transpose_bft(dy, B, 32 * D2, T, to_tbf=False).view(B, 32, D2, T)
     m2, v2 = ctx.st2
     bf = cfg.precision == "bf16"
     if bf:
-        _, dy2p, dy2n = ops.bn2d_act_bwd_fused(ctx.y2, da2, lens_dev, m2, v2, W[cp + "4.weight"], W[cp + "4.bias"], Gr[cp + "4.weight"],
-                                               Gr[cp + "4.bias"], Gr[cp + "3.bias"], want_pad=CONV2_WGRAD != "nhwc", want_nhwc=True)
+        da2 = ops.transpose_bft_sums(dy, ctx.y2, lens_dev, m2, v2, W[cp + "4.weight"], W[cp + "4.bias"], Gr[cp + "4.weight"], Gr[cp + "4.bias"])
+        _, dy2p, dy2n = ops.bn2d_act_bwd_from_sums(ctx.y2, da2, lens_dev, m2, v2, W[cp + "4.weight"], W[cp + "4.bias"], Gr[cp + "4.weight"],
+                                                   Gr[cp + "4.bias"], Gr[cp + "3.bias"], want_pad=CONV2_WGRAD != "nhwc", want_nhwc=True)
         del da2
         if CONV2_WGRAD == "nhwc":
             ops.conv2_wgrad_nhwc_bf16(ctx.a1p, dy2n, lens_dev, Gr[cp + "3.weight"])
         else:
             ops.conv2_wgrad_bf16(ctx.a1p, dy2p, lens_dev, Gr[cp + "3.weight"], T)
-        da1 = ops.conv2_dgrad_bf16(dy2n, ctx.packs[1], ctx.packs[2], D1)
+        m1, v1 = ctx.st1
+        da1 = ops.conv2_dgrad_bf16_sums(dy2n, ctx.packs[1], ctx.packs[2], D1, ctx.y1, lens_dev, m1, v1, W[cp + "1.weight"], W[cp + "1.bias"],
+                                        Gr[cp + "1.weight"], Gr[cp + "1.bias"])
         del dy2p, dy2n
-        m1, v1 = ctx.st1
-        dy1, _, _ = ops.bn2d_act_bwd_fused(ctx.y1, da1, lens_dev, m1, v1, W[cp + "1.weight"], W[cp + "1.bias"], Gr[cp + "1.weight"],
-                                           Gr[cp + "1.bias"], Gr[cp + "0.bias"], want_f32=True)
+        dy1, _, _ = ops.bn2d_act_bwd_from_sums(ctx.y1, da1, lens_dev, m1, v1, W[cp + "1.weight"], W[cp + "1.bias"], Gr[cp + "1.weight"],
+                                               Gr[cp + "1.bias"], Gr[cp + "0.bias"], want_f32=True)
         del da1
         ops.conv1_wgrad_bf16(ctx.x16t, dy1, lens_dev, Gr[cp + "0.weight"], ctx.x.shape[3])
         ctx.x16t = None
     elif F32_CONV == "split":
+        da2 = ops.transpose_bft(dy, B, 32 * D2, T, to_tbf=False).view(B, 32, D2, T)
         dy2, dy2p, dy2n = ops.bn2d_act_bwd_fused(ctx.y2, da2, lens_dev, m2, v2, W[cp + "4.weight"], W[cp + "4.bias"], Gr[cp + "4.weight"],
                                                  Gr[cp + "4.bias"], Gr[cp + "3.bias"], want_f32=True, want_pad=True, want_nhwc=True)
         del da2
@@ -746,6 +748,7 @@
         Gr[cp + "0.bias"].copy_(ops.chan_sum(dy1))
         ops.conv1_wgrad(ctx.x, dy1, lens_dev, Gr[cp + "0.weight"])
     else:
+        da2 = ops.transpose_bft(dy, B, 32 * D2, T, to_tbf=False).view(B, 32, D2, T)
         dy2 = ops.bn2d_act_bwd(ctx.y2, da2, lens_dev, m2, v2, W[cp + "4.weight"], W[cp + "4.bias"], Gr[cp + "4.weight"], Gr[cp + "4.bias"])
         del da2
         Gr[cp + "3.bias"].copy_(ops.chan_sum(dy2))
diff --git a/asr_amd/ops.py b/asr_amd/ops.py
--- a/asr_amd/ops.py
+++ b/asr_amd/ops.py
@@ -643,6 +643,37 @@
     return d32, dpad, dnh
 
 
+def bn2d_act_bwd_from_sums(Y: Tensor, dA: Tensor, lens_dev: Tensor, mean, var, gamma, beta, dgamma: Tensor, dbeta: Tensor, dbias: Tensor,
+                           want_f32=False, want_pad=False, want_nhwc=False):
+    _chk_f32(Y, dA, mean, var, gamma, beta, dgamma, dbeta, dbias)
+    lib = _lib.load()
+    B, Cc, D, T = Y.shape
+    assert Cc == 32 and Y.is_contiguous() and dA.is_contiguous() and dA.shape == Y.shape
+    d32 = torch.empty_like(Y) if want_f32 else None
+    dpad = torch.empty(B, 32, D, lib.ds2_conv_padded_pitch(T), dtype=torch.bfloat16, device=Y.device) if want_pad else None
+    dnh = torch.empty(B, D, T, 32, dtype=torch.bfloat16, device=Y.device) if want_nhwc else None
+    wsb = lib.ds2_bn2d_act_bwd_from_sums_workspace_bytes(B, D, T)
+    ws = _ws(wsb, Y.device)
+    _lib.check(lib.ds2_bn2d_act_bwd_from_sums(Y.data_ptr(), dA.data_ptr(), B, D, T, lens_dev.data_ptr(), mean.data_ptr(), var.data_ptr(),
+                                              gamma.data_ptr(), beta.data_ptr(), BN_EPS, dgamma.data_ptr(), dbeta.data_ptr(), dbias.data_ptr(),
+                                              _ptr(d32), _ptr(dpad), _ptr(dnh), ws.data_ptr(), wsb, _stream()), "ds2_bn2d_act_bwd_from_sums")
+    return d32, dpad, dnh
+
+
+def transpose_bft_sums(src: Tensor, Y: Tensor, lens_dev: Tensor, mean, var, gamma, beta, dgamma: Tensor, dbeta: Tensor) -> Tensor:
+    _chk_f32(src, Y, mean, var, gamma, beta, dgamma, dbeta)
+    B, Cc, D, T = Y.shape
+    assert Cc == 32 and Y.is_contiguous() and src.is_contiguous() and src.numel() == Y.numel()
+    lib = _lib.load()
+    dst = torch.empty_like(Y)
+    wsb = lib.ds2_transpose_bft_sums_workspace_bytes(B, D, T)
+    ws = _ws(wsb, Y.device)
+    _lib.check(lib.ds2_transpose_bft_sums(src.data_ptr(), dst.data_ptr(), B, D, T, Y.data_ptr(), lens_dev.data_ptr(), mean.data_ptr(),
+                                          var.data_ptr(), gamma.data_ptr(), beta.data_ptr(), BN_EPS, dgamma.data_ptr(), dbeta.data_ptr(),
+                                          ws.data_ptr(), wsb, _stream()), "ds2_transpose_bft_sums")
+    return dst
+
+
 def chan_sum(Y: Tensor) -> Tensor:
     mean, _ = bn2d_stats(Y)
     B, Cc, D, T = Y.shape
@@ -831,6 +862,21 @@
     da1 = torch.empty(B, 32, D1, T, dtype=torch.float32, device=dy2_nhwc.device)
     _lib.check(_lib.load().ds2_conv2_dgrad_bf16(dy2_nhwc.data_ptr(), wd0.data_ptr(), wd1.data_ptr(), da1.data_ptr(), B, D1, T, _stream()),
                "ds2_conv2_dgrad_bf16")
+    return da1
+
+
+def conv2_dgrad_bf16_sums(dy2_nhwc: Tensor, wd0: Tensor, wd1: Tensor, D1: int, y1: Tensor, lens_dev: Tensor, mean, var, gamma, beta,
+                          dgamma: Tensor, dbeta: Tensor) -> Tensor:
+    _chk_f32(y1, mean, var, gamma, beta, dgamma, dbeta)
+    B, D2, T, _ = dy2_nhwc.shape
+    assert y1.is_contiguous() and tuple(y1.shape) == (B, 32, D1, T)
+    lib = _lib.load()
+    da1 = torch.empty(B, 32, D1, T, dtype=torch.float32, device=dy2_nhwc.device)
+    wsb = lib.ds2_conv2_dgrad_bf16_sums_workspace_bytes(B, D1, T)
+    ws = _ws(wsb, y1.device)
+    _lib.check(lib.ds2_conv2_dgrad_bf16_sums(dy2_nhwc.data_ptr(), wd0.data_ptr(), wd1.data_ptr(), da1.data_ptr(), B, D1, T, y1.data_ptr(),
+                                             lens_dev.data_ptr(), mean.data_ptr(), var.data_ptr(), gamma.data_ptr(), beta.data_ptr(), BN_EPS,
+                                             dgamma.data_ptr(), dbeta.data_ptr(), ws.data_ptr(), wsb, _stream()), "ds2_conv2_dgrad_bf16_sums")
     return da1
 
 
diff --git a/include/ds2hip.h b/include/ds2hip.h
--- a/include/ds2hip.h
+++ b/include/ds2hip.h
@@ -135,6 +135,21 @@
                                 float momentum, void* ws, size_t ws_bytes, void* stream);
 int ds2_conv2_dgrad_bf16(const void* dy2_nhwc, const void* wd0, const void* wd1, float* da1, int B, int D1, int T, void* stream);
 
+size_t ds2_bn2d_bwd_sums_from_partials_workspace_bytes(void);
+int ds2_bn2d_bwd_sums_from_partials(const float* part, int nslots, float* dgamma, float* dbeta, void* ws, size_t ws_bytes, void* stream);
+size_t ds2_conv2_dgrad_bf16_sums_workspace_bytes(int B, int D1, int T);
+int ds2_conv2_dgrad_bf16_sums(const void* dy2_nhwc, const void* wd0, const void* wd1, float* da1, int B, int D1, int T, const float* y1,
+                              const int* lens_dev, const float* mean, const float* var, const float* gamma, const float* beta, float eps,
+                              float* dgamma, float* dbeta, void* ws, size_t ws_bytes, void* stream);
+size_t ds2_transpose_bft_sums_workspace_bytes(int B, int D, int T);
+int ds2_transpose_bft_sums(const float* src, float* dst, int B, int D, int T, const float* Y, const int* lens_dev, const float* mean,
+                           const float* var, const float* gamma, const float* beta, float eps, float* dgamma, float* dbeta, void* ws,
+                           size_t ws_bytes, void* stream);
+size_t ds2_bn2d_act_bwd_from_sums_workspace_bytes(int B, int D, int T);
+int ds2_bn2d_act_bwd_from_sums(const float* Y, const float* dA, int B, int D, int T, const int* lens_dev, const float* mean, const float* var,
+                               const float* gamma, const float* beta, float eps, const float* dgamma, const float* dbeta, float* dbias,
+                               float* dy_f32, void* dy_pad, void* dy_nhwc, void* ws, size_t ws_bytes, void* stream);
+
 int ds2_conv_padded_pitch(int T);
 int ds2_padcast_bf16(const float* src, void* dst, long long R, int T, void* stream);
 size_t ds2_conv2_wgrad_bf16_workspace_bytes(int B, int D1);
```

Result: no change. 2867, median of 6 (+0.4%).
